# teofum/rust_raytracer

Measured on AMD Instinct MI355X. Metric: Msamples/sec (whole node), cornell_dragon 870k tri @1000spp, higher is better.
Workload: dtype f64; 1 GPU; scenes/cornell_dragon 1200x1200 @1000spp (10 replicas x 10x10 strata), 871200-tri stand-in mesh; spp=1000, seed=1, pipeline=auto, frames_in_flight=1, partition=1200-row bands round-robin over 1 GPU(s)

## Files before the change

### include/rt_mi355.h

```cpp
#ifndef RT_MI355_H
#define RT_MI355_H

#include <stdint.h>
#include <stddef.h>

#ifdef __cplusplus
extern "C" {
#endif

#define RT_MI355_ABI_VERSION 2

typedef enum RtStatus {
    RT_OK = 0,
    RT_E_INVALID = -1,
    RT_E_UNSUPPORTED = -2,
    RT_E_DEVICE = -3,
    RT_E_NOMEM = -4
} RtStatus;

typedef enum RtNodeType {
    RT_NODE_SPHERE = 1,
    RT_NODE_PLANE = 2,
    RT_NODE_MESH = 3,
    RT_NODE_LIST = 4,
// ... 58 lines not shown

typedef enum RtTextureType {
    RT_TEX_CONST_COLOR = 1,
    RT_TEX_CONST_FLOAT = 2,
    RT_TEX_CHECKER = 3,
    RT_TEX_CHECKER_SOLID = 4,
    RT_TEX_LERP = 5,
    RT_TEX_IMAGE = 6,
    RT_TEX_NOISE_SOLID = 7,
    RT_TEX_CHANNEL = 8,
    RT_TEX_UV_DEBUG = 9
} RtTextureType;

typedef struct RtTexture {
    uint32_t type;
    int32_t  a, b, c;
    uint32_t channel;
    uint32_t samples;
    double   v[3];
    double   scale;
    const float* texels;
    uint32_t width, height;
    const double*   perlin_vec;
    const uint32_t* perlin_perm;
} RtTexture;

typedef struct RtSceneDesc {
    uint32_t abi_version;
    uint32_t n_nodes;
    const RtNode* nodes;
    uint32_t n_child_indices;
    uint32_t n_transforms;
    const uint32_t* child_indices;
    const RtTransform* transforms;
    uint32_t n_meshes;
    uint32_t n_materials;
    const RtMesh* meshes;
    const RtMaterial* materials;
    uint32_t n_textures;
    uint32_t world_root;
    const RtTexture* textures;
    uint32_t lights_root;
    uint32_t flags;
} RtSceneDesc;

#define RT_SCENE_BVH_ON_DEVICE 1u

typedef struct RtCameraDesc {
    uint32_t image_width, image_height;
    double position[3];
    double first_pixel[3];
    double pixel_delta_u[3];
    double pixel_delta_v[3];
    double basis_u[3];
    double basis_v[3];
    uint32_t has_aperture;
    uint32_t _pad;
    double aperture_radius;
} RtCameraDesc;

typedef enum RtPrecision { RT_PRECISION_F64 = 0, RT_PRECISION_F32 = 1 } RtPrecision;
typedef enum RtPipeline { RT_PIPELINE_AUTO = 0, RT_PIPELINE_MEGAKERNEL = 1, RT_PIPELINE_WAVEFRONT = 2 } RtPipeline;

typedef struct RtRenderParams {
    uint32_t sqrt_spt;
    uint32_t thread_count;
    uint32_t max_depth;
    uint32_t has_background;
    double   light_bias;
    double   background[3];
    uint64_t seed;
    uint32_t band_rows;
    uint32_t n_parts;
    uint32_t part;
    uint32_t precision;
    uint32_t pipeline;
    uint32_t collect_stats;
} RtRenderParams;

typedef struct RtRenderStats {
    double   kernel_ms;
    double   traversal_kernel_ms;
    uint32_t n_launches;
    uint32_t pipeline_used;
    uint64_t samples;
    uint64_t rays;
    uint64_t mesh_rays;
    uint64_t node_visits;
    uint64_t tri_tests;
    uint64_t prim_tests;
    uint64_t bytes_node;
    uint64_t bytes_tri;
    uint64_t bytes_attr;
    uint64_t bytes_state;
    double   prims_kernel_ms;
    double   shade_kernel_ms;
    uint64_t bytes_state_prims;
    uint64_t bytes_state_shade;
    uint32_t n_iterations;
    uint32_t n_replica_groups;
    uint32_t n_tail_compactions;
    uint32_t _reserved;
} RtRenderStats;

typedef struct RtScene RtScene;

int rt_device_count(void);

int rt_scene_create(const RtSceneDesc* desc, int device, RtScene** out);
void rt_scene_destroy(RtScene* scene);

typedef struct RtSceneUpdateInfo {
    uint32_t n_meshes_refit;
    uint32_t n_triangles_refit;
    uint64_t bytes_uploaded;
    double   refit_kernel_ms;
    double   total_ms;
    uint32_t _reserved[4];
} RtSceneUpdateInfo;
int rt_scene_update(RtScene* scene, const RtSceneDesc* desc, RtSceneUpdateInfo* info_or_null);
int rt_scene_update_check(const RtSceneDesc* a, const RtSceneDesc* b);
int rt_scene_refit_mesh(const RtSceneDesc* a, const RtSceneDesc* b, uint32_t mesh, uint32_t f32, int32_t* children_out,
                        uint32_t* cones_out, float* boxes_out, uint32_t node_capacity, uint32_t* n_nodes_out,
                        double* tris_out, uint32_t* tri_order_out, uint32_t tri_capacity, uint32_t* n_tris_out);
int rt_debug_scene_mesh(const RtScene* scene, uint32_t mesh, uint32_t f32, int32_t* children_out, uint32_t* cones_out,
                        float* boxes_out, uint32_t node_capacity, uint32_t* n_nodes_out, double* tris_out,
                        uint32_t* tri_order_out, uint32_t tri_capacity, uint32_t* n_tris_out);
int rt_debug_scene_mesh_digest(const RtScene* scene, uint32_t f32, uint64_t out[8]);
int rt_debug_live_resources(uint64_t out[4]);

uint32_t rt_owned_rows(uint32_t image_height, const RtRenderParams* params);

int rt_render(const RtScene* scene, const RtCameraDesc* camera,
              const RtRenderParams* params, double* rgba_out);

int rt_render_device(const RtScene* scene, const RtCameraDesc* camera,
                     const RtRenderParams* params, double* d_rgba_out, void* stream);

int rt_get_stats(const RtScene* scene, RtRenderStats* out);

int rt_debug_trace_sample(const RtScene* scene, const RtCameraDesc* camera, const RtRenderParams* params,
                          uint32_t tid, uint32_t x, uint32_t y, uint32_t sx, uint32_t sy,
                          double* rgb_out, double* trace_out, uint32_t max_bounces);

int rt_debug_fuzzy_reflection(int device, uint32_t n, const double* reflected, const double* fuzz, const uint64_t* state, double* out, uint64_t* state_out);

#define RT_SCENE_INFO_ZERO_WEIGHT_STOP 1u
#define RT_SCENE_INFO_TEX_INTERPRETER 2u
#define RT_SCENE_INFO_VOLUMES 4u
int rt_scene_info(const RtSceneDesc* desc, uint32_t* flags_out);
int rt_scene_mesh_stats(const RtSceneDesc* desc, uint64_t out[8]);
int rt_scene_mesh_cones(const RtSceneDesc* desc, uint32_t mesh, uint32_t f32, int32_t* children_out, uint32_t* cones_out,
                        uint32_t node_capacity, uint32_t* n_nodes_out, double* tris_out, uint32_t tri_capacity, uint32_t* n_tris_out);
int rt_debug_handout_replay(const uint32_t* policy, uint32_t n, uint32_t waves, const uint32_t* order, uint32_t n_order, uint32_t* asks_out,
                            uint32_t capacity, uint32_t* n_asks_out, uint32_t* atomics_out);
int rt_scene_program(const RtSceneDesc* desc, int32_t* ops_out, uint32_t capacity, uint32_t* n_ops_out, uint64_t info[8]);

int rt_scene_set_tail_flag(RtScene* scene, int32_t* flag);

typedef struct RtAccum RtAccum;
int rt_accum_create(const RtScene* scene, const RtCameraDesc* camera, const RtRenderParams* params, RtAccum** out);
void rt_accum_destroy(RtAccum* acc);
int rt_accum_render(RtAccum* acc, uint32_t n_replicas, const RtRenderParams* params_or_null, void* stream);
uint32_t rt_accum_replicas_done(const RtAccum* acc);
int rt_accum_estimate(const RtAccum* acc, double* rgba_out);
int rt_accum_estimate_device(const RtAccum* acc, double* d_rgba_out, void* stream);
int rt_accum_preview_rgb8(const RtAccum* acc, uint8_t* rgb_out);
size_t rt_accum_state_size(const RtAccum* acc);
int rt_accum_save_state(const RtAccum* acc, void* buf, size_t size);
int rt_accum_load_state(RtAccum* acc, const void* buf, size_t size);
int rt_tonemap_rgb8_device(int device, const double* d_rgba, uint32_t width, uint32_t height, uint8_t* d_rgb, void* stream);

int rt_render_aov(const RtScene* scene, const RtCameraDesc* camera, const RtRenderParams* params, uint32_t n_replicas,
                  double* aov_out);
int rt_render_aov_device(const RtScene* scene, const RtCameraDesc* camera, const RtRenderParams* params, uint32_t n_replicas,
                         double* d_aov_out, void* stream);

#define RT_DENOISE_DEMODULATE 1u
#define RT_DENOISE_MAX_ITERATIONS 16u
typedef struct RtDenoiseParams {
    uint32_t iterations;
    uint32_t aov_replicas;
    uint32_t flags;
    uint32_t _reserved0;
    double   sigma_color, sigma_normal, sigma_albedo, sigma_depth;
    double   _reserved[4];
} RtDenoiseParams;
int rt_denoise_default_params(RtDenoiseParams* out);
int rt_denoise(int device, const double* rgba, const double* aov, uint32_t w, uint32_t h, const RtDenoiseParams* dp,
               double* rgba_out);
int rt_denoise_device(int device, const double* d_rgba, const double* d_aov, uint32_t w, uint32_t h,
                      const RtDenoiseParams* dp, double* d_rgba_out, void* stream);
int rt_accum_estimate_denoised(const RtAccum* acc, const RtDenoiseParams* dp, double* rgba_out);
int rt_accum_preview_denoised_rgb8(const RtAccum* acc, const RtDenoiseParams* dp, uint8_t* rgb_out);

typedef struct RtAdaptiveParams {
    double   threshold;
    double   floor;
    uint32_t min_replicas;
    uint32_t check_interval;
    uint32_t radius;
    uint32_t _reserved0;
    double   _reserved[4];
} RtAdaptiveParams;
int rt_adaptive_default_params(RtAdaptiveParams* out);
int rt_accum_set_adaptive(RtAccum* acc, const RtAdaptiveParams* params);
uint32_t rt_accum_active_pixels(const RtAccum* acc);
int rt_accum_finished(const RtAccum* acc);
int rt_accum_sample_counts(const RtAccum* acc, uint32_t* counts_out);
int rt_accum_noise(const RtAccum* acc, double* noise_out);

#define RT_LIGHT_GROUPS_MAX 16u
typedef struct RtLightGroups {
    uint32_t n_groups;
    uint32_t n_materials;
    const uint8_t* material_group;
    uint32_t background_group, unlit_group;
    uint32_t _reserved[4];
} RtLightGroups;
int rt_light_groups_auto(const RtSceneDesc* desc, uint32_t max_groups, int has_background, uint8_t* material_group_out,
                         uint32_t* background_group_out, uint32_t* n_groups_out);
int rt_render_light_groups(const RtScene* scene, const RtCameraDesc* camera, const RtRenderParams* params,
                           const RtLightGroups* groups, double* groups_out, double* rgba_out_or_null);
int rt_render_light_groups_device(const RtScene* scene, const RtCameraDesc* camera, const RtRenderParams* params,
                                  const RtLightGroups* groups, double* d_groups_out, double* d_rgba_out_or_null, void* stream);
int rt_light_mix(int device, const double* groups, uint32_t n_groups, uint32_t w, uint32_t h, const double* tints,
                 double* rgba_out);
int rt_light_mix_device(int device, const double* d_groups, uint32_t n_groups, uint32_t w, uint32_t h, const double* tints,
                        double* d_rgba_out, void* stream);

#define RT_RAY_HIT          1u
#define RT_RAY_FRONT_FACE   2u
#define RT_RAY_ENVIRONMENT  4u
typedef struct RtRayHit {
    double   t;
    double   pos[3], normal[3];
    double   u, v;
    int32_t  material;
    int32_t  node;
    int32_t  prim;
    uint32_t flags;
    uint64_t _reserved;
} RtRayHit;
typedef struct RtRayQueryStats {
    double   kernel_ms;
    uint64_t rays;
    uint32_t n_chunks, precision;
    uint32_t _reserved[4];
} RtRayQueryStats;

int rt_trace_rays(const RtScene* scene, uint64_t n, const double* origins, const double* dirs, uint32_t precision, RtRayHit* hits_out);
int rt_trace_rays_device(const RtScene* scene, uint64_t n, const double* d_origins, const double* d_dirs, uint32_t precision,
                         RtRayHit* d_hits_out, void* stream);
int rt_occluded(const RtScene* scene, uint64_t n, const double* origins, const double* dirs, const double* t_min, const double* t_max,
                uint32_t precision, uint8_t* out);
int rt_occluded_device(const RtScene* scene, uint64_t n, const double* d_origins, const double* d_dirs, const double* d_t_min,
                       const double* d_t_max, uint32_t precision, uint8_t* d_out, void* stream);
int rt_ray_query_stats(const RtScene* scene, RtRayQueryStats* out);
int rt_scene_op_nodes(const RtSceneDesc* desc, int32_t* nodes_out, uint32_t capacity, uint32_t* n_ops_out);

typedef struct RtBakeParams {
    uint32_t samples;
    uint32_t precision;
    uint64_t seed;
    double   bias;
    double   max_distance;
    uint32_t _reserved[4];
} RtBakeParams;
typedef struct RtBakeResult {
    double   visibility;
    double   bent[3];
} RtBakeResult;
int rt_bake_visibility(const RtScene* scene, uint64_t n, const double* positions, const double* normals, const RtBakeParams* params,
                       RtBakeResult* out);
int rt_bake_visibility_device(const RtScene* scene, uint64_t n, const double* d_positions, const double* d_normals,
                              const RtBakeParams* params, RtBakeResult* d_out, void* stream);
int rt_bake_visibility_hits_device(const RtScene* scene, uint64_t n, const RtRayHit* d_hits, const RtBakeParams* params,
                                   RtBakeResult* d_out, void* stream);
int rt_bake_stats(const RtScene* scene, RtRayQueryStats* out);

const char* rt_last_error(void);

#ifdef __cplusplus
}
#endif
#endif
```

### rust_raytracer_amd/api.py

```python
from __future__ import annotations

import ctypes as C
import os
import sys
from typing import Optional, Sequence

import numpy as np

PKG_DIR = os.path.dirname(os.path.abspath(__file__))
REPO_DIR = os.path.dirname(PKG_DIR)

RT_OK = 0
RT_E_INVALID, RT_E_UNSUPPORTED, RT_E_DEVICE, RT_E_NOMEM = -1, -2, -3, -4
RT_PRECISION_F64, RT_PRECISION_F32 = 0, 1
RT_PIPELINE_AUTO, RT_PIPELINE_MEGAKERNEL, RT_PIPELINE_WAVEFRONT = 0, 1, 2
RT_SCENE_BVH_ON_DEVICE = 1
RT_MESH_HIT_BACK_FACES = 2
RT_DENOISE_DEMODULATE = 1
RT_DENOISE_MAX_ITERATIONS = 16
AOV_CHANNELS = 8

(RT_NODE_SPHERE, RT_NODE_PLANE, RT_NODE_MESH, RT_NODE_LIST, RT_NODE_TRANSFORM, RT_NODE_BVH,
 RT_NODE_SKY, RT_NODE_SUN, RT_NODE_VOLUME, RT_NODE_NULL) = range(1, 11)
(RT_MAT_LAMBERTIAN, RT_MAT_METAL, RT_MAT_DIELECTRIC, RT_MAT_GLOSSY, RT_MAT_EMISSIVE,
# ... 128 lines not shown
                ("background_group", C.c_uint32), ("unlit_group", C.c_uint32), ("_reserved", C.c_uint32 * 4)]

    @classmethod
    def make(cls, n_groups: int, material_group, background_group: int = 0, unlit_group: int = 0) -> "RtLightGroups":
        table = np.ascontiguousarray(material_group, dtype=np.uint8).copy()
        g = cls()
        g.n_groups, g.n_materials = n_groups, table.size
        g.material_group = table.ctypes.data_as(C.POINTER(C.c_uint8))
        g.background_group, g.unlit_group = background_group, unlit_group
        g._table = table
        return g

    @property
    def table(self) -> np.ndarray:
        return self._table


class RtSceneUpdateInfo(C.Structure):
    _fields_ = [("n_meshes_refit", C.c_uint32), ("n_triangles_refit", C.c_uint32), ("bytes_uploaded", C.c_uint64),
                ("refit_kernel_ms", C.c_double), ("total_ms", C.c_double), ("_reserved", C.c_uint32 * 4)]


class RtRayQueryStats(C.Structure):
    _fields_ = [("kernel_ms", C.c_double), ("rays", C.c_uint64), ("n_chunks", C.c_uint32), ("precision", C.c_uint32),
                ("_reserved", C.c_uint32 * 4)]


RT_RAY_HIT, RT_RAY_FRONT_FACE, RT_RAY_ENVIRONMENT = 1, 2, 4
RtRayHit = np.dtype([("t", "<f8"), ("pos", "<f8", (3,)), ("normal", "<f8", (3,)), ("u", "<f8"), ("v", "<f8"), ("material", "<i4"),
                     ("node", "<i4"), ("prim", "<i4"), ("flags", "<u4"), ("_reserved", "<u8")])
assert RtRayHit.itemsize == 96


class RtBakeParams(C.Structure):
    _fields_ = [("samples", C.c_uint32), ("precision", C.c_uint32), ("seed", C.c_uint64), ("bias", C.c_double),
                ("max_distance", C.c_double), ("_reserved", C.c_uint32 * 4)]

    @classmethod
    def defaults(cls, **overrides) -> "RtBakeParams":
        p = cls(samples=64, precision=RT_PRECISION_F64, seed=0, bias=1e-3, max_distance=float("inf"))
        for k, v in overrides.items():
            setattr(p, k, v)
        return p


RtBakeResult = np.dtype([("visibility", "<f8"), ("bent", "<f8", (3,))])
assert RtBakeResult.itemsize == 32


class RtError(RuntimeError):
    def __init__(self, status: int, message: str):
        super().__init__(f"rt status {status}: {message}")
        self.status = status


HOST_LIB_PATH = os.path.join(PKG_DIR, "librt_host.so")
DEVICE_LIB_PATH = os.environ.get("RT_DEVICE_LIB") or os.path.join(PKG_DIR, "librt_mi355.so")

_host_lib = None
_device_lib = None


def load_host_lib() -> C.CDLL:
    global _host_lib
    if _host_lib is None:
        if not os.path.exists(HOST_LIB_PATH):
            raise FileNotFoundError(
                f"{HOST_LIB_PATH} is missing: run `python -c 'import __graft_entry__ as g; g.build()'`")
        lib = C.CDLL(HOST_LIB_PATH)
        lib.rth_load.argtypes = [C.c_int, C.POINTER(C.c_char_p), C.POINTER(C.c_void_p)]
        lib.rth_load.restype = C.c_int
        lib.rth_destroy.argtypes = [C.c_void_p]
        lib.rth_destroy.restype = None
        lib.rth_scene.argtypes = [C.c_void_p]
        lib.rth_scene.restype = C.POINTER(RtSceneDesc)
        lib.rth_camera.argtypes = [C.c_void_p]
        lib.rth_camera.restype = C.POINTER(RtCameraDesc)
        lib.rth_params.argtypes = [C.c_void_p]
        lib.rth_params.restype = C.POINTER(RtRenderParams)
        lib.rth_gpus.argtypes = [C.c_void_p]
        lib.rth_gpus.restype = C.c_uint32
        lib.rth_band_rows.argtypes = [C.c_uint32, C.c_uint32]
        lib.rth_band_rows.restype = C.c_uint32
        lib.rth_samples_per_pixel.argtypes = [C.c_void_p]
        lib.rth_samples_per_pixel.restype = C.c_uint32
        lib.rth_pick.argtypes = [C.c_void_p, C.c_void_p, C.c_uint32]
        lib.rth_pick.restype = C.c_uint32
        lib.rth_ao.argtypes = [C.c_void_p, C.POINTER(C.c_double)]
        lib.rth_ao.restype = C.c_uint32
        lib.rth_log.argtypes = [C.c_void_p]
        lib.rth_log.restype = C.c_char_p
        lib.rth_make_camera.argtypes = [C.c_uint32, C.c_double, C.c_double, C.c_double, C.c_double,
                                        C.POINTER(C.c_double), C.POINTER(C.c_double),
                                        C.POINTER(RtCameraDesc)]
        lib.rth_make_camera.restype = C.c_int
        lib.rth_tonemap_rgb8.argtypes = [C.c_void_p, C.c_uint32, C.c_uint32, C.c_void_p]
        lib.rth_tonemap_rgb8.restype = C.c_int
        lib.rth_save_png.argtypes = [C.c_char_p, C.c_void_p, C.c_uint32, C.c_uint32]
        lib.rth_save_png.restype = C.c_int
        lib.rth_load_image.argtypes = [C.c_char_p, C.POINTER(C.POINTER(C.c_float)), C.POINTER(C.c_uint32), C.POINTER(C.c_uint32)]
        lib.rth_load_image.restype = C.c_int
        lib.rth_free_image.argtypes = [C.POINTER(C.c_float)]
        lib.rth_free_image.restype = None
        lib.rth_last_error.argtypes = []
        lib.rth_last_error.restype = C.c_char_p
        _host_lib = lib
    return _host_lib


def load_device_lib() -> C.CDLL:
    global _device_lib
    if _device_lib is None:
        if not os.path.exists(DEVICE_LIB_PATH):
            raise FileNotFoundError(
                f"{DEVICE_LIB_PATH} is missing — the HIP render path was not built "
                "(run __graft_entry__.build()); refusing to fall back to any CPU path")
        if "torch" not in sys.modules and os.environ.get("RT_NO_TORCH_PRELOAD", "0") != "1":
            try:
                import torch
            except Exception:
                pass
        lib = C.CDLL(DEVICE_LIB_PATH)
        lib.rt_device_count.argtypes = []
        lib.rt_device_count.restype = C.c_int
        lib.rt_scene_create.argtypes = [C.POINTER(RtSceneDesc), C.c_int, C.POINTER(C.c_void_p)]
        lib.rt_scene_create.restype = C.c_int
        lib.rt_scene_destroy.argtypes = [C.c_void_p]
        lib.rt_scene_destroy.restype = None
        lib.rt_owned_rows.argtypes = [C.c_uint32, C.POINTER(RtRenderParams)]
        lib.rt_owned_rows.restype = C.c_uint32
        lib.rt_render.argtypes = [C.c_void_p, C.POINTER(RtCameraDesc), C.POINTER(RtRenderParams), C.c_void_p]
        lib.rt_render.restype = C.c_int
        lib.rt_render_device.argtypes = [C.c_void_p, C.POINTER(RtCameraDesc), C.POINTER(RtRenderParams),
                                         C.c_void_p, C.c_void_p]
        lib.rt_render_device.restype = C.c_int
        lib.rt_get_stats.argtypes = [C.c_void_p, C.POINTER(RtRenderStats)]
        lib.rt_get_stats.restype = C.c_int
        lib.rt_debug_trace_sample.argtypes = [C.c_void_p, C.POINTER(RtCameraDesc), C.POINTER(RtRenderParams),
                                              C.c_uint32, C.c_uint32, C.c_uint32, C.c_uint32, C.c_uint32,
                                              C.POINTER(C.c_double), C.POINTER(C.c_double), C.c_uint32]
        lib.rt_debug_trace_sample.restype = C.c_int
        lib.rt_scene_info.argtypes = [C.POINTER(RtSceneDesc), C.POINTER(C.c_uint32)]
        lib.rt_scene_info.restype = C.c_int
        if hasattr(lib, "rt_scene_set_tail_flag"):
            lib.rt_scene_set_tail_flag.argtypes = [C.c_void_p, C.c_void_p]
            lib.rt_scene_set_tail_flag.restype = C.c_int
        if hasattr(lib, "rt_scene_mesh_stats"):
            lib.rt_scene_mesh_stats.argtypes = [C.POINTER(RtSceneDesc), C.POINTER(C.c_uint64)]
            lib.rt_scene_mesh_stats.restype = C.c_int
        if hasattr(lib, "rt_scene_mesh_cones"):
            lib.rt_scene_mesh_cones.argtypes = [C.POINTER(RtSceneDesc), C.c_uint32, C.c_uint32, C.c_void_p, C.c_void_p, C.c_uint32,
                                                C.POINTER(C.c_uint32), C.c_void_p, C.c_uint32, C.POINTER(C.c_uint32)]
            lib.rt_scene_mesh_cones.restype = C.c_int
        if hasattr(lib, "rt_debug_handout_replay"):
            lib.rt_debug_handout_replay.argtypes = [C.c_void_p, C.c_uint32, C.c_uint32, C.c_void_p, C.c_uint32, C.c_void_p, C.c_uint32,
                                                    C.POINTER(C.c_uint32), C.c_void_p]
            lib.rt_debug_handout_replay.restype = C.c_int
        if hasattr(lib, "rt_accum_create"):
            for name, res, args in (
                    ("rt_accum_create", C.c_int, [C.c_void_p, C.POINTER(RtCameraDesc), C.POINTER(RtRenderParams), C.POINTER(C.c_void_p)]),
                    ("rt_accum_destroy", None, [C.c_void_p]),
                    ("rt_accum_render", C.c_int, [C.c_void_p, C.c_uint32, C.POINTER(RtRenderParams), C.c_void_p]),
                    ("rt_accum_replicas_done", C.c_uint32, [C.c_void_p]),
                    ("rt_accum_estimate", C.c_int, [C.c_void_p, C.c_void_p]),
                    ("rt_accum_estimate_device", C.c_int, [C.c_void_p, C.c_void_p, C.c_void_p]),
                    ("rt_accum_preview_rgb8", C.c_int, [C.c_void_p, C.c_void_p]),
                    ("rt_accum_state_size", C.c_size_t, [C.c_void_p]),
                    ("rt_accum_save_state", C.c_int, [C.c_void_p, C.c_void_p, C.c_size_t]),
                    ("rt_accum_load_state", C.c_int, [C.c_void_p, C.c_void_p, C.c_size_t]),
                    ("rt_tonemap_rgb8_device", C.c_int, [C.c_int, C.c_void_p, C.c_uint32, C.c_uint32, C.c_void_p, C.c_void_p])):
                fn = getattr(lib, name)
                fn.argtypes = args
                fn.restype = res
        if hasattr(lib, "rt_render_aov"):
            dp = C.POINTER(RtDenoiseParams)
            for name, res, args in (
                    ("rt_render_aov", C.c_int, [C.c_void_p, C.POINTER(RtCameraDesc), C.POINTER(RtRenderParams), C.c_uint32, C.c_void_p]),
                    ("rt_render_aov_device", C.c_int, [C.c_void_p, C.POINTER(RtCameraDesc), C.POINTER(RtRenderParams), C.c_uint32,
                                                       C.c_void_p, C.c_void_p]),
                    ("rt_denoise_default_params", C.c_int, [dp]),
                    ("rt_denoise", C.c_int, [C.c_int, C.c_void_p, C.c_void_p, C.c_uint32, C.c_uint32, dp, C.c_void_p]),
                    ("rt_denoise_device", C.c_int, [C.c_int, C.c_void_p, C.c_void_p, C.c_uint32, C.c_uint32, dp, C.c_void_p, C.c_void_p]),
                    ("rt_accum_estimate_denoised", C.c_int, [C.c_void_p, dp, C.c_void_p]),
                    ("rt_accum_preview_denoised_rgb8", C.c_int, [C.c_void_p, dp, C.c_void_p])):
                fn = getattr(lib, name)
                fn.argtypes = args
                fn.restype = res
        if hasattr(lib, "rt_accum_set_adaptive"):
            for name, res, args in (
                    ("rt_adaptive_default_params", C.c_int, [C.POINTER(RtAdaptiveParams)]),
                    ("rt_accum_set_adaptive", C.c_int, [C.c_void_p, C.POINTER(RtAdaptiveParams)]),
                    ("rt_accum_active_pixels", C.c_uint32, [C.c_void_p]),
                    ("rt_accum_finished", C.c_int, [C.c_void_p]),
                    ("rt_accum_sample_counts", C.c_int, [C.c_void_p, C.c_void_p]),
                    ("rt_accum_noise", C.c_int, [C.c_void_p, C.c_void_p])):
                fn = getattr(lib, name)
                fn.argtypes = args
                fn.restype = res
        if hasattr(lib, "rt_render_light_groups"):
            lg = C.POINTER(RtLightGroups)
            for name, res, args in (
                    ("rt_light_groups_auto", C.c_int, [C.POINTER(RtSceneDesc), C.c_uint32, C.c_int, C.c_void_p, C.POINTER(C.c_uint32),
                                                       C.POINTER(C.c_uint32)]),
                    ("rt_render_light_groups", C.c_int, [C.c_void_p, C.POINTER(RtCameraDesc), C.POINTER(RtRenderParams), lg, C.c_void_p,
                                                         C.c_void_p]),
                    ("rt_render_light_groups_device", C.c_int, [C.c_void_p, C.POINTER(RtCameraDesc), C.POINTER(RtRenderParams), lg,
                                                                C.c_void_p, C.c_void_p, C.c_void_p]),
                    ("rt_light_mix", C.c_int, [C.c_int, C.c_void_p, C.c_uint32, C.c_uint32, C.c_uint32, C.c_void_p, C.c_void_p]),
                    ("rt_light_mix_device", C.c_int, [C.c_int, C.c_void_p, C.c_uint32, C.c_uint32, C.c_uint32, C.c_void_p, C.c_void_p,
                                                      C.c_void_p])):
                fn = getattr(lib, name)
                fn.argtypes = args
                fn.restype = res
        if hasattr(lib, "rt_scene_update"):
            mesh_out = [C.c_void_p, C.c_void_p, C.c_void_p, C.c_uint32, C.POINTER(C.c_uint32), C.c_void_p, C.c_void_p, C.c_uint32,
                        C.POINTER(C.c_uint32)]
            for name, res, args in (
                    ("rt_scene_update", C.c_int, [C.c_void_p, C.POINTER(RtSceneDesc), C.POINTER(RtSceneUpdateInfo)]),
                    ("rt_scene_update_check", C.c_int, [C.POINTER(RtSceneDesc), C.POINTER(RtSceneDesc)]),
                    ("rt_scene_refit_mesh", C.c_int, [C.POINTER(RtSceneDesc), C.POINTER(RtSceneDesc), C.c_uint32, C.c_uint32] + mesh_out),
                    ("rt_debug_scene_mesh", C.c_int, [C.c_void_p, C.c_uint32, C.c_uint32] + mesh_out),
                    ("rt_debug_scene_mesh_digest", C.c_int, [C.c_void_p, C.c_uint32, C.POINTER(C.c_uint64)])):
                fn = getattr(lib, name)
                fn.argtypes = args
                fn.restype = res
        if hasattr(lib, "rt_trace_rays"):
            for name, res, args in (
                    ("rt_trace_rays", C.c_int, [C.c_void_p, C.c_uint64, C.c_void_p, C.c_void_p, C.c_uint32, C.c_void_p]),
                    ("rt_trace_rays_device", C.c_int, [C.c_void_p, C.c_uint64, C.c_void_p, C.c_void_p, C.c_uint32, C.c_void_p, C.c_void_p]),
                    ("rt_occluded", C.c_int, [C.c_void_p, C.c_uint64, C.c_void_p, C.c_void_p, C.c_void_p, C.c_void_p, C.c_uint32, C.c_void_p]),
                    ("rt_occluded_device", C.c_int, [C.c_void_p, C.c_uint64, C.c_void_p, C.c_void_p, C.c_void_p, C.c_void_p, C.c_uint32,
                                                     C.c_void_p, C.c_void_p]),
                    ("rt_ray_query_stats", C.c_int, [C.c_void_p, C.POINTER(RtRayQueryStats)]),
                    ("rt_scene_op_nodes", C.c_int, [C.POINTER(RtSceneDesc), C.c_void_p, C.c_uint32, C.POINTER(C.c_uint32)])):
                fn = getattr(lib, name)
                fn.argtypes = args
                fn.restype = res
        if hasattr(lib, "rt_bake_visibility"):
            for name, res, args in (
                    ("rt_bake_visibility", C.c_int, [C.c_void_p, C.c_uint64, C.c_void_p, C.c_void_p, C.POINTER(RtBakeParams), C.c_void_p]),
                    ("rt_bake_visibility_device", C.c_int, [C.c_void_p, C.c_uint64, C.c_void_p, C.c_void_p, C.POINTER(RtBakeParams),
                                                            C.c_void_p, C.c_void_p]),
                    ("rt_bake_visibility_hits_device", C.c_int, [C.c_void_p, C.c_uint64, C.c_void_p, C.POINTER(RtBakeParams), C.c_void_p,
                                                                 C.c_void_p]),
                    ("rt_bake_stats", C.c_int, [C.c_void_p, C.POINTER(RtRayQueryStats)])):
                fn = getattr(lib, name)
                fn.argtypes = args
                fn.restype = res
        if hasattr(lib, "rt_debug_live_resources"):
            lib.rt_debug_live_resources.argtypes = [C.POINTER(C.c_uint64)]
            lib.rt_debug_live_resources.restype = C.c_int
        lib.rt_last_error.argtypes = []
        lib.rt_last_error.restype = C.c_char_p
        _device_lib = lib
    return _device_lib


RT_SCENE_INFO_ZERO_WEIGHT_STOP, RT_SCENE_INFO_TEX_INTERPRETER, RT_SCENE_INFO_VOLUMES = 1, 2, 4


def scene_info(desc) -> int:
    lib = load_device_lib()
    flags = C.c_uint32()
    st = lib.rt_scene_info(desc, C.byref(flags))
    if st != RT_OK:
        raise RtError(st, lib.rt_last_error().decode())
    return flags.value


def scene_mesh_stats(desc) -> dict:
    lib = load_device_lib()
    out = (C.c_uint64 * 8)()
    st = lib.rt_scene_mesh_stats(desc, out)
    if st != RT_OK:
        raise RtError(st, lib.rt_last_error().decode())
    return dict(zip(("triangles", "bvh2_nodes", "bvh4_nodes", "bvh2_depth", "bvh4_stack", "ops", "rebuilt_groups", "rebuilt_prims"),
                    [int(x) for x in out]))


def live_resources() -> tuple:
    lib = load_device_lib()
    out = (C.c_uint64 * 4)()
    st = lib.rt_debug_live_resources(out)
    if st != RT_OK:
        raise RtError(st, lib.rt_last_error().decode())
    return tuple(int(x) for x in out)


def handout_replay(n: int, waves: int, order, policy=None, out=None) -> tuple:
    lib = load_device_lib()
    order = np.ascontiguousarray(order, dtype=np.uint32)
    pol = None if policy is None else np.asarray(policy, dtype=np.uint32)
    cap = n // 64 + 4 * waves + 16
    if out is None or out.shape[0] < cap:
        out = np.empty((cap, 3), dtype=np.uint32)
    n_asks = C.c_uint32(0)
    atomics = np.zeros(2, dtype=np.uint32)
    st = lib.rt_debug_handout_replay(None if pol is None else pol.ctypes.data, n, waves, order.ctypes.data, order.size, out.ctypes.data,
                                     out.shape[0], C.byref(n_asks), atomics.ctypes.data)
    if st != 0:
        raise RuntimeError(f"rt_debug_handout_replay: {lib.rt_last_error().decode()}")
    if n_asks.value > out.shape[0]:
        raise RuntimeError(f"rt_debug_handout_replay: {n_asks.value} asks for n = {n}, {waves} waves")
    return out[:n_asks.value], int(atomics[0]), int(atomics[1])


def scene_mesh_cones(desc, mesh: int = 0, f32: bool = False) -> tuple:
    import numpy as np
    lib = load_device_lib()
    nn, nt = C.c_uint32(), C.c_uint32()
    st = lib.rt_scene_mesh_cones(desc, mesh, int(f32), None, None, 0, C.byref(nn), None, 0, C.byref(nt))
    if st != RT_OK:
        raise RtError(st, lib.rt_last_error().decode())
    children = np.zeros((nn.value, 4), dtype=np.int32)
    cones = np.zeros((nn.value, 4), dtype=np.uint32)
    tris = np.zeros((nt.value, 3, 3), dtype=np.float64)
    st = lib.rt_scene_mesh_cones(desc, mesh, int(f32), children.ctypes.data, cones.ctypes.data, nn.value, C.byref(nn),
                                 tris.ctypes.data, nt.value, C.byref(nt))
    if st != RT_OK:
        raise RtError(st, lib.rt_last_error().decode())
    return children, cones.view(np.int8).reshape(-1, 4, 4), tris


def scene_update_check(a, b) -> None:
    lib = load_device_lib()
    st = lib.rt_scene_update_check(a, b)
    if st != RT_OK:
        raise RtError(st, lib.rt_last_error().decode())


def _mesh_export(call) -> dict:
    lib = load_device_lib()
    nn, nt = C.c_uint32(), C.c_uint32()
    st = call(None, None, None, 0, C.byref(nn), None, None, 0, C.byref(nt))
    if st != RT_OK:
        raise RtError(st, lib.rt_last_error().decode())
    children = np.zeros((nn.value, 4), dtype=np.int32)
    cones = np.zeros((nn.value, 4), dtype=np.uint32)
    boxes = np.zeros((nn.value, 4, 2, 3), dtype=np.float32)
    tris = np.zeros((nt.value, 3, 3), dtype=np.float64)
    order = np.zeros(nt.value, dtype=np.uint32)
    st = call(children.ctypes.data, cones.ctypes.data, boxes.ctypes.data, nn.value, C.byref(nn), tris.ctypes.data, order.ctypes.data,
              nt.value, C.byref(nt))
    if st != RT_OK:
        raise RtError(st, lib.rt_last_error().decode())
    return {"children": children, "cones": cones.view(np.int8).reshape(-1, 4, 4), "boxes": boxes, "tris": tris, "order": order}


def scene_refit_mesh(a, b, mesh: int = 0, f32: bool = False) -> dict:
    lib = load_device_lib()
    return _mesh_export(lambda *out: lib.rt_scene_refit_mesh(a, b, mesh, int(f32), *out))


def scene_program(desc) -> tuple:
    import numpy as np
    lib = load_device_lib()
    lib.rt_scene_program.argtypes = [C.POINTER(RtSceneDesc), C.POINTER(C.c_int32), C.c_uint32, C.POINTER(C.c_uint32), C.POINTER(C.c_uint64)]
    lib.rt_scene_program.restype = C.c_int
    n = C.c_uint32()
    info = (C.c_uint64 * 8)()
    st = lib.rt_scene_program(desc, None, 0, C.byref(n), info)
    if st != RT_OK:
        raise RtError(st, lib.rt_last_error().decode())
    ops = np.zeros((n.value, 4), dtype=np.int32)
    st = lib.rt_scene_program(desc, ops.ctypes.data_as(C.POINTER(C.c_int32)), n.value, C.byref(n), info)
    if st != RT_OK:
        raise RtError(st, lib.rt_last_error().decode())
    plan = int(info[6])
    return ops, {"mesh_ops": int(info[0]), "groups": int(info[1]), "group_nodes": int(info[2]), "group_stack": int(info[3]),
                 "lights": int(info[4]), "volumes": int(info[5]), "group_prims": int(info[7]),
                 "split": bool(plan & 1), "vol_prims": bool(plan & 2), "multi_mesh": bool(plan & 4), "group_bvh": bool(plan & 8)}


def scene_op_nodes(desc) -> np.ndarray:
    lib = load_device_lib()
    n = C.c_uint32()
    st = lib.rt_scene_op_nodes(desc, None, 0, C.byref(n))
    if st != RT_OK:
        raise RtError(st, lib.rt_last_error().decode())
    nodes = np.full(n.value, -1, dtype=np.int32)
    st = lib.rt_scene_op_nodes(desc, nodes.ctypes.data, n.value, C.byref(n))
    if st != RT_OK:
        raise RtError(st, lib.rt_last_error().decode())
    return nodes


def light_groups_auto(desc, max_groups: int = RT_LIGHT_GROUPS_MAX, has_background: bool = False) -> RtLightGroups:
    lib = load_device_lib()
    d = desc.contents if hasattr(desc, "contents") else desc
    table = np.zeros(d.n_materials, dtype=np.uint8)
    bg, n = C.c_uint32(), C.c_uint32()
    st = lib.rt_light_groups_auto(desc, max_groups, int(bool(has_background)), table.ctypes.data, C.byref(bg), C.byref(n))
    if st != RT_OK:
        raise RtError(st, lib.rt_last_error().decode())
    return RtLightGroups.make(n.value, table, bg.value, 0)


def light_mix(groups: np.ndarray, tints, device: int = 0) -> np.ndarray:
    lib = load_device_lib()
    groups = np.ascontiguousarray(groups, dtype=np.float64)
    if groups.ndim != 4 or groups.shape[3] != 4:
        raise ValueError(f"light_mix: expected a (G, H, W, 4) array, got {groups.shape}")
    g, h, w = groups.shape[:3]
    tints = np.asarray(tints, dtype=np.float64)
    if tints.ndim == 1:
        tints = np.repeat(tints[:, None], 3, axis=1)
    tints = np.ascontiguousarray(tints)
    if tints.shape != (g, 3):
        raise ValueError(f"light_mix: expected {g} x 3 tints, got {tints.shape}")
    out = np.empty((h, w, 4), dtype=np.float64)
    st = lib.rt_light_mix(device, groups.ctypes.data, g, w, h, tints.ctypes.data, out.ctypes.data)
    if st != RT_OK:
        raise RtError(st, lib.rt_last_error().decode())
    return out


def owned_rows(height: int, params: RtRenderParams) -> list:
    if params.band_rows == 0 or params.n_parts <= 1:
        return list(range(height))
    return [y for y in range(height) if (y // params.band_rows) % params.n_parts == params.part]


class HostScene:

    def __init__(self, args: Sequence[str], cwd: Optional[str] = None):
        lib = load_host_lib()
        argv = [b"rtrace"] + [a.encode() for a in args]
        arr = (C.c_char_p * len(argv))(*argv)
        handle = C.c_void_p()
        old = os.getcwd()
        try:
            os.chdir(cwd or REPO_DIR)
            st = lib.rth_load(len(argv), arr, C.byref(handle))
        finally:
            os.chdir(old)
        if st != RT_OK:
            raise RtError(st, lib.rth_last_error().decode())
        self._lib = lib
        self._h = handle
        self.desc = lib.rth_scene(handle)
        self.camera = lib.rth_camera(handle).contents
        self.params = lib.rth_params(handle).contents.copy()
        self.gpus = lib.rth_gpus(handle)
        self.spp = lib.rth_samples_per_pixel(handle)
        self.log = lib.rth_log(handle).decode()
        xy = np.zeros((lib.rth_pick(handle, None, 0), 2), dtype=np.uint32)
        lib.rth_pick(handle, xy.ctypes.data, len(xy))
        self.pick = [(int(x), int(y)) for x, y in xy]
        dist = C.c_double()
        self.ao = (int(lib.rth_ao(handle, C.byref(dist))), dist.value)

    @property
    def width(self) -> int:
        return self.camera.image_width

    @property
    def height(self) -> int:
        return self.camera.image_height

    def close(self):
        if self._h:
            self._lib.rth_destroy(self._h)
            self._h = None

    def __del__(self):
        try:
            self.close()
        except Exception:
            pass


def tonemap_rgb8(rgba: np.ndarray) -> np.ndarray:
    lib = load_host_lib()
    rgba = np.ascontiguousarray(rgba, dtype=np.float64)
    h, w = rgba.shape[:2]
    out = np.empty((h, w, 3), dtype=np.uint8)
# ... 420 lines not shown
```

### rust_raytracer_amd/csrc/rt_bvh.cpp

```cpp
#include "rt_bvh.h"

#include <algorithm>
#include <cmath>
#include <cstdlib>
#include <limits>

#include "rt_refit.h"
#include "rt_scene.h"

namespace rt {
namespace {

constexpr int kMaxBins = 64;
static int g_bins = 16;
constexpr double kInf = std::numeric_limits<double>::infinity();

struct Box {
    double lo[3] = {kInf, kInf, kInf};
    double hi[3] = {-kInf, -kInf, -kInf};
    void grow(const double* p) {
        for (int a = 0; a < 3; a++) {
            if (p[a] < lo[a]) lo[a] = p[a];
            if (p[a] > hi[a]) hi[a] = p[a];
        }
// ... 125 lines not shown
    BvhBuild out;
    if (n_tris <= b.max_leaf) {
        BuildNode root{};
        Box bx;
        for (uint32_t t = 0; t < n_tris; t++) bx.grow(b.tri_box[t]);
        for (int a = 0; a < 3; a++) {
            root.lo0[a] = bx.lo[a]; root.hi0[a] = bx.hi[a];
            root.lo1[a] = kInf; root.hi1[a] = -kInf;
        }
        root.c0 = n_tris ? Builder::leaf_ref(0, n_tris) : kEmptyChild;
        root.c1 = kEmptyChild;
        out.nodes.push_back(root);
        out.max_depth = 1;
    } else {
        Box root_box;
        b.build(0, n_tris, &root_box, 0);
        out.nodes = std::move(b.nodes);
        out.max_depth = b.max_depth;
    }
    out.tri_order = std::move(b.order);
    return out;
}


namespace {
struct Cand {
    int32_t ref;
    double lo[3], hi[3];
    double area() const {
        double dx = hi[0] - lo[0], dy = hi[1] - lo[1], dz = hi[2] - lo[2];
        if (!(dx >= 0 && dy >= 0 && dz >= 0)) return -1.0;
        return dx * dy + dy * dz + dz * dx;
    }
};
template <int W>
struct Collapser {
    const BvhBuild& b2;
    BvhNBuild<W> out;
    uint32_t build(int32_t n2, uint32_t depth, uint32_t stack_above) {
        uint32_t idx = uint32_t(out.nodes.size());
        out.nodes.emplace_back();
        if (depth + 1 > out.max_depth) out.max_depth = depth + 1;
        std::vector<Cand> c;
        auto add_children = [&](int32_t node2) {
            const BuildNode& n = b2.nodes[size_t(node2)];
            Cand a{n.c0, {n.lo0[0], n.lo0[1], n.lo0[2]}, {n.hi0[0], n.hi0[1], n.hi0[2]}};
            Cand b{n.c1, {n.lo1[0], n.lo1[1], n.lo1[2]}, {n.hi1[0], n.hi1[1], n.hi1[2]}};
            if (a.ref != kEmptyChild) c.push_back(a);
            if (b.ref != kEmptyChild) c.push_back(b);
        };
        add_children(n2);
        for (;;) {
            if (c.size() >= size_t(W)) break;
            int best = -1;
            double best_area = -1.0;
            for (size_t i = 0; i < c.size(); i++)
                if (c[i].ref >= 0 && c[i].area() > best_area) { best_area = c[i].area(); best = int(i); }
            if (best < 0) break;
            int32_t expand = c[size_t(best)].ref;
            c.erase(c.begin() + best);
            add_children(expand);
        }
        uint32_t n_children = uint32_t(c.size());
        uint32_t stack_here = stack_above + (n_children > 0 ? n_children - 1 : 0);
        if (stack_here + 1 > out.max_stack) out.max_stack = stack_here + 1;
        BuildNodeN<W> node{};
        for (int k = 0; k < W; k++) {
            node.child[k] = kEmptyChild;
            for (int a = 0; a < 3; a++) { node.lo[k][a] = kInf; node.hi[k][a] = -kInf; }
        }
        for (uint32_t k = 0; k < n_children; k++) {
            for (int a = 0; a < 3; a++) { node.lo[k][a] = c[k].lo[a]; node.hi[k][a] = c[k].hi[a]; }
            node.child[k] = c[k].ref;
        }
        out.nodes[idx] = node;
        for (uint32_t k = 0; k < n_children; k++)
            if (c[k].ref >= 0) {
                uint32_t child_idx = build(c[k].ref, depth + 1, stack_here);
                out.nodes[idx].child[k] = int32_t(child_idx);
            }
        return idx;
    }
};
}

namespace {
template <int W>
BvhNBuild<W> collapse(const BvhBuild& b2) {
    Collapser<W> c{b2, {}};
    c.out.nodes.reserve(b2.nodes.size() / (W == 4 ? 2 : 3) + 4);
    c.build(0, 0, 0);
    for (int a = 0; a < 3; a++) { c.out.root_lo[a] = kInf; c.out.root_hi[a] = -kInf; }
    const BuildNodeN<W>& r = c.out.nodes[0];
    for (int k = 0; k < W; k++)
        if (r.child[k] != kEmptyChild)
            for (int a = 0; a < 3; a++) {
                c.out.root_lo[a] = std::min(c.out.root_lo[a], r.lo[k][a]);
                c.out.root_hi[a] = std::max(c.out.root_hi[a], r.hi[k][a]);
            }
    return std::move(c.out);
}
}

Bvh4Build collapse_bvh4(const BvhBuild& b2) { return collapse<4>(b2); }



ConeLimits cone_limits(bool f32) {
    if (f32) return ConeLimits{1.0 / 32.0, 1e-12, 1e12};
    return ConeLimits{1.0 / 1048576.0, 1e-100, 1e100};
}

void build_mesh_cones(const std::vector<BuildNode4>& nodes4, const std::vector<TriRec<double>>& tris, const ConeLimits& lim,
                      std::vector<uint32_t>* out) {
    const size_t n_tris = tris.size();
    std::vector<double> normal(3 * n_tris);
    const double kNaN = std::numeric_limits<double>::quiet_NaN();
    for (size_t t = 0; t < n_tris; t++) rf_tri_normal(tris[t].v0, tris[t].e1, tris[t].e2, lim, &normal[3 * t]);
    struct Below {
        uint32_t lo = UINT32_MAX, hi = 0, count = 0;
        double sum[3] = {0.0, 0.0, 0.0};
        void add(const Below& o) {
            lo = std::min(lo, o.lo); hi = std::max(hi, o.hi); count += o.count;
            for (int a = 0; a < 3; a++) sum[a] += o.sum[a];
        }
    };
    auto cone_word = [&](const Below& b) -> uint32_t { return rf_cone_word(normal.data(), b.lo, b.hi, b.count, b.sum); };
    out->assign(4 * nodes4.size(), kNeutralCone);
    std::vector<Below> below(nodes4.size());
    for (size_t i = nodes4.size(); i-- > 0;) {
        const BuildNode4& nd = nodes4[i];
        Below all;
        for (int k = 0; k < 4; k++) {
            const int32_t ch = nd.child[k];
            if (ch == kEmptyChild) continue;
            Below b;
            if (ch >= 0) {
                if (size_t(ch) <= i || size_t(ch) >= nodes4.size()) { all.sum[0] = kNaN; continue; }
                b = below[size_t(ch)];
            } else {
                const uint32_t code = uint32_t(~ch), first = code >> 3, count = (code & 7u) + 1u;
                if (size_t(first) + count > n_tris) { all.sum[0] = kNaN; continue; }
                b.lo = first; b.hi = first + count; b.count = count;
                for (uint32_t t = first; t < first + count; t++)
                    for (int a = 0; a < 3; a++) b.sum[a] += normal[3 * size_t(t) + a];
            }
            (*out)[4 * i + size_t(k)] = cone_word(b);
            all.add(b);
        }
        below[i] = all;
    }
}

}
```

### rust_raytracer_amd/csrc/rt_bvh.h

```cpp
#pragma once
#include <cstdint>
#include <string>
#include <vector>

#include "rt_scene.h"

namespace rt {

struct BuildNode {
    double lo0[3], hi0[3], lo1[3], hi1[3];
    int32_t c0, c1;
};

struct BvhBuild {
    std::vector<BuildNode> nodes;
    std::vector<uint32_t> tri_order;
    uint32_t max_depth = 0;
};

BvhBuild build_bvh(const double* positions, const uint32_t* tri_pos, uint32_t n_tris, uint32_t max_leaf);

bool build_bvh_device(const double* positions, uint32_t n_positions, const uint32_t* tri_pos, uint32_t n_tris, uint32_t max_leaf,
                      BvhBuild* out, std::string* err);

template <int W>
struct BuildNodeN {
    double lo[W][3], hi[W][3];
    int32_t child[W];
};
template <int W>
struct BvhNBuild {
    std::vector<BuildNodeN<W>> nodes;
    uint32_t max_depth = 0;
    uint32_t max_stack = 0;
    double root_lo[3], root_hi[3];
};
using BuildNode4 = BuildNodeN<4>;
using Bvh4Build = BvhNBuild<4>;
Bvh4Build collapse_bvh4(const BvhBuild& bvh2);

struct ConeLimits {
    double sigma;
    double min_edge;
    double max_edge;
};
ConeLimits cone_limits(bool f32);
void build_mesh_cones(const std::vector<BuildNode4>& nodes4, const std::vector<TriRec<double>>& tris, const ConeLimits& lim,
                      std::vector<uint32_t>* out);

}
```

### rust_raytracer_amd/csrc/rt_kernels.hip

```cpp
#include <hip/hip_runtime.h>

#include <algorithm>
#include <array>
#include <chrono>
#include <cmath>
#include <cstdio>
#include <cstdlib>
#include <cstring>
#include <memory>
#include <new>
#include <string>
#include <type_traits>
#include <variant>
#include <vector>

#include "rt_aov.h"
#include "rt_bake.h"
#include "rt_compile.h"
#include "rt_device.h"
#include "rt_owned.h"
#include "rt_query.h"
#include "rt_refit.h"
#include "rt_wavefront.h"

// ... 85 lines not shown
    }
}

template <typename R>
__global__ void k_trace_sample(SceneView<R> sc, CameraView<R> cam, ParamsView<R> prm, uint32_t tid, uint32_t px, uint32_t py,
                               uint32_t sx, uint32_t sy, double* rgb, double* trace, uint32_t max_bounces, uint32_t* n_out) {
    extern __shared__ int lds_stack[];
    if (threadIdx.x != 0) return;
    LaneCounters cnt;
    Rng rng;
    rng.key(prm.seed, tid, uint64_t(py) * cam.width + px, sy * cam.sqrt_spt + sx);
    PathState<R> ps;
    ps.ray = get_ray(cam, px, py, sx, sy, rng);
    ps.throughput = mk<R>(1, 1, 1);
    ps.radiance = mk<R>(0, 0, 0);
    ps.depth = cam.max_depth;
    uint32_t n = 0;
    while (ps.depth != 0) {
        Best<R> best;
        world_test<R, false, true>(sc, ps.ray, R(0.001), best, lds_stack, int(blockDim.x), cnt, &rng);
        if (n < max_bounces) {
            double* t = trace + 17 * n;
            for (int k = 0; k < 17; k++) t[k] = 0;
            t[0] = double(best.t);
            t[4] = -1; t[5] = -1; t[6] = double(best.tri);
            if (best.pc >= 0) {
                HitInfo<R> h = resolve_hit<R, true>(sc, ps.ray, best);
                t[1] = double(h.pos.x); t[2] = double(h.pos.y); t[3] = double(h.pos.z);
                t[4] = double(h.material);
                t[5] = double(sc.ops[best.pc].type);
                t[8] = double(h.normal.x); t[9] = double(h.normal.y); t[10] = double(h.normal.z);
            }
            t[11] = double(ps.ray.o.x); t[12] = double(ps.ray.o.y); t[13] = double(ps.ray.o.z);
            t[14] = double(ps.ray.d.x); t[15] = double(ps.ray.d.y); t[16] = double(ps.ray.d.z);
        }
        n++;
        bool cont = shade<R, false, true>(sc, prm, ps, best, rng, cnt);
        ps.depth--;
        if (cont && ps.depth == 0) end_black(ps);
        if (!cont) break;
    }
    rgb[0] = double(ps.radiance.x); rgb[1] = double(ps.radiance.y); rgb[2] = double(ps.radiance.z);
    *n_out = n;
}

struct DeviceBuffers {
    std::vector<DevBuf<char>> allocs;
    uint64_t uploaded_bytes = 0;
    void adopt(DeviceBuffers& from, const void* p) {
        auto it = std::find_if(from.allocs.begin(), from.allocs.end(), [p](const DevBuf<char>& b) { return b.get() == p; });
        if (it == from.allocs.end()) return;
        allocs.push_back(std::move(*it));
        from.allocs.erase(it);
    }
    template <typename T> int alloc(size_t bytes, T** out) {
        allocs.emplace_back();
        if (int st = allocs.back().reserve(bytes)) return st;
        *out = reinterpret_cast<T*>(allocs.back().get());
        return RT_OK;
    }
    template <typename T> int upload(const std::vector<T>& v, const T** out) {
        *out = nullptr;
        T* p = nullptr;
        if (int st = alloc((v.empty() ? 1 : v.size()) * sizeof(T), &p)) return st;
        if (!v.empty()) HIP_TRY(hipMemcpy(p, v.data(), v.size() * sizeof(T), hipMemcpyHostToDevice));
        uploaded_bytes += v.size() * sizeof(T);
        *out = p;
        return RT_OK;
    }
};

template <typename R, size_t N> void cast_arr(R (&dst)[N], const double (&src)[N]) {
    for (size_t i = 0; i < N; i++) dst[i] = R(src[i]);
}

template <typename R>
struct DeviceScene {
    using Real = R;
    DeviceBuffers buf;
    SceneView<R> view{};

    int build(const CompiledScene& cs, const DeviceScene<R>* keep = nullptr) {
        const bool mesh_tables = keep == nullptr;
        std::vector<Bounds<R>> bounds(cs.bounds.size());
        for (size_t i = 0; i < bounds.size(); i++) {
            cast_arr(bounds[i].lo, cs.bounds[i].lo);
            cast_arr(bounds[i].hi, cs.bounds[i].hi);
        }
        std::vector<Xform<R>> xforms(cs.xforms.size());
        for (size_t i = 0; i < xforms.size(); i++) {
            cast_arr(xforms[i].m, cs.xforms[i].m);
            cast_arr(xforms[i].inv, cs.xforms[i].inv);
        }
        std::vector<SpherePrim<R>> spheres(cs.spheres.size());
        for (size_t i = 0; i < spheres.size(); i++) {
            cast_arr(spheres[i].center, cs.spheres[i].center);
            spheres[i].radius = R(cs.spheres[i].radius);
            spheres[i].material = cs.spheres[i].material;
            spheres[i]._pad = 0;
        }
        std::vector<PlanePrim<R>> planes(cs.planes.size());
        for (size_t i = 0; i < planes.size(); i++) {
            const auto& s = cs.planes[i];
            cast_arr(planes[i].corner, s.corner); cast_arr(planes[i].normal, s.normal);
            cast_arr(planes[i].u, s.u); cast_arr(planes[i].v, s.v);
            cast_arr(planes[i].inv_u, s.inv_u); cast_arr(planes[i].inv_v, s.inv_v);
            planes[i].area = R(s.area);
            planes[i].material = s.material;
            planes[i].backface = s.backface;
        }
        std::vector<SunPrim<R>> suns(cs.suns.size());
        for (size_t i = 0; i < suns.size(); i++) {
            cast_arr(suns[i].direction, cs.suns[i].direction);
            suns[i].material = cs.suns[i].material;
            suns[i]._pad = 0;
        }
        std::vector<BvhNode<R>> nodes(mesh_tables ? cs.nodes.size() : 0);
        for (size_t i = 0; i < nodes.size(); i++) {
            const BuildNode& s = cs.nodes[i];
            BvhNode<R>& n = nodes[i];
            for (int a = 0; a < 3; a++) {
                rf_pad_box2<R>(s.lo0[a], s.hi0[a], &n.lo0[a], &n.hi0[a]);
                rf_pad_box2<R>(s.lo1[a], s.hi1[a], &n.lo1[a], &n.hi1[a]);
            }
            n.c0 = s.c0;
            n.c1 = s.c1;
        }
        std::vector<BvhNode4f> nodes4(mesh_tables ? cs.nodes4.size() : 0);
        {
            size_t inst = 0;
            std::vector<std::pair<uint32_t, double>> pads;
            for (const MeshInst& mi : cs.meshes) {
                const Bounds<double>& b = cs.mesh_bounds[inst++];
                pads.emplace_back(mi.node4_base, rf_pad_of_box(b.lo, b.hi));
            }
            std::sort(pads.begin(), pads.end());
            size_t pi = 0;
            for (size_t i = 0; i < nodes4.size(); i++) {
                while (pi + 1 < pads.size() && pads[pi + 1].first <= i) pi++;
                const double m = pads.empty() ? 0.0 : pads[pi].second;
                const BuildNode4& sn = cs.nodes4[i];
                BvhNode4f& dn = nodes4[i];
                for (int k = 0; k < 4; k++) {
                    float* lo[3] = {&dn.lox[k], &dn.loy[k], &dn.loz[k]};
                    float* hi[3] = {&dn.hix[k], &dn.hiy[k], &dn.hiz[k]};
                    for (int a = 0; a < 3; a++) rf_pad_box4f(sn.lo[k][a], sn.hi[k][a], m, lo[a], hi[a]);
                    dn.child[k] = sn.child[k];
                    dn._pad[k] = 0;
                }
            }
        }
        std::vector<BvhNode4q> nodes4q(mesh_tables ? cs.nodes4.size() : 0);
        std::vector<BvhNode4q> group_nodes;
        {
            auto pad_of = [&]() {
                std::vector<std::pair<uint32_t, double>> pads;
                size_t inst = 0;
                for (const MeshInst& mi : cs.meshes) {
                    const Bounds<double>& b = cs.mesh_bounds[inst++];
                    pads.emplace_back(mi.node4_base, rf_pad_of_box(b.lo, b.hi));
                }
                std::sort(pads.begin(), pads.end());
                return pads;
            };
            auto quantise = [](const BuildNode4& sn, double m, BvhNode4q& qn) -> bool {
                for (int k = 0; k < 4; k++) qn.child[k] = sn.child[k];
                return rf_quantise4(sn.lo, sn.hi, sn.child, m, qn.org, qn.cell, qn.qlo, qn.qhi);
            };
            const auto pads4 = pad_of();
            size_t pi = 0;
            for (size_t i = 0; i < nodes4q.size(); i++) {
                while (pi + 1 < pads4.size() && pads4[pi + 1].first <= i) pi++;
                const BuildNode4& sn = cs.nodes4[i];
                BvhNode4q& qn = nodes4q[i];
                if (!quantise(sn, pads4.empty() ? 0.0 : pads4[pi].second, qn))
                    return set_err(RT_E_UNSUPPORTED, "BVH node does not fit the 8-bit grid");
            }
            group_nodes.resize(cs.group_nodes4.size());
            for (size_t g = 0; g < cs.groups.size(); g++) {
                const GroupRec<double>& gr = cs.groups[g];
                double S = 0.0;
                for (int a = 0; a < 3; a++) S = std::fmax(S, std::fmax(std::fabs(gr.lo[a]), std::fabs(gr.hi[a])));
                if (!std::isfinite(S)) return set_err(RT_E_UNSUPPORTED, "primitive group with an unbounded box");
                const size_t end = g + 1 < cs.groups.size() ? cs.groups[g + 1].root : cs.group_nodes4.size();
                for (size_t i = gr.root; i < end; i++) {
                    const BuildNode4& sn = cs.group_nodes4[i];
                    BvhNode4q& qn = group_nodes[i];
                    if (!quantise(sn, S * (1.0 / 524288.0), qn))
                        return set_err(RT_E_UNSUPPORTED, "group BVH node does not fit the 8-bit grid");
                }
            }
        }
        std::vector<uint32_t> cone_words;
        if (mesh_tables) build_mesh_cones(cs.nodes4, cs.tris, cone_limits(sizeof(R) == 4), &cone_words);
        std::vector<MeshNode4qc> nodes4qc(mesh_tables ? cs.nodes4.size() : 0);
        for (size_t i = 0; i < nodes4qc.size(); i++) {
            nodes4qc[i].node = nodes4q[i];
            for (int k = 0; k < 4; k++) nodes4qc[i].cones.word[k] = cone_words[4 * i + size_t(k)];
            for (uint32_t& x : nodes4qc[i]._pad) x = 0;
        }
        std::vector<Bounds<R>> mesh_bounds(cs.mesh_bounds.size());
        for (size_t i = 0; i < mesh_bounds.size(); i++)
            for (int a = 0; a < 3; a++) {
                mesh_bounds[i].lo[a] = round_down<R>(cs.mesh_bounds[i].lo[a]);
                mesh_bounds[i].hi[a] = round_up<R>(cs.mesh_bounds[i].hi[a]);
            }
        std::vector<TriRec<R>> tris(mesh_tables ? cs.tris.size() : 0);
        for (size_t i = 0; i < tris.size(); i++) {
            cast_arr(tris[i].v0, cs.tris[i].v0); cast_arr(tris[i].e1, cs.tris[i].e1); cast_arr(tris[i].e2, cs.tris[i].e2);
            tris[i]._pad = R(0);
        }
        std::vector<TriAttr<R>> attrs(mesh_tables ? cs.attrs.size() : 0);
        for (size_t i = 0; i < attrs.size(); i++) {
            const auto& s = cs.attrs[i];
            cast_arr(attrs[i].n0, s.n0); cast_arr(attrs[i].n1, s.n1); cast_arr(attrs[i].n2, s.n2);
            cast_arr(attrs[i].uv0, s.uv0); cast_arr(attrs[i].uv1, s.uv1); cast_arr(attrs[i].uv2, s.uv2);
            attrs[i].has_uv = s.has_uv;
            attrs[i]._pad = 0;
        }
        std::vector<MaterialParams<R>> mparams(cs.material_params.size());
        for (size_t i = 0; i < mparams.size(); i++) {
            mparams[i].ior = R(cs.material_params[i].ior);
            mparams[i].inv_ior = R(cs.material_params[i].inv_ior);
            auto r0_of = [](R x) { R r0 = (R(1) - x) / (R(1) + x); return r0 * r0; };
            mparams[i].inv_ior_r = R(1) / mparams[i].ior;
            mparams[i].r0_glossy = r0_of(mparams[i].inv_ior);
            mparams[i].r0_front = r0_of(mparams[i].inv_ior_r);
            mparams[i].r0_back = r0_of(mparams[i].ior);
        }
        std::vector<TextureRec<R>> textures(cs.textures.size());
        for (size_t i = 0; i < textures.size(); i++) {
            const auto& s = cs.textures[i];
            textures[i].type = s.type; textures[i].aux = s.aux; textures[i].data = s.data;
            textures[i].width = s.width; textures[i].height = s.height; textures[i]._pad = 0;
            cast_arr(textures[i].v, s.v);
            textures[i].scale = R(s.scale);
        }
        std::vector<VolumeRec<R>> volumes(cs.volumes.size());
        for (size_t i = 0; i < volumes.size(); i++) {
            volumes[i].neg_inv_density = R(cs.volumes[i].neg_inv_density);
            volumes[i].material = cs.volumes[i].material;
            volumes[i]._pad = 0;
        }
        std::vector<R> perlin_vec(cs.perlin_vec.size());
        for (size_t i = 0; i < perlin_vec.size(); i++) perlin_vec[i] = R(cs.perlin_vec[i]);
        int st;
        if ((st = buf.upload(cs.ops, &view.ops)) != RT_OK) return st;
        if ((st = buf.upload(bounds, &view.bounds)) != RT_OK) return st;
        if ((st = buf.upload(cs.chain_offsets, &view.chain_offsets)) != RT_OK) return st;
        if ((st = buf.upload(cs.chain_items, &view.chain_items)) != RT_OK) return st;
        if ((st = buf.upload(xforms, &view.xforms)) != RT_OK) return st;
        if ((st = buf.upload(spheres, &view.spheres)) != RT_OK) return st;
        if ((st = buf.upload(planes, &view.planes)) != RT_OK) return st;
        if ((st = buf.upload(suns, &view.suns)) != RT_OK) return st;
        if ((st = buf.upload(cs.meshes, &view.meshes)) != RT_OK) return st;
        if ((st = buf.upload(volumes, &view.volumes)) != RT_OK) return st;
        if (mesh_tables) {
            if ((st = buf.upload(nodes, &view.nodes)) != RT_OK) return st;
            if ((st = buf.upload(nodes4, &view.nodes4)) != RT_OK) return st;
            if ((st = buf.upload(nodes4qc, &view.nodes4q)) != RT_OK) return st;
            if ((st = buf.upload(tris, &view.tris)) != RT_OK) return st;
            if ((st = buf.upload(attrs, &view.attrs)) != RT_OK) return st;
        } else {
            view.nodes = keep->view.nodes; view.nodes4 = keep->view.nodes4; view.nodes4q = keep->view.nodes4q;
            view.tris = keep->view.tris; view.attrs = keep->view.attrs;
        }
        if ((st = buf.upload(mesh_bounds, &view.mesh_bounds)) != RT_OK) return st;
        if ((st = buf.upload(cs.mesh_ops, &view.mesh_ops)) != RT_OK) return st;
        view.n_mesh_ops = int32_t(cs.mesh_ops.size());
        std::vector<MeshOpRec<R>> mesh_op_recs(cs.mesh_ops.size());
        for (size_t m = 0; m < mesh_op_recs.size(); m++) {
            const Op& op = cs.ops[size_t(cs.mesh_ops[m])];
            const MeshInst& mi = cs.meshes[size_t(op.arg)];
            MeshOpRec<R>& r = mesh_op_recs[m];
            r.pc = cs.mesh_ops[m];
            r.chain = op.chain;
            r.node4_base = mi.node4_base;
            const int32_t cb = cs.chain_offsets[size_t(op.chain)], ce = cs.chain_offsets[size_t(op.chain) + 1];
            r.flags = (mi.flags & 0xFFFFu) | (uint32_t(std::min(ce - cb, 0xFFFF)) << 16);
            for (int a = 0; a < 3; a++) { r.lo[a] = mesh_bounds[size_t(op.arg)].lo[a]; r.hi[a] = mesh_bounds[size_t(op.arg)].hi[a]; }
            for (int k = 0; k < 12; k++) r.inv[k] = ce - cb == 1 ? xforms[size_t(cs.chain_items[size_t(cb)])].inv[k] : R(0);
        }
        if ((st = buf.upload(mesh_op_recs, &view.mesh_op_recs)) != RT_OK) return st;
        std::vector<GroupRec<R>> groups(cs.groups.size());
        for (size_t g = 0; g < groups.size(); g++) {
            groups[g].root = cs.groups[g].root;
            for (int a = 0; a < 3; a++) { groups[g].lo[a] = round_down<R>(cs.groups[g].lo[a]); groups[g].hi[a] = round_up<R>(cs.groups[g].hi[a]); }
        }
        if ((st = buf.upload(groups, &view.groups)) != RT_OK) return st;
        if ((st = buf.upload(group_nodes, &view.group_nodes)) != RT_OK) return st;
        if ((st = buf.upload(cs.group_prims, &view.group_prims)) != RT_OK) return st;
        if ((st = buf.upload(cs.group_guards, &view.group_guards)) != RT_OK) return st;
        view.n_group_nodes = int32_t(group_nodes.size());
        view.group_stack_levels = int32_t(cs.max_group_stack);
        if ((st = buf.upload(cs.materials, &view.materials)) != RT_OK) return st;
        if ((st = buf.upload(mparams, &view.material_params)) != RT_OK) return st;
        if ((st = buf.upload(textures, &view.textures)) != RT_OK) return st;
        if ((st = buf.upload(cs.texels, &view.texels)) != RT_OK) return st;
        if ((st = buf.upload(perlin_vec, &view.perlin_vec)) != RT_OK) return st;
        if ((st = buf.upload(cs.perlin_perm, &view.perlin_perm)) != RT_OK) return st;
        if ((st = buf.upload(cs.lights, &view.lights)) != RT_OK) return st;
        {
            struct Tbl { const void* data; size_t bytes; };
            const Tbl tbl[ST_COUNT] = {
                {cs.ops.data(), cs.ops.size() * sizeof(Op)}, {bounds.data(), bounds.size() * sizeof(Bounds<R>)},
                {cs.chain_offsets.data(), cs.chain_offsets.size() * 4}, {cs.chain_items.data(), cs.chain_items.size() * 4},
                {xforms.data(), xforms.size() * sizeof(Xform<R>)}, {spheres.data(), spheres.size() * sizeof(SpherePrim<R>)},
                {planes.data(), planes.size() * sizeof(PlanePrim<R>)}, {suns.data(), suns.size() * sizeof(SunPrim<R>)},
                {cs.meshes.data(), cs.meshes.size() * sizeof(MeshInst)}, {cs.materials.data(), cs.materials.size() * sizeof(MaterialRec)},
                {mparams.data(), mparams.size() * sizeof(MaterialParams<R>)}, {textures.data(), textures.size() * sizeof(TextureRec<R>)},
                {cs.lights.data(), cs.lights.size() * sizeof(LightRec)}};
            auto pack = [&](const int (&order)[ST_COUNT], SmallLayout& L, const char** out) -> int {
                std::vector<char> blob;
                for (int k : order) {
                    const size_t off = (blob.size() + 15) & ~size_t(15);
                    blob.resize(off + tbl[k].bytes);
                    if (tbl[k].bytes) std::memcpy(blob.data() + off, tbl[k].data, tbl[k].bytes);
                    L.begin[k] = uint32_t(off);
                    L.end[k] = uint32_t(off + tbl[k].bytes);
                }
                blob.resize((blob.size() + 15) & ~size_t(15));
                L.total_bytes = uint32_t(blob.size());
                return buf.upload(blob, out);
            };
            const int order_prims[ST_COUNT] = {ST_OPS, ST_CHAIN_OFFSETS, ST_CHAIN_ITEMS, ST_XFORMS, ST_MESHES, ST_SUNS, ST_PLANES, ST_BOUNDS, ST_SPHERES,
                                               ST_MATERIALS, ST_MATERIAL_PARAMS, ST_LIGHTS, ST_TEXTURES};
            const int order_shade[ST_COUNT] = {ST_OPS, ST_CHAIN_OFFSETS, ST_CHAIN_ITEMS, ST_XFORMS, ST_MESHES, ST_SUNS, ST_LIGHTS, ST_PLANES, ST_MATERIALS,
                                               ST_MATERIAL_PARAMS, ST_TEXTURES, ST_SPHERES, ST_BOUNDS};
            if ((st = pack(order_prims, view.lay, &view.small_blob)) != RT_OK) return st;
            if ((st = pack(order_shade, view.lay_shade, &view.small_blob_shade)) != RT_OK) return st;
        }
        view.n_lights = cs.n_top_lights;
        view.inv_n_lights = R(1) / R(cs.n_top_lights);
        view.lights_is_list = cs.lights_is_list;
        view.stop_on_zero_weight = cs.zero_weight_stop ? 1 : 0;
        if (const char* e = std::getenv("RT_ZERO_WEIGHT_STOP")) view.stop_on_zero_weight = std::atoi(e) != 0;
        view.stack_entries = int32_t(std::max(cs.max_bvh_depth + 2, cs.max_bvh4_stack + 1));
        view.n_ops = int32_t(cs.ops.size());
        HIP_TRY(hipDeviceSynchronize());
        return RT_OK;
    }
    void take_mesh_tables(DeviceScene<R>& from) {
        for (const void* p : {(const void*)view.nodes, (const void*)view.nodes4, (const void*)view.nodes4q, (const void*)view.tris, (const void*)view.attrs})
            buf.adopt(from.buf, p);
    }
};

struct HeldDesc {
    RtSceneDesc d{};
    std::vector<RtNode> nodes;
    std::vector<uint32_t> child_indices;
// ... 99 lines not shown
    return "scene update: the description has another structure than the scene (first difference: " + field + ")";
}

template <typename R>
struct PathPool {
    WfPool<R> view{};
    WfPool<R>* dev = nullptr;
    uint32_t* queue[2] = {nullptr, nullptr};
    uint32_t* mesh_queue = nullptr;
    std::vector<DevBuf<char>> owned;
};
template <typename R> using PoolPair = std::array<PathPool<R>, 2>;
using AnyPools = std::variant<std::monostate, PoolPair<float>, PoolPair<double>>;

struct ChunkStage {
    DevBuf<char> staging;
    Event ev0, ev1;
};

}

struct RtScene {
    int device = -1;
    rt::CompiledScene compiled;
    std::unique_ptr<rt::DeviceScene<double>> f64;
    std::unique_ptr<rt::DeviceScene<float>> f32;
    rt::Stream stream;
    rt::Event ev0, ev1;
    rt::DevBuf<rt::DeviceCounters> d_counters;
    RtRenderStats stats{};
    int32_t* tail_flag = nullptr;
    uint64_t content_digest = 0;
    rt::HeldDesc held;
    uint64_t generation = 0;
    std::vector<rt::RefitMesh> refit;
    struct Wavefront {
        rt::AnyPools pools;
        rt::DevBuf<uint2> mesh_spill;
        rt::DevBuf<rt::WfCounters> d_ctr;
        rt::PinnedBuf<rt::WfCounters> h_ctr;
        rt::DevBuf<double> sample_L, acc;
        rt::DevBuf<uint8_t> sample_G, lg_table;
        rt::DevBuf<double> acc_g;
        rt::Event ev_res[2];
        std::vector<rt::Event> events;
    } wf;
    struct Query {
        rt::AnyPools pools;
        rt::DevBuf<uint2> mesh_spill;
        rt::DevBuf<rt::WfCounters> d_ctr;
        rt::PinnedBuf<rt::WfCounters> h_ctr;
        rt::DevBuf<int32_t> op_node;
        rt::DevBuf<uint32_t> tri_order;
        uint64_t tables_generation = ~0ull;
        rt::ChunkStage stage;
        RtRayQueryStats stats{};
    } rq;
    struct Bake {
        rt::ChunkStage stage;
        RtRayQueryStats stats{};
    } bake;
    ~RtScene() { if (device >= 0) (void)hipSetDevice(device); }
};

namespace rt {

template <typename R> CameraView<R> make_camera_view(const RtCameraDesc& c, const RtRenderParams& p) {
    CameraView<R> v{};
    for (int i = 0; i < 3; i++) {
        v.position[i] = R(c.position[i]);
        v.first_pixel[i] = R(c.first_pixel[i]);
        v.pdu[i] = R(c.pixel_delta_u[i]);
        v.pdv[i] = R(c.pixel_delta_v[i]);
        v.basis_u[i] = R(c.basis_u[i]);
        v.basis_v[i] = R(c.basis_v[i]);
    }
    v.aperture_radius = R(c.aperture_radius);
    v.inv_sqrt_spt = R(1.0 / double(p.sqrt_spt));
    v.has_aperture = int32_t(c.has_aperture);
    v.width = c.image_width;
    v.height = c.image_height;
    v.sqrt_spt = p.sqrt_spt;
    v.thread_count = p.thread_count;
    v.max_depth = p.max_depth;
    return v;
}

template <typename R> ParamsView<R> make_params_view(const RtRenderParams& p, uint32_t owned) {
    ParamsView<R> v{};
    v.light_bias = R(p.light_bias);
    for (int i = 0; i < 3; i++) v.background[i] = p.has_background ? R(p.background[i]) : R(0);
    v.seed = p.seed;
    v.band_rows = p.band_rows;
    v.n_parts = p.n_parts;
    v.part = p.part;
    v.owned_rows = owned;
    v.spp = double(p.sqrt_spt) * double(p.sqrt_spt) * double(p.thread_count);
    v.inv_spp = 1.0 / v.spp;
    return v;
}

template <typename R>
int render_typed(RtScene* s, DeviceScene<R>& ds, const RtCameraDesc& cam, const RtRenderParams& p, uint32_t owned,
                 uint32_t t_first, uint32_t n, double* d_out, hipStream_t stream) {
    CameraView<R> cv = make_camera_view<R>(cam, p);
    ParamsView<R> pv = make_params_view<R>(p, owned);
    const uint32_t tiles_x = (cam.image_width + 15u) / 16u, tiles_y = (owned + 15u) / 16u;
    const dim3 grid(tiles_x * tiles_y), block(256);
    const size_t lds = size_t(ds.view.stack_entries) * 256 * sizeof(int);
    if (lds > 160 * 1024) return set_err(RT_E_UNSUPPORTED, "mesh BVH too deep for the LDS traversal stack");
    HIP_TRY(hipMemsetAsync(s->d_counters, 0, sizeof(DeviceCounters), stream));
    HIP_TRY(hipEventRecord(s->ev0, stream));
    const bool tex = s->compiled.needs_tex_interpreter || !s->compiled.volumes.empty();
#define RT_LAUNCH_MEGA(ST, TX) hipLaunchKernelGGL((k_megakernel<R, ST, TX>), grid, block, lds, stream, ds.view, cv, pv, d_out, s->d_counters.get(), t_first, n)
    if (p.collect_stats) { if (tex) RT_LAUNCH_MEGA(true, true); else RT_LAUNCH_MEGA(true, false); }
    else { if (tex) RT_LAUNCH_MEGA(false, true); else RT_LAUNCH_MEGA(false, false); }
#undef RT_LAUNCH_MEGA
    HIP_TRY(hipGetLastError());
    HIP_TRY(hipEventRecord(s->ev1, stream));
    HIP_TRY(hipStreamSynchronize(stream));
    float ms = 0.f;
    HIP_TRY(hipEventElapsedTime(&ms, s->ev0, s->ev1));
    DeviceCounters hc{};
    HIP_TRY(hipMemcpy(&hc, s->d_counters, sizeof hc, hipMemcpyDeviceToHost));
    RtRenderStats& st = s->stats;
    st = RtRenderStats{};
    st.kernel_ms = ms;
    st.traversal_kernel_ms = ms;
    st.n_launches = 1;
    st.pipeline_used = RT_PIPELINE_MEGAKERNEL;
    st.samples = uint64_t(cam.image_width) * owned * p.sqrt_spt * p.sqrt_spt * n;
    st.rays = hc.rays;
    st.mesh_rays = hc.mesh_rays;
    st.node_visits = hc.node_visits;
    st.tri_tests = hc.tri_tests;
    st.prim_tests = hc.prim_tests;
    st.bytes_node = sizeof(BvhNode<R>);
    st.bytes_tri = sizeof(TriRec<R>);
    st.bytes_attr = sizeof(TriAttr<R>);
    st.bytes_state = 0;
    return RT_OK;
}

template <typename R>
int aov_typed(RtScene* s, DeviceScene<R>& ds, const RtCameraDesc& cam, const RtRenderParams& p, uint32_t owned, uint32_t n,
              double* d_out, hipStream_t stream) {
    if (size_t(ds.view.stack_entries) * 256 * sizeof(int) > 160 * 1024) return set_err(RT_E_UNSUPPORTED, "mesh BVH too deep for the LDS traversal stack");
    const bool tex = s->compiled.needs_tex_interpreter || !s->compiled.volumes.empty();
    HIP_TRY(aov_launch<R>(ds.view, make_camera_view<R>(cam, p), make_params_view<R>(p, owned), tex, n, d_out, stream));
    HIP_TRY(hipStreamSynchronize(stream));
    return RT_OK;
}

static uint32_t env_u32(const char* name, uint32_t dflt) {
    const char* v = std::getenv(name);
    if (!v || !*v) return dflt;
    return uint32_t(std::strtoul(v, nullptr, 10));
}

template <typename R> using IntersectKernel = decltype(&k_wf_intersect<R, false, false>);
template <typename R> using PrimsKernel = decltype(&k_wf_prims<R, false, 0, false, false>);
template <typename R> using MeshKernel = decltype(&k_wf_mesh<R, false, 1, false>);
template <typename R, typename G> using ShadeKernel = decltype(&k_wf_shade<R, false, 0, false, G, false>);

template <typename R>
IntersectKernel<R> pick_intersect(bool stats, bool vol) {
    if (stats) return vol ? &k_wf_intersect<R, true, true> : &k_wf_intersect<R, true, false>;
    return vol ? &k_wf_intersect<R, false, true> : &k_wf_intersect<R, false, false>;
}

template <typename R, bool ST>
PrimsKernel<R> pick_prims_st(bool vol, bool groups, int lds) {
    if (vol) return &k_wf_prims<R, ST, 0, true, false>;
    if (groups) return lds == 2 ? &k_wf_prims<R, ST, 2, false, true> : (lds == 1 ? &k_wf_prims<R, ST, 1, false, true> : &k_wf_prims<R, ST, 0, false, true>);
    return lds == 2 ? &k_wf_prims<R, ST, 2, false, false> : (lds == 1 ? &k_wf_prims<R, ST, 1, false, false> : &k_wf_prims<R, ST, 0, false, false>);
}
template <typename R>
PrimsKernel<R> pick_prims(bool stats, bool vol, bool groups, int lds) {
    return stats ? pick_prims_st<R, true>(vol, groups, lds) : pick_prims_st<R, false>(vol, groups, lds);
}

template <typename R, bool ST>
MeshKernel<R> pick_mesh_st(int node_kind, bool multi) {
    if (node_kind == 1) return multi ? &k_wf_mesh<R, ST, 1, true> : &k_wf_mesh<R, ST, 1, false>;
    return multi ? &k_wf_mesh<R, ST, 0, true> : &k_wf_mesh<R, ST, 0, false>;
}
template <typename R>
MeshKernel<R> pick_mesh(bool stats, int node_kind, bool multi) {
    return stats ? pick_mesh_st<R, true>(node_kind, multi) : pick_mesh_st<R, false>(node_kind, multi);
}

template <typename R, typename G>
ShadeKernel<R, G> pick_shade_lean(int lds, bool tex) {
    if (tex) return &k_wf_shade<R, false, 0, true, G>;
    return lds == 1 ? &k_wf_shade<R, false, 1, false, G> : (lds == 2 ? &k_wf_shade<R, false, 2, false, G> : &k_wf_shade<R, false, 0, false, G>);
}
template <typename R>
ShadeKernel<R, WfGroup<R>> pick_shade(bool stats, int lds, bool tex, bool fuse) {
    if (fuse) return &k_wf_shade<R, false, 1, false, WfGroup<R>, true>;
    if (!stats) return pick_shade_lean<R, WfGroup<R>>(lds, tex);
    if (tex) return &k_wf_shade<R, true, 0, true>;
    return lds == 1 ? &k_wf_shade<R, true, 1, false> : (lds == 2 ? &k_wf_shade<R, true, 2, false> : &k_wf_shade<R, true, 0, false>);
}

template <typename R>
struct SearchSetup {
    WavefrontPlan plan;
    bool stats, vol;
    bool use_split, prims_only, split;
    bool multi_mesh;
    int node_kind;
    uint32_t cones_on;
    int mesh_levels, lds_levels;
    uint32_t refill_min, inner_min;
    HandoutPolicy handout;
    bool lds_tables;
    uint32_t lds_budget;
    bool groups;
    uint32_t group_levels;
    size_t lds_groups;
    uint32_t staged_prims;
    int lds_prims;
    size_t lds_isect, lds_mesh, lds_prims_launch;
    uint32_t isect_blocks;
    int blocks_per_cu;
    size_t spill_bytes;
    IntersectKernel<R> k_intersect;
    PrimsKernel<R> k_prims;
    MeshKernel<R> k_mesh;
};

static uint32_t staged_prefix(const SmallLayout& L, bool lds_tables, uint32_t lds_budget) {
    if (!lds_tables) return 0u;
    if (L.total_bytes <= lds_budget) return L.total_bytes;
    uint32_t best = 0;
    for (int k = 0; k < ST_COUNT; k++)
        if (L.end[k] <= lds_budget && L.end[k] > best) best = L.end[k];
    return (best + 15u) & ~15u;
}

template <typename R>
int make_search_setup(RtScene* s, DeviceScene<R>& ds, bool stats, bool vol, SearchSetup<R>* out) {
    SearchSetup<R>& su = *out;
    su.stats = stats;
    su.vol = vol;
    su.lds_isect = size_t(ds.view.stack_entries) * 256 * sizeof(int);
    if (su.lds_isect > 160 * 1024) return set_err(RT_E_UNSUPPORTED, "mesh BVH too deep for the LDS traversal stack");
    su.plan = plan_wavefront(s->compiled);
    const int n_mesh_ops = int(s->compiled.mesh_ops.size());
    su.use_split = env_u32("RT_WF_SPLIT", 1) != 0 && su.plan.split;
    su.prims_only = su.use_split && n_mesh_ops == 0;
    su.split = su.use_split && n_mesh_ops > 0;
    su.multi_mesh = su.plan.multi_mesh || env_u32("RT_WF_MESH_MULTI", 0) != 0;
    su.node_kind = env_u32("RT_WF_NODES", 1) != 0 ? 1 : 0;
    su.cones_on = env_u32("RT_WF_CONES", 1) != 0 ? 1u : 0u;
    su.mesh_levels = int(s->compiled.max_bvh4_stack) + 1;
    su.lds_levels = std::min<int>(su.mesh_levels, int(env_u32("RT_WF_LDS_LEVELS", 12)));
    su.lds_mesh = size_t(su.lds_levels) * 256 * sizeof(uint2) + 4 * kMeshWaveLds<R>;
    su.refill_min = env_u32("RT_WF_REFILL", 32);
    su.inner_min = env_u32("RT_WF_INNER_MIN", 24);
    su.handout.mode = std::min<uint32_t>(env_u32("RT_WF_HANDOUT", 2), 2u);
    su.handout.left256 = env_u32("RT_WF_HANDOUT_256", kHandoutLeft256);
    su.handout.left128 = std::min<uint32_t>(env_u32("RT_WF_HANDOUT_128", kHandoutLeft128), su.handout.left256);
    su.lds_tables = env_u32("RT_LDS_TABLES", 1) != 0;
    su.lds_budget = env_u32("RT_LDS_BUDGET", 32u * 1024u);
    su.group_levels = uint32_t(ds.view.group_stack_levels);
    const size_t group_node_bytes = size_t(ds.view.n_group_nodes) * sizeof(BvhNode4q);
    su.groups = (su.split || su.prims_only) && su.plan.groups && env_u32("RT_WF_GROUPS", 1) != 0;
    su.lds_groups = su.groups ? size_t(su.group_levels) * 256 * 8 + group_node_bytes : 0;
    su.staged_prims = staged_prefix(ds.view.lay, su.lds_tables, su.lds_budget);
    if (su.groups && su.lds_groups + su.staged_prims > 44u * 1024u) su.staged_prims = 0;
    su.lds_prims = su.staged_prims == 0 ? 0 : (su.staged_prims == ds.view.lay.total_bytes ? 1 : 2);
    su.lds_prims_launch = (vol ? size_t(0) : size_t(su.staged_prims) + su.lds_groups) + (WF_CHUNK + 4) * 4;
    su.k_intersect = pick_intersect<R>(stats, vol);
    su.k_prims = pick_prims<R>(stats, vol, su.groups, su.lds_prims);
    su.k_mesh = pick_mesh<R>(stats, su.node_kind, su.multi_mesh);
    int n_cu = 0, blocks_per_cu = 0;
    HIP_TRY(hipDeviceGetAttribute(&n_cu, hipDeviceAttributeMultiprocessorCount, s->device));
    if (su.split) HIP_TRY(hipOccupancyMaxActiveBlocksPerMultiprocessor(&blocks_per_cu, su.k_mesh, 256, su.lds_mesh));
    else HIP_TRY(hipOccupancyMaxActiveBlocksPerMultiprocessor(&blocks_per_cu, pick_intersect<R>(false, vol), 256, su.lds_isect));
    if (blocks_per_cu < 1) blocks_per_cu = 1;
    if (su.split) blocks_per_cu = std::min<int>(blocks_per_cu, int(env_u32("RT_WF_MESH_BLOCKS", 64)));
    su.isect_blocks = uint32_t(n_cu) * uint32_t(blocks_per_cu);
    su.blocks_per_cu = blocks_per_cu;
    if (const uint32_t grid = env_u32("RT_WF_MESH_GRID", 0)) su.isect_blocks = std::min<uint32_t>(grid, 16384u);
    su.spill_bytes = su.split ? size_t(std::max(su.mesh_levels - su.lds_levels, 1)) * su.isect_blocks * 256 * sizeof(uint2) : size_t(0);
    return RT_OK;
}

struct SearchQueues {
    const uint32_t* queue;
    uint32_t* mesh_queue;
    void* mesh_spill;
    WfCounters* ctr;
    DeviceCounters* counters;
    hipStream_t stream;
};
template <typename R>
void launch_prims(const SearchSetup<R>& su, const DeviceScene<R>& ds, const WfPool<R>& pool, const SearchQueues& sq, uint32_t n_queued) {
    hipLaunchKernelGGL(su.k_prims, dim3((n_queued + WF_CHUNK - 1) / WF_CHUNK), dim3(256), su.lds_prims_launch, sq.stream, ds.view, pool, sq.queue,
                       sq.mesh_queue, sq.ctr, sq.counters, su.staged_prims, su.group_levels);
}
template <typename R>
void launch_mesh(const SearchSetup<R>& su, const DeviceScene<R>& ds, const WfPool<R>& pool, const SearchQueues& sq) {
    hipLaunchKernelGGL(su.k_mesh, dim3(su.isect_blocks), dim3(256), su.lds_mesh, sq.stream, ds.view, pool, sq.mesh_queue, sq.ctr, sq.counters,
                       su.refill_min, su.inner_min, static_cast<uint2*>(sq.mesh_spill), su.lds_levels, &sq.ctr->n_mesh, &sq.ctr->cursor, su.cones_on, su.handout.mode, su.handout.left256, su.handout.left128);
}
template <typename R>
void launch_intersect(const SearchSetup<R>& su, const DeviceScene<R>& ds, const WfPool<R>& pool, const SearchQueues& sq) {
    hipLaunchKernelGGL(su.k_intersect, dim3(su.isect_blocks), dim3(256), su.lds_isect, sq.stream, ds.view, pool, sq.queue, sq.ctr, sq.counters,
                       su.refill_min, su.handout.mode, su.handout.left256, su.handout.left128);
}

template <typename R>
int build_pool(PathPool<R>& pl, uint32_t capacity, bool full, int n_queues, const char* nomem) {
    pl = PathPool<R>{};
    WfPool<R>& v = pl.view;
    v.capacity = capacity;
    std::vector<std::pair<void**, size_t>> want;
    auto per_slot = [&](auto** at, size_t each) { want.emplace_back(reinterpret_cast<void**>(at), size_t(capacity) * each); };
    for (R** r : {&v.ox, &v.oy, &v.oz, &v.dx, &v.dy, &v.dz, &v.ht, &v.hu, &v.hv}) per_slot(r, sizeof(R));
    per_slot(&v.hpc, 4);
    per_slot(&v.htri, 4);
    if (full) {
        for (R** r : {&v.tr, &v.tg, &v.tb}) per_slot(r, sizeof(R));
        per_slot(&v.rng, 8);
        per_slot(&v.sample, 8);
        per_slot(&v.depth, 4);
    }
    for (int q = 0; q < n_queues; q++) per_slot(&pl.queue[q], 4);
    if (n_queues) per_slot(&pl.mesh_queue, 4);
    if (full) want.emplace_back(reinterpret_cast<void**>(&pl.dev), sizeof(WfPool<R>));
    const uint32_t limit = env_u32("RT_WF_FAKE_OOM_ABOVE", 0);
    int st = RT_OK;
    for (size_t i = 0; i < want.size() && st == RT_OK; i++) {
        pl.owned.emplace_back();
        if (limit && capacity > limit && i + 1 == want.size()) st = set_err(RT_E_NOMEM, std::string(nomem) + " (RT_WF_FAKE_OOM_ABOVE)");
        else st = pl.owned.back().reserve(want[i].second, nomem);
        *want[i].first = pl.owned.back().get();
    }
    if (st == RT_OK && full)
        if (const hipError_t e = hipMemcpy(pl.dev, &v, sizeof v, hipMemcpyHostToDevice); e != hipSuccess) st = set_err(RT_E_DEVICE, std::string("hipMemcpy: ") + hipGetErrorString(e));
    if (st != RT_OK) pl = PathPool<R>{};
    return st;
}

template <typename R>
int wf_ensure(RtScene* s, uint32_t capacity) {
    RtScene::Wavefront& w = s->wf;
    const auto* have = std::get_if<PoolPair<R>>(&w.pools);
    if (have && (*have)[0].view.capacity == capacity) return RT_OK;
    w.pools = std::monostate{};
    const char* nomem = "path pool does not fit in device memory";
    if (int st = w.d_ctr.reserve(sizeof(WfCounters), nomem)) return st;
    if (int st = w.h_ctr.reserve(sizeof(WfCounters), nomem)) return st;
    w.events.resize(136);
    for (Event& e : w.events)
        if (int st = e.ensure()) return st;
    PoolPair<R> pp;
    if (int st = build_pool(pp[0], capacity, true, 2, nomem)) return st;
    if (int st = build_pool(pp[1], std::max<uint32_t>(64u, uint32_t((uint64_t(capacity) * 3 + 3) / 4)), true, 0, nomem)) return st;
    w.pools = std::move(pp);
    return RT_OK;
}

struct AdaptivePass {
    const uint32_t* active = nullptr;
    uint32_t n_active = 0;
    bool sparse = false;
    double *s1 = nullptr, *s2 = nullptr;
    uint32_t* cnt = nullptr;
};

struct LightGroupPass {
    uint32_t n_groups = 0, n_materials = 0;
    const uint8_t* table = nullptr;
    double* d_groups_out = nullptr;
};

static uint32_t wf_pool_capacity(uint32_t strata, uint64_t npix_frame, uint32_t T) {
    const double total_samples = double(strata) * double(npix_frame) * double(T);
    double c = 134217728.0 * std::sqrt(total_samples / 1.44e9);
    c = std::fmin(std::fmax(c, 1048576.0), 134217728.0);
    uint32_t capacity = env_u32("RT_WF_POOL", uint32_t(c) & ~0xFFFFFu);
    if (capacity > (1u << 28)) capacity = 1u << 28;
    if (uint64_t(capacity) > uint64_t(strata) * npix_frame * T) capacity = uint32_t(uint64_t(strata) * npix_frame * T);
    return std::max<uint32_t>(capacity, 64u);
}

static int wf_plan_samples(RtScene::Wavefront& w, uint64_t per_replica, uint64_t npix, uint32_t n, bool adaptive, const LightGroupPass* lg,
                           hipStream_t stream, uint32_t* group_out) {
    size_t free_b = 0, total_b = 0;
    HIP_TRY(hipMemGetInfo(&free_b, &total_b));
    size_t budget = size_t(env_u32("RT_WF_SAMPLE_GB", 64)) << 30;
    size_t avail = free_b + w.sample_L.bytes() + (lg ? w.sample_G.bytes() : size_t(0));
    if (budget > avail / 2) budget = avail / 2;
    uint64_t bytes_per_replica = per_replica * (lg ? 25ull : 24ull);
    uint32_t group = uint32_t(std::min<uint64_t>(n, std::max<uint64_t>(1, budget / bytes_per_replica)));
    group = (n + (n + group - 1) / group - 1) / ((n + group - 1) / group);
    if (bytes_per_replica > avail) return set_err(RT_E_NOMEM, "per-sample radiance buffer of one replica does not fit in device memory");
    if (int st = w.sample_L.reserve(size_t(per_replica) * 24 * group)) return st;
    if (lg) {
        if (int st = w.sample_G.reserve(size_t(per_replica) * group)) return st;
        if (int st = w.acc_g.reserve(group < n ? size_t(npix) * 24 * lg->n_groups : size_t(0))) return st;
        const size_t need_t = size_t(lg->n_materials) + 2;
        if (int st = w.lg_table.reserve(need_t)) return st;
        HIP_TRY(hipMemcpyAsync(w.lg_table, lg->table, need_t, hipMemcpyHostToDevice, stream));
        HIP_TRY(hipStreamSynchronize(stream));
        for (Event& e : w.ev_res)
            if (int st = e.ensure()) return st;
    }
    if (group < n && !adaptive)
        if (int st = w.acc.reserve(size_t(npix) * 24)) return st;
    *group_out = group;
    return RT_OK;
}

template <typename R>
int wf_trace_dump(const WfPool<R>& pool, uint32_t first, const uint32_t* queue, uint32_t n_in, uint32_t iteration) {
    const uint32_t n = std::min<uint32_t>(std::min(first, pool.capacity), env_u32("RT_WF_TRACE", 0));
    std::vector<R> a[12];
    R* src[12] = {pool.ox, pool.oy, pool.oz, pool.dx, pool.dy, pool.dz, pool.tr, pool.tg, pool.tb, pool.ht, pool.hu, pool.hv};
    for (int k = 0; k < 12; k++) { a[k].resize(n); HIP_TRY(hipMemcpy(a[k].data(), src[k], n * sizeof(R), hipMemcpyDeviceToHost)); }
    std::vector<uint64_t> rngs(n), smp(n);
    std::vector<uint32_t> dep(n), qn(first);
    std::vector<int32_t> hpc(n);
    HIP_TRY(hipMemcpy(rngs.data(), pool.rng, n * 8, hipMemcpyDeviceToHost));
    HIP_TRY(hipMemcpy(smp.data(), pool.sample, n * 8, hipMemcpyDeviceToHost));
    HIP_TRY(hipMemcpy(dep.data(), pool.depth, n * 4, hipMemcpyDeviceToHost));
    HIP_TRY(hipMemcpy(hpc.data(), pool.hpc, n * 4, hipMemcpyDeviceToHost));
    HIP_TRY(hipMemcpy(qn.data(), queue, size_t(n_in) * 4, hipMemcpyDeviceToHost));
    std::fprintf(stderr, "[wf trace] iteration %u: %u paths queued:", iteration, n_in);
    for (uint32_t k = 0; k < n_in && k < 64; k++) std::fprintf(stderr, " %u", qn[k]);
    std::fprintf(stderr, "\n");
    for (uint32_t k = 0; k < n; k++)
        std::fprintf(stderr, "  slot %u sample %llu depth %u o %.17g %.17g %.17g d %.17g %.17g %.17g thr %.6g %.6g %.6g hit t %.17g pc %d rng %016llx\n", k,
                     (unsigned long long)smp[k], dep[k], double(a[0][k]), double(a[1][k]), double(a[2][k]), double(a[3][k]), double(a[4][k]),
                     double(a[5][k]), double(a[6][k]), double(a[7][k]), double(a[8][k]), double(a[9][k]), hpc[k], (unsigned long long)rngs[k]);
    return RT_OK;
}

struct WfTally {
    double phase_ms[3];
    double resolve_ms;
    uint32_t search_launches;
    uint32_t iterations, n_groups, n_compactions;
};

template <typename R>
int wf_fill_stats(RtScene* s, const SearchSetup<R>& su, const WfTally& ty, const LightGroupPass* lg, bool fusable, uint64_t samples) {
    float ms = 0.f;
    HIP_TRY(hipEventElapsedTime(&ms, s->ev0, s->ev1));
    DeviceCounters hc{};
    HIP_TRY(hipMemcpy(&hc, s->d_counters, sizeof hc, hipMemcpyDeviceToHost));
    RtRenderStats& st = s->stats;
    st = RtRenderStats{};
    st.kernel_ms = ms;
    st.traversal_kernel_ms = su.prims_only ? 0.0 : ty.phase_ms[1];
    st.prims_kernel_ms = (su.split || su.prims_only) ? ty.phase_ms[0] : 0.0;
// ... 1053 lines not shown
    const MeshExportOut o{children_out, cones_out, boxes_out, node_capacity, n_nodes_out, tris_out, tri_order_out, tri_capacity, n_tris_out};
    return with_tables(s, f32 ? RT_PRECISION_F32 : RT_PRECISION_F64, [&](auto& ds) { return mesh_export_device(s->compiled, *g, ds, o); });
}

int rt_debug_scene_mesh_digest(const RtScene* scene, uint32_t f32, uint64_t out[8]) {
    using namespace rt;
    if (!scene || !out) return set_err(RT_E_INVALID, "rt_debug_scene_mesh_digest: NULL argument");
    RtScene* s = const_cast<RtScene*>(scene);
    HIP_TRY(hipSetDevice(s->device));
    const CompiledScene& cs = s->compiled;
    std::vector<char> h;
    auto digest_of = [&](const void* d_ptr, size_t bytes, uint64_t* o) -> int {
        h.resize(bytes);
        if (bytes) HIP_TRY(hipMemcpy(h.data(), d_ptr, bytes, hipMemcpyDeviceToHost));
        Digest g;
        g.bytes(h.data(), bytes);
        *o = g.value();
        return RT_OK;
    };
    for (int k = 0; k < 8; k++) out[k] = 0;
    if (int st = with_tables(s, f32 ? RT_PRECISION_F32 : RT_PRECISION_F64, [&](auto& ds) -> int {
            using R = typename std::decay_t<decltype(ds)>::Real;
            const std::pair<const void*, size_t> tables[7] = {
                {ds.view.nodes, cs.nodes.size() * sizeof(BvhNode<R>)},        {ds.view.nodes4, cs.nodes4.size() * sizeof(BvhNode4f)},
                {ds.view.nodes4q, cs.nodes4.size() * sizeof(MeshNode4qc)},    {ds.view.tris, cs.tris.size() * sizeof(TriRec<R>)},
                {ds.view.attrs, cs.attrs.size() * sizeof(TriAttr<R>)},        {ds.view.mesh_bounds, cs.mesh_bounds.size() * sizeof(Bounds<R>)},
                {ds.view.mesh_op_recs, cs.mesh_ops.size() * sizeof(MeshOpRec<R>)}};
            for (int k = 0; k < 7; k++)
                if (int st = digest_of(tables[k].first, tables[k].second, &out[k])) return st;
            return RT_OK;
        }))
        return st;
    out[7] = s->generation;
    return RT_OK;
}

int rt_scene_info(const RtSceneDesc* desc, uint32_t* flags_out) {
    using namespace rt;
    if (!desc || !flags_out) return set_err(RT_E_INVALID, "rt_scene_info: NULL argument");
    CompiledScene cs;
    std::string err;
    int st = compile_scene(desc, &cs, &err, CompileOptions());
    if (st != RT_OK) return set_err(st, err);
    *flags_out = (cs.zero_weight_stop ? RT_SCENE_INFO_ZERO_WEIGHT_STOP : 0u) | (cs.needs_tex_interpreter ? RT_SCENE_INFO_TEX_INTERPRETER : 0u) |
                 (cs.volumes.empty() ? 0u : RT_SCENE_INFO_VOLUMES);
    return RT_OK;
}

int rt_scene_mesh_stats(const RtSceneDesc* desc, uint64_t out[8]) {
    using namespace rt;
    if (!desc || !out) return set_err(RT_E_INVALID, "rt_scene_mesh_stats: NULL argument");
    CompiledScene cs;
    std::string err;
    const CompileOptions opt = compile_options_from_env();
    int st = compile_scene(desc, &cs, &err, opt);
    if (st != RT_OK) return set_err(st, err);
    out[0] = cs.tris.size();
    out[1] = cs.nodes.size();
    out[2] = cs.nodes4.size();
    out[3] = cs.max_bvh_depth;
    out[4] = cs.max_bvh4_stack;
    out[5] = cs.ops.size();
    out[6] = cs.n_rebuilt_groups;
    out[7] = cs.n_rebuilt_prims;
    return RT_OK;
}

int rt_debug_handout_replay(const uint32_t* policy, uint32_t n, uint32_t waves, const uint32_t* order, uint32_t n_order, uint32_t* asks_out,
                            uint32_t capacity, uint32_t* n_asks_out, uint32_t* atomics_out) {
    using namespace rt;
    if (!order || !n_asks_out || !atomics_out || (!asks_out && capacity)) return set_err(RT_E_INVALID, "rt_debug_handout_replay: NULL argument");
    if (waves == 0u || waves > 65536u || n_order == 0u) return set_err(RT_E_INVALID, "rt_debug_handout_replay: 1..65536 waves and a non-empty order");
    std::vector<uint8_t> seen(waves, 0);
    for (uint32_t i = 0; i < n_order; i++) {
        if (order[i] >= waves) return set_err(RT_E_INVALID, "rt_debug_handout_replay: wave index out of range");
        seen[order[i]] = 1;
    }
    for (uint32_t g = 0; g < waves; g++)
        if (!seen[g]) return set_err(RT_E_INVALID, "rt_debug_handout_replay: every wave must appear in the order");
    HandoutPolicy hp{2u, kHandoutLeft256, kHandoutLeft128};
    if (policy) hp = HandoutPolicy{policy[0], policy[1], policy[2]};
    struct Wave { uint32_t end = 0; uint8_t state = 0; };
    std::vector<Wave> ws(waves);
    const uint32_t s0 = handout_first(hp, n, waves), start = waves * s0;
    uint32_t cursor = 0, n_asks = 0, open = waves;
    atomics_out[0] = atomics_out[1] = 0;
    auto record = [&](uint32_t g, uint32_t base, uint32_t end) {
        if (n_asks < capacity) { asks_out[3 * size_t(n_asks)] = g; asks_out[3 * size_t(n_asks) + 1] = base; asks_out[3 * size_t(n_asks) + 2] = end; }
        n_asks++;
    };
    for (uint32_t i = 0; open != 0u; i = (i + 1u) % n_order) {
        const uint32_t g = order[i];
        Wave& w = ws[g];
        if (w.state == 3) continue;
        if (w.state == 0) {
            uint32_t cur = 0;
            handout_static(n, s0, g, &cur, &w.end);
            w.state = 1;
            if (cur < w.end) { record(g, cur, w.end); continue; }
        }
        uint32_t base = 0, end = 0;
        uint32_t& atomics = atomics_out[w.state == 2 ? 1 : 0];
        const bool got = handout_next(hp, n, waves, start, w.end, [&](uint32_t size) { atomics++; const uint32_t old = cursor; cursor += size; return old; }, &base, &end);
        if (got) { w.end = end; record(g, base, end); }
        else record(g, 0xFFFFFFFFu, 0xFFFFFFFFu);
        if (w.state == 2) { w.state = 3; open--; }
        else if (!got) w.state = 2;
    }
    *n_asks_out = n_asks;
    return RT_OK;
}

int rt_scene_mesh_cones(const RtSceneDesc* desc, uint32_t mesh, uint32_t f32, int32_t* children_out, uint32_t* cones_out,
                        uint32_t node_capacity, uint32_t* n_nodes_out, double* tris_out, uint32_t tri_capacity, uint32_t* n_tris_out) {
    using namespace rt;
    if (!desc || !n_nodes_out || !n_tris_out) return set_err(RT_E_INVALID, "rt_scene_mesh_cones: NULL argument");
    CompiledScene cs;
    std::string err;
    int st = compile_scene(desc, &cs, &err, CompileOptions());
    if (st != RT_OK) return set_err(st, err);
    if (mesh >= cs.meshes.size()) return set_err(RT_E_INVALID, "rt_scene_mesh_cones: mesh index out of range");
    const MeshInst& mi = cs.meshes[mesh];
    size_t node_end = cs.nodes4.size();
    for (const MeshInst& o : cs.meshes)
        if (o.node4_base > mi.node4_base) node_end = std::min(node_end, size_t(o.node4_base));
    const size_t n_nodes = node_end - mi.node4_base;
    *n_nodes_out = uint32_t(n_nodes);
    *n_tris_out = mi.n_tris;
    if (children_out && cones_out) {
        std::vector<uint32_t> words;
        build_mesh_cones(cs.nodes4, cs.tris, cone_limits(f32 != 0), &words);
        for (size_t i = 0; i < n_nodes && i < node_capacity; i++)
            for (int k = 0; k < 4; k++) {
                int32_t ch = cs.nodes4[mi.node4_base + i].child[k];
                if (ch != kEmptyChild) {
                    if (ch >= 0) ch -= int32_t(mi.node4_base);
                    else {
                        const uint32_t code = uint32_t(~ch);
                        ch = ~int32_t((((code >> 3) - mi.tri_base) << 3) | (code & 7u));
                    }
                }
                children_out[4 * i + size_t(k)] = ch;
                cones_out[4 * i + size_t(k)] = words[4 * (mi.node4_base + i) + size_t(k)];
            }
    }
    if (tris_out)
        for (size_t t = 0; t < mi.n_tris && t < tri_capacity; t++) {
            const TriRec<double>& r = cs.tris[mi.tri_base + t];
            for (int a = 0; a < 3; a++) { tris_out[9 * t + size_t(a)] = r.v0[a]; tris_out[9 * t + 3 + size_t(a)] = r.e1[a]; tris_out[9 * t + 6 + size_t(a)] = r.e2[a]; }
        }
    return RT_OK;
}

int rt_scene_program(const RtSceneDesc* desc, int32_t* ops_out, uint32_t capacity, uint32_t* n_ops_out, uint64_t info[8]) {
    using namespace rt;
    if (!desc || !n_ops_out || !info) return set_err(RT_E_INVALID, "rt_scene_program: NULL argument");
    CompiledScene cs;
    std::string err;
    const CompileOptions opt = compile_options_from_env();
    int st = compile_scene(desc, &cs, &err, opt);
    if (st != RT_OK) return set_err(st, err);
    *n_ops_out = uint32_t(cs.ops.size());
    if (ops_out)
        for (size_t i = 0; i < cs.ops.size() && i < capacity; i++) {
            ops_out[4 * i + 0] = cs.ops[i].type; ops_out[4 * i + 1] = cs.ops[i].arg;
            ops_out[4 * i + 2] = cs.ops[i].skip; ops_out[4 * i + 3] = cs.ops[i].chain;
        }
    const WavefrontPlan plan = plan_wavefront(cs);
    info[0] = cs.mesh_ops.size();
    info[1] = cs.groups.size();
    info[2] = cs.group_nodes4.size();
    info[3] = cs.max_group_stack;
    info[4] = cs.lights.size();
    info[5] = cs.volumes.size();
    info[6] = (plan.split ? 1u : 0u) | (plan.vol_prims ? 2u : 0u) | (plan.multi_mesh ? 4u : 0u) | (plan.groups ? 8u : 0u);
    info[7] = cs.group_prims.size();
    return RT_OK;
}

int rt_accum_create(const RtScene* scene, const RtCameraDesc* camera, const RtRenderParams* params, RtAccum** out) {
    using namespace rt;
    if (!out) return set_err(RT_E_INVALID, "rt_accum_create: out is NULL");
    *out = nullptr;
    if (!scene || !camera || !params) return set_err(RT_E_INVALID, "rt_accum_create: NULL argument");
    if (int v = validate_render_args(camera, params)) return v;
    const uint32_t owned = owned_rows(camera->image_height, params);
    if (owned == 0) return set_err(RT_E_INVALID, "rt_accum_create: the row partition gives this part no rows");
    std::unique_ptr<RtAccum> a(new (std::nothrow) RtAccum);
    if (!a) return set_err(RT_E_NOMEM, "out of memory");
    a->scene = const_cast<RtScene*>(scene);
    a->generation = scene->generation;
    a->device = scene->device;
    a->camera = *camera;
    a->params = *params;
    a->owned = owned;
    a->T = params->thread_count;
    a->frame_digest = frame_digest(*camera, *params);
    HIP_TRY(hipSetDevice(scene->device));
    if (int st = a->d_sum.reserve(a->n_doubles() * sizeof(double))) return st;
    HIP_TRY(hipMemset(a->d_sum, 0, a->n_doubles() * sizeof(double)));
    HIP_TRY(hipDeviceSynchronize());
    *out = a.release();
    return RT_OK;
}

void rt_accum_destroy(RtAccum* acc) { delete acc; }

static int adaptive_compact(RtAccum* a, const uint32_t* src, uint32_t n_src, hipStream_t st) {
    using namespace rt;
    const uint32_t n_blocks = (n_src + AD_CHUNK - 1) / AD_CHUNK;
    hipLaunchKernelGGL(k_ad_scan, dim3(1), dim3(64), 0, st, a->d_block.get(), n_blocks, a->d_n_out.get());
    hipLaunchKernelGGL(k_ad_scatter, dim3(n_blocks), dim3(256), 0, st, src, n_src, a->d_keep.get(), a->d_block.get(), a->d_active[a->cur ^ 1].get(), a->d_state.get());
    HIP_TRY(hipGetLastError());
    uint32_t n_new = 0;
    HIP_TRY(hipMemcpyAsync(&n_new, a->d_n_out, 4, hipMemcpyDeviceToHost, st));
    HIP_TRY(hipStreamSynchronize(st));
    if (n_new > n_src) return set_err(RT_E_DEVICE, "adaptive compaction returned more pixels than it was given");
    a->cur ^= 1;
    a->n_active = n_new;
    return RT_OK;
}

static int adaptive_decide(RtAccum* a, hipStream_t st) {
    using namespace rt;
    if (a->n_active == 0) return RT_OK;
    const uint32_t n = a->n_active, n_blocks = (n + AD_CHUNK - 1) / AD_CHUNK;
    const uint32_t* list = a->d_active[a->cur];
    hipLaunchKernelGGL(k_ad_quiet, dim3((n + 255) / 256), dim3(256), 0, st, list, n, a->d_s1.get(), a->d_s2.get(), a->k, a->ap.threshold, a->ap.floor, a->d_state.get());
    hipLaunchKernelGGL(k_ad_window, dim3(n_blocks), dim3(256), 0, st, list, n, a->d_state.get(), a->camera.image_width, a->owned, int(a->ap.radius), a->d_keep.get(), a->d_block.get());
    return adaptive_compact(a, list, n, st);
}

static int adaptive_rebuild(RtAccum* a, hipStream_t st) {
    using namespace rt;
    const uint32_t n = uint32_t(a->npix()), n_blocks = (n + AD_CHUNK - 1) / AD_CHUNK;
    hipLaunchKernelGGL(k_ad_flags_from_counts, dim3(n_blocks), dim3(256), 0, st, a->d_cnt.get(), n, a->k, a->d_active[a->cur].get(), a->d_keep.get(), a->d_state.get(), a->d_block.get());
    if (int r = adaptive_compact(a, a->d_active[a->cur], n, st)) return r;
    if (a->decision_point(a->k)) return adaptive_decide(a, st);
    return RT_OK;
}

static void stats_add(RtRenderStats& total, const RtRenderStats& part, bool first) {
    if (first) { total = part; return; }
    total.kernel_ms += part.kernel_ms; total.traversal_kernel_ms += part.traversal_kernel_ms;
    total.prims_kernel_ms += part.prims_kernel_ms; total.shade_kernel_ms += part.shade_kernel_ms;
    total.n_launches += part.n_launches; total.n_iterations += part.n_iterations; total.samples += part.samples;
    total.n_replica_groups += part.n_replica_groups; total.n_tail_compactions += part.n_tail_compactions;
}

static int accum_render_adaptive(RtAccum* acc, uint32_t n_replicas, RtRenderParams p, void* stream) {
    using namespace rt;
    if (p.pipeline == RT_PIPELINE_MEGAKERNEL) return set_err(RT_E_UNSUPPORTED, "rt_accum_render: adaptive passes run the wavefront scheduler, RT_PIPELINE_MEGAKERNEL is not supported");
    if (p.collect_stats) return set_err(RT_E_UNSUPPORTED, "rt_accum_render: collect_stats is not supported on an adaptive accumulator");
    p.pipeline = RT_PIPELINE_WAVEFRONT;
    RtScene* s = acc->scene;
    HIP_TRY(hipSetDevice(acc->device));
    hipStream_t st = stream ? static_cast<hipStream_t>(stream) : s->stream;
    uint32_t left = std::min(n_replicas, acc->T - acc->k);
    RtRenderStats total{};
    bool first = true;
    int32_t* const flag = s->tail_flag;
    s->tail_flag = nullptr;
    int r = RT_OK;
    while (left > 0 && acc->n_active > 0) {
        uint32_t next = acc->T;
        if (acc->k < acc->ap.min_replicas) next = std::min(acc->T, acc->ap.min_replicas);
        else if (acc->k < acc->T) next = uint32_t(std::min<uint64_t>(acc->T, uint64_t(acc->k) + acc->ap.check_interval - (acc->k - acc->ap.min_replicas) % acc->ap.check_interval));
        const uint32_t m = std::min(left, next - acc->k);
        AdaptivePass ad;
        ad.active = acc->d_active[acc->cur];
        ad.n_active = acc->n_active;
        ad.sparse = acc->n_active < acc->npix();
        ad.s1 = acc->d_s1; ad.s2 = acc->d_s2; ad.cnt = acc->d_cnt;
        r = render_device_impl(s, &acc->camera, &p, acc->k, m, acc->d_sum, st, &ad);
        if (r != RT_OK) break;
        stats_add(total, s->stats, first);
        first = false;
        acc->k += m;
        left -= m;
        if (acc->decision_point(acc->k) && (r = adaptive_decide(acc, st)) != RT_OK) break;
    }
    s->tail_flag = flag;
    if (!first) s->stats = total;
    else if (r == RT_OK) { s->stats = RtRenderStats{}; s->stats.pipeline_used = RT_PIPELINE_WAVEFRONT; }
    return r;
}

static int accum_render_impl(RtAccum* acc, uint32_t n_replicas, const RtRenderParams* params_or_null, void* stream) {
    using namespace rt;
    if (!acc) return set_err(RT_E_INVALID, "rt_accum_render: NULL accumulator");
    if (accum_is_stale(acc)) return accum_stale_error();
    RtRenderParams p = acc->params;
    if (params_or_null) {
        const RtRenderParams a = frame_fields(acc->params), b = frame_fields(*params_or_null);
        if (std::memcmp(&a, &b, sizeof a) != 0)
            return set_err(RT_E_INVALID, "rt_accum_render: params differ from the accumulator's in more than pipeline / collect_stats");
        p.pipeline = params_or_null->pipeline;
        p.collect_stats = params_or_null->collect_stats;
    }
    if (acc->adaptive) return accum_render_adaptive(acc, n_replicas, p, stream);
    const uint32_t n = std::min(n_replicas, acc->T - acc->k);
    if (n == 0) return RT_OK;
    const int r = render_device_impl(acc->scene, &acc->camera, &p, acc->k, n, acc->d_sum, stream);
    if (r == RT_OK) acc->k += n;
    return r;
}
// ... 644 lines not shown
```

### rust_raytracer_amd/csrc/rt_refit.h

```cpp
#pragma once
#include <cmath>
#include <cstdint>
#include <cstring>
#include <limits>
#include <string>
#include <vector>

#include "../../include/rt_mi355.h"
#include "rt_bvh.h"
#include "rt_scene.h"

#if defined(__HIP__)
#include <hip/hip_runtime.h>

#include "rt_owned.h"
#define RT_HD __host__ __device__
#else
#define RT_HD
#endif

namespace rt {

RT_HD inline double rf_min(double a, double b) { return b < a ? b : a; }
RT_HD inline double rf_max(double a, double b) { return b > a ? b : a; }
// ... 6 lines not shown
    else b -= 1u;
    memcpy(&f, &b, 4);
    return f;
}
RT_HD inline float rf_float_above(float f) {
    uint32_t b;
    memcpy(&b, &f, 4);
    if ((b << 1) == 0u) b = 0x00000001u;
    else if (b >> 31) b -= 1u;
    else b += 1u;
    memcpy(&f, &b, 4);
    return f;
}

template <typename R> RT_HD inline R round_down(double x);
template <typename R> RT_HD inline R round_up(double x);
template <> RT_HD inline double round_down<double>(double x) { return x; }
template <> RT_HD inline double round_up<double>(double x) { return x; }
template <> RT_HD inline float round_down<float>(double x) {
    float f = float(x);
    if (double(f) > x) f = rf_float_below(f);
    return f;
}
template <> RT_HD inline float round_up<float>(double x) {
    float f = float(x);
    if (double(f) < x) f = rf_float_above(f);
    return f;
}

template <typename R> RT_HD inline void rf_pad_box2(double lo, double hi, R* olo, R* ohi) {
    if (!(lo <= hi)) { *olo = R(lo); *ohi = R(hi); return; }
    const double m = std::fmax(std::fabs(lo), std::fabs(hi));
    const double e = 8.0 * double(std::numeric_limits<R>::epsilon()) * std::fmax(m, hi - lo);
    *olo = round_down<R>(lo - e);
    *ohi = round_up<R>(hi + e);
}

RT_HD inline double rf_pad_of_box(const double* lo, const double* hi) {
    double S = 0.0;
    for (int a = 0; a < 3; a++) S = std::fmax(S, std::fmax(std::fabs(lo[a]), std::fabs(hi[a])));
    if (!std::isfinite(S)) S = 0.0;
    return S * (1.0 / 524288.0);
}

RT_HD inline void rf_pad_box4f(double lo, double hi, double m, float* olo, float* ohi) {
    if (!(lo <= hi)) { *olo = INFINITY; *ohi = -INFINITY; }
    else { *olo = round_down<float>(lo - m); *ohi = round_up<float>(hi + m); }
}

RT_HD inline bool rf_quantise4(const double (*lo)[3], const double (*hi)[3], const int32_t* child, double m, float* org_out, float* cell_out,
                               uint32_t* qlo, uint32_t* qhi) {
    for (int a = 0; a < 3; a++) {
        double flo[4], fhi[4];
        bool real[4];
        double lo_min = INFINITY, hi_max = -INFINITY;
        for (int k = 0; k < 4; k++) {
            real[k] = child[k] != kEmptyChild && lo[k][a] <= hi[k][a];
            if (!real[k]) continue;
            flo[k] = double(round_down<float>(lo[k][a] - m));
            fhi[k] = double(round_up<float>(hi[k][a] + m));
            lo_min = std::fmin(lo_min, flo[k]);
            hi_max = std::fmax(hi_max, fhi[k]);
        }
        const bool any = lo_min <= hi_max && std::isfinite(lo_min) && std::isfinite(hi_max);
        const double org = any ? lo_min : 0.0;
        const double ext = any ? hi_max - org : 0.0;
        int e = -100;
        if (ext > 0.0) {
            (void)std::frexp(ext / 255.0, &e);
            while (ext / std::ldexp(1.0, e) > 255.0) e++;
            while (e > -100 && ext / std::ldexp(1.0, e - 1) <= 255.0) e--;
            e = e < -100 ? -100 : (e > 120 ? 120 : e);
        }
        const double cell = std::ldexp(1.0, e);
        org_out[a] = float(org);
        cell_out[a] = float(cell);
        qlo[a] = 0;
        qhi[a] = 0;
        for (int k = 0; k < 4; k++) {
            uint32_t ql = 255u, qh = 0u;
            if (any && real[k]) {
                const double l = std::floor((flo[k] - org) / cell), h = std::ceil((fhi[k] - org) / cell);
                const double lc = 255.0 < l ? 255.0 : l, hc = 255.0 < h ? 255.0 : h;
                ql = uint32_t(0.0 < lc ? lc : 0.0);
                qh = uint32_t(0.0 < hc ? hc : 0.0);
                if (!(org + ql * cell <= flo[k] && org + qh * cell >= fhi[k])) return false;
            }
            qlo[a] |= ql << (8 * k);
            qhi[a] |= qh << (8 * k);
        }
    }
    return true;
}

constexpr double kConeDirSlack = 0.00682;
constexpr double kConeSafety = 0.001;
constexpr double kConeMinCos = 0.125;

RT_HD inline void rf_tri_normal(const double* v0, const double* a, const double* b, const ConeLimits& lim, double* out) {
    const double cx = a[1] * b[2] - a[2] * b[1], cy = a[2] * b[0] - a[0] * b[2], cz = a[0] * b[1] - a[1] * b[0];
    const double la = std::sqrt(a[0] * a[0] + a[1] * a[1] + a[2] * a[2]), lb = std::sqrt(b[0] * b[0] + b[1] * b[1] + b[2] * b[2]);
    const double lc = std::sqrt(cx * cx + cy * cy + cz * cz);
    bool ok = std::isfinite(v0[0]) && std::isfinite(v0[1]) && std::isfinite(v0[2]);
    ok = ok && la >= lim.min_edge && la <= lim.max_edge && lb >= lim.min_edge && lb <= lim.max_edge;
    ok = ok && lc >= lim.sigma * la * lb && lc > 0.0;
    const double kNaN = std::numeric_limits<double>::quiet_NaN();
    out[0] = ok ? cx / lc : kNaN;
    out[1] = ok ? cy / lc : kNaN;
    out[2] = ok ? cz / lc : kNaN;
}

RT_HD inline uint32_t rf_cone_around(const double* normal, uint32_t lo, uint32_t hi, const double* axis) {
    const double l = std::sqrt(axis[0] * axis[0] + axis[1] * axis[1] + axis[2] * axis[2]);
    if (!(l > 0.0) || !std::isfinite(l)) return kNeutralCone;
    int q[3];
    double al = 0.0;
    for (int a = 0; a < 3; a++) { q[a] = int(std::lround(127.0 * axis[a] / l)); al += double(q[a]) * double(q[a]); }
    al = std::sqrt(al);
    if (!(al > 0.0)) return kNeutralCone;
    const double ax = q[0] / al, ay = q[1] / al, az = q[2] / al;
    double c = 1.0;
    for (uint32_t t = lo; t < hi; t++) {
        const double d = ax * normal[3 * size_t(t)] + ay * normal[3 * size_t(t) + 1] + az * normal[3 * size_t(t) + 2];
        c = d < c ? d : c;
        if (c < kConeMinCos) return kNeutralCone;
    }
    if (!(c >= kConeMinCos)) return kNeutralCone;
    const double s = std::sqrt(std::fmax(0.0, 1.0 - c * c));
    const double w = std::ceil(al * (s + kConeDirSlack + kConeSafety));
    if (!(w >= 1.0 && w <= 127.0)) return kNeutralCone;
    return uint32_t(q[0] & 0xFF) | (uint32_t(q[1] & 0xFF) << 8) | (uint32_t(q[2] & 0xFF) << 16) | (uint32_t(w) << 24);
}

RT_HD inline uint32_t rf_cone_word(const double* normal, uint32_t lo, uint32_t hi, uint32_t count, const double* sum) {
    if (count == 0 || hi - lo != count) return kNeutralCone;
    uint32_t word = rf_cone_around(normal, lo, hi, sum);
    if (word == kNeutralCone && count >= 2 && count <= 8 && std::isfinite(sum[0])) {
        uint32_t bi = lo, bj = lo;
        double least = 2.0;
        for (uint32_t i = lo; i < hi; i++)
            for (uint32_t j = i + 1; j < hi; j++) {
                const double* ni = &normal[3 * size_t(i)];
                const double* nj = &normal[3 * size_t(j)];
                const double dij = ni[0] * nj[0] + ni[1] * nj[1] + ni[2] * nj[2];
                if (dij < least) { least = dij; bi = i; bj = j; }
            }
        const double mid[3] = {normal[3 * size_t(bi)] + normal[3 * size_t(bj)], normal[3 * size_t(bi) + 1] + normal[3 * size_t(bj) + 1],
                               normal[3 * size_t(bi) + 2] + normal[3 * size_t(bj) + 2]};
        word = rf_cone_around(normal, lo, hi, mid);
    }
    return word;
}

#if defined(__HIP__)
struct RefitMesh {
    uint32_t n_tris = 0, n_nodes = 0, n_nodes4 = 0, n_positions = 0, n_normals = 0, n_uvs = 0;
    DevBuf<uint32_t> tri_order, tri_pos, tri_nrm;
    DevBuf<int32_t> tri_uv;
    DevBuf<int32_t> child2, child4;
    DevBuf<int32_t> parent2, parent4;
    DevBuf<uint32_t> inner2, inner4;
    DevBuf<uint32_t> arrived2, arrived4;
    DevBuf<double> positions, normals, uvs;
    DevBuf<double> tri_box, tri_normal;
    DevBuf<double> box2, box4;
    DevBuf<double> sum4;
    DevBuf<uint32_t> run4;
};

template <typename R>
struct RefitTarget {
    BvhNode<R>* nodes;
    BvhNode4f* nodes4;
    MeshNode4qc* nodes4q;
    TriRec<R>* tris;
    TriAttr<R>* attrs;
    double pad4;
};

bool refit_mesh_upload(RefitMesh& rm, const RtMesh& m, const uint32_t* tri_order, const int32_t* child2, uint32_t n_nodes, const int32_t* child4,
                       uint32_t n_nodes4, hipStream_t stream, uint64_t* bytes, std::string* err);
template <typename R> bool refit_mesh_launch(RefitMesh& rm, const RefitTarget<R>& t, hipStream_t stream, std::string* err);
#endif

}
```

### rust_raytracer_amd/csrc/rt_refit.hip

```cpp
#include "rt_refit.h"

#include <algorithm>

namespace rt {
namespace {

#define REFIT_TRY(expr)                                                                 \
    do {                                                                                \
        hipError_t e_ = (expr);                                                         \
        if (e_ != hipSuccess) {                                                         \
            *err = std::string("scene refit: ") + hipGetErrorString(e_) + " at " #expr; \
            return false;                                                               \
        }                                                                               \
    } while (0)

template <typename R>
__global__ void k_refit_tris(uint32_t n, const uint32_t* __restrict__ tri_order, const uint32_t* __restrict__ tri_pos,
                             const uint32_t* __restrict__ tri_nrm, const int32_t* __restrict__ tri_uv, const double* __restrict__ positions,
                             const double* __restrict__ normals, const double* __restrict__ uvs, ConeLimits lim, TriRec<R>* __restrict__ tris,
                             TriAttr<R>* __restrict__ attrs, double* __restrict__ tri_box, double* __restrict__ tri_normal) {
    const uint32_t slot = blockIdx.x * blockDim.x + threadIdx.x;
    if (slot >= n) return;
    const size_t t = tri_order[slot];
    const double* p0 = positions + 3 * size_t(tri_pos[3 * t]);
    const double* p1 = positions + 3 * size_t(tri_pos[3 * t + 1]);
    const double* p2 = positions + 3 * size_t(tri_pos[3 * t + 2]);
    double v0[3], e1[3], e2[3];
    for (int a = 0; a < 3; a++) {
        v0[a] = p0[a];
        e1[a] = p1[a] - p0[a];
        e2[a] = p2[a] - p0[a];
        tri_box[6 * size_t(slot) + a] = rf_min(p0[a], rf_min(p1[a], p2[a]));
        tri_box[6 * size_t(slot) + 3 + a] = rf_max(p0[a], rf_max(p1[a], p2[a]));
    }
    TriRec<R>& r = tris[slot];
    for (int a = 0; a < 3; a++) { r.v0[a] = R(v0[a]); r.e1[a] = R(e1[a]); r.e2[a] = R(e2[a]); }
    rf_tri_normal(v0, e1, e2, lim, tri_normal + 3 * size_t(slot));
    TriAttr<R>& at = attrs[slot];
    const double* n0 = normals + 3 * size_t(tri_nrm[3 * t]);
    const double* n1 = normals + 3 * size_t(tri_nrm[3 * t + 1]);
    const double* n2 = normals + 3 * size_t(tri_nrm[3 * t + 2]);
    for (int a = 0; a < 3; a++) { at.n0[a] = R(n0[a]); at.n1[a] = R(n1[a]); at.n2[a] = R(n2[a]); }
    const bool has_uv = tri_uv && tri_uv[3 * t] >= 0 && tri_uv[3 * t + 1] >= 0 && tri_uv[3 * t + 2] >= 0;
    if (has_uv) {
        const double* a0 = uvs + 3 * size_t(tri_uv[3 * t]);
        const double* a1 = uvs + 3 * size_t(tri_uv[3 * t + 1]);
        const double* a2 = uvs + 3 * size_t(tri_uv[3 * t + 2]);
        at.uv0[0] = R(a0[0]); at.uv0[1] = R(a0[1]);
        at.uv1[0] = R(a1[0]); at.uv1[1] = R(a1[1]);
        at.uv2[0] = R(a2[0]); at.uv2[1] = R(a2[1]);
    }
}

template <int W>
__global__ void k_refit_parents(uint32_t n_nodes, const int32_t* __restrict__ child, int32_t* __restrict__ parent, uint32_t* __restrict__ inner) {
    const uint32_t i = blockIdx.x * blockDim.x + threadIdx.x;
    if (i >= n_nodes) return;
    uint32_t cnt = 0;
    for (int k = 0; k < W; k++) {
        const int32_t c = child[W * size_t(i) + k];
        if (c >= 0 && uint32_t(c) < n_nodes) { parent[c] = int32_t(i); cnt++; }
    }
    inner[i] = cnt;
    if (i == 0) parent[0] = -1;
}

template <int W>
__device__ inline void refit_node(uint32_t i, uint32_t n_nodes, uint32_t n_tris, const int32_t* __restrict__ child, const double* __restrict__ tri_box,
                                  const double* __restrict__ tri_normal, double* box, double* sum, uint32_t* run) {
    for (int k = 0; k < W; k++) {
        const int32_t c = child[W * size_t(i) + k];
        double lo[3] = {INFINITY, INFINITY, INFINITY}, hi[3] = {-INFINITY, -INFINITY, -INFINITY};
        double s[3] = {0.0, 0.0, 0.0};
        uint32_t rlo = UINT32_MAX, rhi = 0, cnt = 0;
        if (c != kEmptyChild && c < 0) {
            const uint32_t code = uint32_t(~c), first = code >> 3, count = (code & 7u) + 1u;
            if (first + count <= n_tris) {
                rlo = first; rhi = first + count; cnt = count;
                for (uint32_t t = first; t < first + count; t++) {
                    for (int a = 0; a < 3; a++) {
                        lo[a] = rf_min(lo[a], tri_box[6 * size_t(t) + a]);
                        hi[a] = rf_max(hi[a], tri_box[6 * size_t(t) + 3 + a]);
                        if (W == 4) s[a] += tri_normal[3 * size_t(t) + a];
                    }
                }
            }
        } else if (c != kEmptyChild && uint32_t(c) < n_nodes) {
            const volatile double* cb = box + 6 * W * size_t(c);
            const volatile double* cs = sum + 3 * W * size_t(c);
            const volatile uint32_t* cr = run + 3 * W * size_t(c);
            for (int j = 0; j < W; j++) {
                if (child[W * size_t(c) + j] == kEmptyChild) continue;
                for (int a = 0; a < 3; a++) {
                    lo[a] = rf_min(lo[a], cb[6 * j + a]);
                    hi[a] = rf_max(hi[a], cb[6 * j + 3 + a]);
                }
                if (W == 4) {
                    rlo = min(rlo, cr[3 * j]); rhi = max(rhi, cr[3 * j + 1]); cnt += cr[3 * j + 2];
                    for (int a = 0; a < 3; a++) s[a] += cs[3 * j + a];
                }
            }
        }
        for (int a = 0; a < 3; a++) {
            box[6 * (W * size_t(i) + k) + a] = lo[a];
            box[6 * (W * size_t(i) + k) + 3 + a] = hi[a];
        }
        if (W == 4) {
            for (int a = 0; a < 3; a++) sum[3 * (W * size_t(i) + k) + a] = s[a];
            run[3 * (W * size_t(i) + k)] = rlo; run[3 * (W * size_t(i) + k) + 1] = rhi; run[3 * (W * size_t(i) + k) + 2] = cnt;
        }
    }
}

template <int W>
__global__ void k_refit_up(uint32_t n_nodes, uint32_t n_tris, const int32_t* __restrict__ child, const int32_t* __restrict__ parent,
                           const uint32_t* __restrict__ inner, unsigned int* __restrict__ arrived, const double* __restrict__ tri_box,
                           const double* __restrict__ tri_normal, double* box, double* sum, uint32_t* run) {
    const uint32_t first = blockIdx.x * blockDim.x + threadIdx.x;
    if (first >= n_nodes || inner[first] != 0u) return;
    int32_t node = int32_t(first);
    for (uint32_t guard = 0; guard <= n_nodes; guard++) {
        refit_node<W>(uint32_t(node), n_nodes, n_tris, child, tri_box, tri_normal, box, sum, run);
        __threadfence();
        const int32_t up = parent[node];
        if (up < 0 || uint32_t(up) >= n_nodes) return;
        if (atomicAdd(&arrived[up], 1u) + 1u < inner[up]) return;
        __threadfence();
        node = up;
    }
}

template <typename R>
__global__ void k_refit_nodes2(uint32_t n_nodes, const double* __restrict__ box, BvhNode<R>* __restrict__ nodes) {
    const uint32_t i = blockIdx.x * blockDim.x + threadIdx.x;
    if (i >= n_nodes) return;
    BvhNode<R>& n = nodes[i];
    const double* b0 = box + 12 * size_t(i);
    const double* b1 = b0 + 6;
    for (int a = 0; a < 3; a++) {
        rf_pad_box2<R>(b0[a], b0[3 + a], &n.lo0[a], &n.hi0[a]);
        rf_pad_box2<R>(b1[a], b1[3 + a], &n.lo1[a], &n.hi1[a]);
    }
}

__global__ void k_refit_nodes4(uint32_t n_nodes, double pad, const int32_t* __restrict__ child, const double* __restrict__ box,
                               const double* __restrict__ sum, const uint32_t* __restrict__ run, const double* __restrict__ tri_normal,
                               BvhNode4f* __restrict__ nodes4, MeshNode4qc* __restrict__ nodes4q) {
    const uint32_t i = blockIdx.x * blockDim.x + threadIdx.x;
    if (i >= n_nodes) return;
    double lo[4][3], hi[4][3];
    int32_t ch[4];
    for (int k = 0; k < 4; k++) {
        ch[k] = child[4 * size_t(i) + k];
        for (int a = 0; a < 3; a++) { lo[k][a] = box[6 * (4 * size_t(i) + k) + a]; hi[k][a] = box[6 * (4 * size_t(i) + k) + 3 + a]; }
    }
    BvhNode4f& f = nodes4[i];
    for (int k = 0; k < 4; k++) {
        rf_pad_box4f(lo[k][0], hi[k][0], pad, &f.lox[k], &f.hix[k]);
        rf_pad_box4f(lo[k][1], hi[k][1], pad, &f.loy[k], &f.hiy[k]);
        rf_pad_box4f(lo[k][2], hi[k][2], pad, &f.loz[k], &f.hiz[k]);
    }
    float org[3], cell[3];
    uint32_t qlo[3], qhi[3];
    MeshNode4qc& q = nodes4q[i];
    if (rf_quantise4(lo, hi, ch, pad, org, cell, qlo, qhi))
        for (int a = 0; a < 3; a++) { q.node.org[a] = org[a]; q.node.cell[a] = cell[a]; q.node.qlo[a] = qlo[a]; q.node.qhi[a] = qhi[a]; }
    for (int k = 0; k < 4; k++) {
        uint32_t word = kNeutralCone;
        if (ch[k] != kEmptyChild) {
            const uint32_t* r = run + 3 * (4 * size_t(i) + k);
            word = rf_cone_word(tri_normal, r[0], r[1], r[2], sum + 3 * (4 * size_t(i) + k));
        }
        q.cones.word[k] = word;
    }
}

template <typename T>
bool dev_alloc(DevBuf<T>& p, size_t n, std::string* err) {
    if (p.reserve(std::max<size_t>(n, 1) * sizeof(T)) == RT_OK) return true;
    *err = "scene refit: " + g_err;
    return false;
}
template <typename T>
bool dev_put(DevBuf<T>& dst, const T* src, size_t n, hipStream_t stream, uint64_t* bytes, std::string* err) {
    if (n) REFIT_TRY(hipMemcpyAsync(dst, src, n * sizeof(T), hipMemcpyHostToDevice, stream));
    *bytes += n * sizeof(T);
    return true;
}

inline dim3 grid_for(uint32_t n) { return dim3((n + 255u) / 256u); }

}

bool refit_mesh_upload(RefitMesh& rm, const RtMesh& m, const uint32_t* tri_order, const int32_t* child2, uint32_t n_nodes, const int32_t* child4,
                       uint32_t n_nodes4, hipStream_t stream, uint64_t* bytes, std::string* err) {
    if (!rm.tri_order) {
        RefitMesh r;
        r.n_tris = m.n_triangles; r.n_nodes = n_nodes; r.n_nodes4 = n_nodes4;
        r.n_positions = m.n_positions; r.n_normals = m.n_normals; r.n_uvs = m.uvs && m.tri_uv ? m.n_uvs : 0;
        const size_t nt = r.n_tris;
        bool ok = dev_alloc(r.tri_order, nt, err) && dev_alloc(r.tri_pos, 3 * nt, err) && dev_alloc(r.tri_nrm, 3 * nt, err) &&
                  (!m.tri_uv || dev_alloc(r.tri_uv, 3 * nt, err)) && dev_alloc(r.child2, 2 * size_t(n_nodes), err) &&
                  dev_alloc(r.child4, 4 * size_t(n_nodes4), err) && dev_alloc(r.parent2, n_nodes, err) && dev_alloc(r.parent4, n_nodes4, err) &&
                  dev_alloc(r.inner2, n_nodes, err) && dev_alloc(r.inner4, n_nodes4, err) && dev_alloc(r.arrived2, n_nodes, err) &&
                  dev_alloc(r.arrived4, n_nodes4, err) && dev_alloc(r.positions, 3 * size_t(r.n_positions), err) &&
                  dev_alloc(r.normals, 3 * size_t(r.n_normals), err) && (!r.n_uvs || dev_alloc(r.uvs, 3 * size_t(r.n_uvs), err)) &&
                  dev_alloc(r.tri_box, 6 * nt, err) && dev_alloc(r.tri_normal, 3 * nt, err) && dev_alloc(r.box2, 12 * size_t(n_nodes), err) &&
                  dev_alloc(r.box4, 24 * size_t(n_nodes4), err) && dev_alloc(r.sum4, 12 * size_t(n_nodes4), err) &&
                  dev_alloc(r.run4, 12 * size_t(n_nodes4), err);
        ok = ok && dev_put(r.tri_order, tri_order, nt, stream, bytes, err) && dev_put(r.tri_pos, m.tri_pos, 3 * nt, stream, bytes, err) &&
             dev_put(r.tri_nrm, m.tri_nrm, 3 * nt, stream, bytes, err) && (!m.tri_uv || dev_put(r.tri_uv, m.tri_uv, 3 * nt, stream, bytes, err)) &&
             dev_put(r.child2, child2, 2 * size_t(n_nodes), stream, bytes, err) && dev_put(r.child4, child4, 4 * size_t(n_nodes4), stream, bytes, err);
        if (!ok) return false;
        hipLaunchKernelGGL(k_refit_parents<2>, grid_for(n_nodes), dim3(256), 0, stream, n_nodes, r.child2.get(), r.parent2.get(), r.inner2.get());
        hipLaunchKernelGGL(k_refit_parents<4>, grid_for(n_nodes4), dim3(256), 0, stream, n_nodes4, r.child4.get(), r.parent4.get(), r.inner4.get());
        hipError_t e = hipGetLastError();
        if (e == hipSuccess) e = hipStreamSynchronize(stream);
        if (e != hipSuccess) { *err = std::string("scene refit: ") + hipGetErrorString(e); return false; }
        rm = std::move(r);
    }
    if (rm.n_tris != m.n_triangles || rm.n_positions != m.n_positions || rm.n_normals != m.n_normals || rm.n_nodes != n_nodes || rm.n_nodes4 != n_nodes4) {
        *err = "scene refit: the mesh has another structure than at its first update";
        return false;
    }
    return dev_put(rm.positions, m.positions, 3 * size_t(rm.n_positions), stream, bytes, err) &&
           dev_put(rm.normals, m.normals, 3 * size_t(rm.n_normals), stream, bytes, err) &&
           (!rm.n_uvs || dev_put(rm.uvs, m.uvs, 3 * size_t(rm.n_uvs), stream, bytes, err));
}

template <typename R>
bool refit_mesh_launch(RefitMesh& rm, const RefitTarget<R>& t, hipStream_t stream, std::string* err) {
    if (rm.n_tris == 0) return true;
    const dim3 block(256);
    REFIT_TRY(hipMemsetAsync(rm.arrived2, 0, size_t(rm.n_nodes) * sizeof(uint32_t), stream));
    REFIT_TRY(hipMemsetAsync(rm.arrived4, 0, size_t(rm.n_nodes4) * sizeof(uint32_t), stream));
    hipLaunchKernelGGL((k_refit_tris<R>), grid_for(rm.n_tris), block, 0, stream, rm.n_tris, rm.tri_order.get(), rm.tri_pos.get(), rm.tri_nrm.get(), rm.uvs ? rm.tri_uv.get() : nullptr,
                       rm.positions.get(), rm.normals.get(), rm.uvs.get(), cone_limits(sizeof(R) == 4), t.tris, t.attrs, rm.tri_box.get(), rm.tri_normal.get());
    hipLaunchKernelGGL((k_refit_up<2>), grid_for(rm.n_nodes), block, 0, stream, rm.n_nodes, rm.n_tris, rm.child2.get(), rm.parent2.get(), rm.inner2.get(), rm.arrived2.get(),
                       rm.tri_box.get(), rm.tri_normal.get(), rm.box2.get(), static_cast<double*>(nullptr), static_cast<uint32_t*>(nullptr));
    hipLaunchKernelGGL((k_refit_up<4>), grid_for(rm.n_nodes4), block, 0, stream, rm.n_nodes4, rm.n_tris, rm.child4.get(), rm.parent4.get(), rm.inner4.get(), rm.arrived4.get(),
                       rm.tri_box.get(), rm.tri_normal.get(), rm.box4.get(), rm.sum4.get(), rm.run4.get());
    hipLaunchKernelGGL((k_refit_nodes2<R>), grid_for(rm.n_nodes), block, 0, stream, rm.n_nodes, rm.box2.get(), t.nodes);
    hipLaunchKernelGGL(k_refit_nodes4, grid_for(rm.n_nodes4), block, 0, stream, rm.n_nodes4, t.pad4, rm.child4.get(), rm.box4.get(), rm.sum4.get(), rm.run4.get(),
                       rm.tri_normal.get(), t.nodes4, t.nodes4q);
    REFIT_TRY(hipGetLastError());
    return true;
}
template bool refit_mesh_launch<float>(RefitMesh&, const RefitTarget<float>&, hipStream_t, std::string*);
template bool refit_mesh_launch<double>(RefitMesh&, const RefitTarget<double>&, hipStream_t, std::string*);

}
```

### rust_raytracer_amd/csrc/rt_scene.h

```cpp
#pragma once
#include <cstdint>

namespace rt {

enum OpType : int32_t {
    OP_END = 0,
    OP_BOUNDS = 1,
    OP_XFORM_PUSH = 2,
    OP_XFORM_POP = 3,
    OP_SPHERE = 4,
    OP_PLANE = 5,
    OP_MESH = 6,
    OP_SKY = 7,
    OP_SUN = 8,
    OP_VOL_BEGIN = 9,
    OP_VOL_MID = 10,
    OP_VOL_END = 11,
    OP_GROUP = 12,
};

struct Op {
    int32_t type;
    int32_t arg;
    int32_t skip;
    int32_t chain;
};

template <typename R>
struct Bounds {
    R lo[3], hi[3];
};

template <typename R>
struct Xform {
    R m[12];
    R inv[12];
};

template <typename R>
struct SpherePrim {
    R center[3];
    R radius;
    int32_t material;
    int32_t _pad;
};

template <typename R>
struct PlanePrim {
    R corner[3], normal[3], u[3], v[3], inv_u[3], inv_v[3];
    R area;
    int32_t material;
    int32_t backface;
};

template <typename R>
struct SunPrim {
    R direction[3];
    int32_t material;
    int32_t _pad;
};

template <typename R>
struct VolumeRec {
    R neg_inv_density;
    int32_t material;
    int32_t _pad;
};

template <typename R>
struct GroupRec {
    uint32_t root;
    uint32_t _pad[3];
    R lo[3], hi[3];
};
struct GroupPrimRef {
    int32_t pc;
    int32_t guard_first;
    int32_t guard_count;
    int32_t _pad;
};

struct MeshInst {
    uint32_t node_base;
    uint32_t tri_base;
    int32_t material;
    uint32_t flags;
    uint32_t n_tris;
    uint32_t max_depth;
    uint32_t node4_base;
    uint32_t _pad;
};
constexpr uint32_t MESH_HAS_UV = 0x100u;

template <typename R>
struct alignas(16) MeshOpRec {
    int32_t pc;
    int32_t chain;
    uint32_t node4_base;
    uint32_t flags;
    R lo[3], hi[3];
    R inv[12];
};


constexpr int32_t kEmptyChild = INT32_MIN;
template <typename R>
struct alignas(sizeof(R) == 8 ? 128 : 64) BvhNode {
    R lo0[3], hi0[3], lo1[3], hi1[3];
    int32_t c0, c1;
};

struct alignas(128) BvhNode4f {
    float lox[4], loy[4], loz[4], hix[4], hiy[4], hiz[4];
    int32_t child[4];
    uint32_t _pad[4];
};

struct alignas(64) BvhNode4q {
    float org[3];
    float cell[3];
    uint32_t qlo[3];
    uint32_t qhi[3];
    int32_t child[4];
};
static_assert(sizeof(BvhNode4q) == 64, "BvhNode4q must be 64 bytes");

struct alignas(16) NodeCones4 {
    uint32_t word[4];
};
struct alignas(128) MeshNode4qc {
    BvhNode4q node;
    NodeCones4 cones;
    uint32_t _pad[12];
};
static_assert(sizeof(MeshNode4qc) == 128, "one cache line per mesh node");
constexpr uint32_t kNeutralCone = 0x7F000000u;
constexpr uint32_t kNoCullDir = 0x81000000u;

template <typename R>
struct alignas(16) TriRec {
    R v0[3], e1[3], e2[3];
    R _pad;
};
template <typename R>
struct alignas(16) TriAttr {
    R n0[3], n1[3], n2[3];
    R uv0[2], uv1[2], uv2[2];
    int32_t has_uv;
    int32_t _pad;
};

struct MaterialRec {
    int32_t type;
    int32_t tex_a, tex_b, tex_c;
    int32_t needs_uv;
    int32_t has_normal_map;
};
template <typename R>
struct MaterialParams {
    R ior;
    R inv_ior;
    R inv_ior_r;
    R r0_glossy;
    R r0_front;
    R r0_back;
};

template <typename R>
struct TextureRec {
    int32_t type;
    int32_t aux;
    uint32_t data;
    uint32_t width, height;
    int32_t _pad;
    R v[3];
    R scale;
};
constexpr int kMaxVolDepth = 2;
constexpr int kTexStackDepth = 4;
constexpr int kTexStackMax = 16;
constexpr int32_t kTexProgShift = 20;

enum LightKind : int32_t { LIGHT_OTHER = 0, LIGHT_PLANE = 1, LIGHT_SPHERE = 2, LIGHT_SKY = 3, LIGHT_SUN = 4, LIGHT_LIST = 5 };
struct LightRec {
    int32_t kind;
    int32_t index;
};
constexpr int32_t kLightListShift = 20;
constexpr int kMaxLightDepth = 8;

enum SmallTable : int {
    ST_OPS, ST_BOUNDS, ST_CHAIN_OFFSETS, ST_CHAIN_ITEMS, ST_XFORMS, ST_SPHERES, ST_PLANES, ST_SUNS, ST_MESHES, ST_MATERIALS,
    ST_MATERIAL_PARAMS, ST_TEXTURES, ST_LIGHTS, ST_COUNT
};
struct SmallLayout {
    uint32_t begin[ST_COUNT], end[ST_COUNT];
    uint32_t total_bytes;
};

template <typename R>
struct SceneView {
    const Op* ops;
    const Bounds<R>* bounds;
    const int32_t* chain_offsets;
    const int32_t* chain_items;
    const Xform<R>* xforms;
    const SpherePrim<R>* spheres;
    const PlanePrim<R>* planes;
    const SunPrim<R>* suns;
    const MeshInst* meshes;
    const VolumeRec<R>* volumes;
    const BvhNode<R>* nodes;
    const BvhNode4f* nodes4;
    const MeshNode4qc* nodes4q;
    const Bounds<R>* mesh_bounds;
    const int32_t* mesh_ops;
    const MeshOpRec<R>* mesh_op_recs;
    int32_t n_mesh_ops;
    const GroupRec<R>* groups;
    const BvhNode4q* group_nodes;
    const GroupPrimRef* group_prims;
    const int32_t* group_guards;
    int32_t n_group_nodes;
    int32_t group_stack_levels;
    const TriRec<R>* tris;
    const TriAttr<R>* attrs;
    const MaterialRec* materials;
    const MaterialParams<R>* material_params;
    const TextureRec<R>* textures;
    const float* texels;
    const R* perlin_vec;
    const uint32_t* perlin_perm;
    const LightRec* lights;
    int32_t n_lights;
    R inv_n_lights;
    int32_t lights_is_list;
    int32_t stop_on_zero_weight;
    int32_t stack_entries;
    int32_t n_ops;
    const char* small_blob;
    SmallLayout lay;
    const char* small_blob_shade;
    SmallLayout lay_shade;
};

template <typename R>
struct CameraView {
    R position[3], first_pixel[3], pdu[3], pdv[3], basis_u[3], basis_v[3];
    R aperture_radius;
    R inv_sqrt_spt;
    int32_t has_aperture;
    uint32_t width, height;
    uint32_t sqrt_spt, thread_count, max_depth;
};

template <typename R>
struct ParamsView {
    R light_bias;
    R background[3];
    uint64_t seed;
    uint32_t band_rows, n_parts, part;
    uint32_t owned_rows;
    double inv_spp;
    double spp;
};

struct DeviceCounters {
    unsigned long long rays, mesh_rays, node_visits, tri_tests, prim_tests;
    unsigned long long node_wave_iters, tri_wave_iters, refill_wave_iters, refill_lanes, pops_culled;
};

}
```

### rust_raytracer_amd/csrc/rt_traverse.h

```cpp
#pragma once

namespace rt {

template <typename R> RT_DEV V3<R> clamped_inv(const Ray<R>& ray) {
    const R big = sizeof(R) == 8 ? R(1e150) : R(1e18);
    return {fabs(ray.inv.x) > big ? copysign(big, ray.inv.x) : ray.inv.x,
            fabs(ray.inv.y) > big ? copysign(big, ray.inv.y) : ray.inv.y,
            fabs(ray.inv.z) > big ? copysign(big, ray.inv.z) : ray.inv.z};
}

template <typename R> RT_DEV bool tri_test(const TriRec<R>& tr, V3<R> o, V3<R> d, bool hit_back, R& t, R& u, R& v) {
    V3<R> edge1 = ld3(tr.e1), edge2 = ld3(tr.e2);
    V3<R> ray_x_edge2 = cross(d, edge2);
    R det = dot(edge1, ray_x_edge2);
    R dd = hit_back ? fabs(det) : det;
    if (!(dd < Lim<R>::det_eps())) {
        R inv_det = R(1) / det;
        V3<R> b = o - ld3(tr.v0);
        R uu = dot(b, ray_x_edge2) * inv_det;
        if (!(uu < R(0) || uu > R(1))) {
            V3<R> b_x_edge1 = cross(b, edge1);
            R vv = dot(d, b_x_edge1) * inv_det;
            if (!(vv < R(0) || uu + vv > R(1))) {
                t = dot(edge2, b_x_edge1) * inv_det;
                u = uu;
                v = vv;
                return true;
            }
        }
    }
    return false;
}

template <typename R> RT_DEV bool node2_step(const BvhNode<R>& n, V3<R> inv, V3<R> oi, R t_lo, R t_max, int32_t& first, int32_t& second) {
    R t0x = n.lo0[0] * inv.x - oi.x, t1x = n.hi0[0] * inv.x - oi.x;
    R t0y = n.lo0[1] * inv.y - oi.y, t1y = n.hi0[1] * inv.y - oi.y;
    R t0z = n.lo0[2] * inv.z - oi.z, t1z = n.hi0[2] * inv.z - oi.z;
    R near0 = fmax(fmax(fmin(t0x, t1x), fmin(t0y, t1y)), fmax(fmin(t0z, t1z), t_lo));
    R far0 = fmin(fmin(fmax(t0x, t1x), fmax(t0y, t1y)), fmin(fmax(t0z, t1z), t_max));
    R s0x = n.lo1[0] * inv.x - oi.x, s1x = n.hi1[0] * inv.x - oi.x;
    R s0y = n.lo1[1] * inv.y - oi.y, s1y = n.hi1[1] * inv.y - oi.y;
    R s0z = n.lo1[2] * inv.z - oi.z, s1z = n.hi1[2] * inv.z - oi.z;
    R near1 = fmax(fmax(fmin(s0x, s1x), fmin(s0y, s1y)), fmax(fmin(s0z, s1z), t_lo));
    R far1 = fmin(fmin(fmax(s0x, s1x), fmax(s0y, s1y)), fmin(fmax(s0z, s1z), t_max));
    int32_t c0 = n.c0, c1 = n.c1;
    bool h0 = (near0 <= far0) && c0 != kEmptyChild;
    bool h1 = (near1 <= far1) && c1 != kEmptyChild;
    second = kEmptyChild;
    if (h0 && h1) {
        bool first0 = near0 <= near1;
        second = first0 ? c1 : c0;
        first = first0 ? c0 : c1;
        return true;
    }
    if (h0) { first = c0; return true; }
    if (h1) { first = c1; return true; }
    return false;
}

template <typename R> RT_DEV float f32_at_least(R x) {
    float f = float(x);
    return f + fabsf(f) * 9.5367431640625e-7f + 1e-30f;
}

template <typename R>
struct CullRay {
    float ivx, ivy, ivz;
    float oix, oiy, oiz;
    R t_shift;
    RT_DEV bool negx() const { return ivx < 0.0f; }
    RT_DEV bool negy() const { return ivy < 0.0f; }
    RT_DEV bool negz() const { return ivz < 0.0f; }
};
template <typename R> RT_DEV CullRay<R> make_cull_ray(const Ray<R>& ray, const R* lo, const R* hi, R floor, R& t_enter, R& t_exit) {
    const V3<R> inv = clamped_inv(ray);
    const R e0x = (lo[0] - ray.o.x) * inv.x, e1x = (hi[0] - ray.o.x) * inv.x;
    const R e0y = (lo[1] - ray.o.y) * inv.y, e1y = (hi[1] - ray.o.y) * inv.y;
    const R e0z = (lo[2] - ray.o.z) * inv.z, e1z = (hi[2] - ray.o.z) * inv.z;
    t_enter = fmax(fmax(fmin(e0x, e1x), fmin(e0y, e1y)), fmax(fmin(e0z, e1z), floor));
    t_exit = fmin(fmin(fmax(e0x, e1x), fmax(e0y, e1y)), fmax(e0z, e1z));
    CullRay<R> cr;
    cr.t_shift = fabs(t_enter) < Lim<R>::inf() ? t_enter : R(0);
    const V3<R> oc = ray.o + ray.d * cr.t_shift;
    const float big32 = 1e18f;
    cr.ivx = 1.0f / float(ray.d.x); cr.ivy = 1.0f / float(ray.d.y); cr.ivz = 1.0f / float(ray.d.z);
    cr.ivx = fabsf(cr.ivx) > big32 ? copysignf(big32, cr.ivx) : cr.ivx;
    cr.ivy = fabsf(cr.ivy) > big32 ? copysignf(big32, cr.ivy) : cr.ivy;
    cr.ivz = fabsf(cr.ivz) > big32 ? copysignf(big32, cr.ivz) : cr.ivz;
    cr.oix = float(oc.x) * cr.ivx; cr.oiy = float(oc.y) * cr.ivy; cr.oiz = float(oc.z) * cr.ivz;
    return cr;
}
template <typename R> RT_DEV bool span_misses(R t_enter, R t_exit, R t_max) {
    const R eps = Lim<R>::eps() * R(16);
    return (t_enter - fabs(t_enter) * eps > t_exit + fabs(t_exit) * eps) || (t_enter - fabs(t_enter) * eps > t_max);
}

template <typename R> RT_DEV uint32_t quantise_dir(V3<R> d, bool cull_allowed) {
    const R len2 = d.x * d.x + d.y * d.y + d.z * d.z;
    const R len_lo = sizeof(R) == 8 ? R(1e-200) : R(1e-24), len_hi = sizeof(R) == 8 ? R(1e200) : R(1e24);
    uint32_t dirq = kNoCullDir;
    if (cull_allowed && len2 > len_lo && len2 < len_hi) {
        const R sc127 = R(127) / sqrt(len2);
        const int qx = int(rint(d.x * sc127)), qy = int(rint(d.y * sc127)), qz = int(rint(d.z * sc127));
        dirq = (uint32_t(qx) & 0xFFu) | ((uint32_t(qy) & 0xFFu) << 8) | ((uint32_t(qz) & 0xFFu) << 16) | kNoCullDir;
    }
    return dirq;
}

RT_DEV void node4q_cull_cones(uint32_t dirq, uint4 cn, int4 cc, int32_t (&ch)[4]) {
    ch[0] = __builtin_amdgcn_sdot4(int(dirq), int(cn.x), 0, false) > 0 ? kEmptyChild : cc.x;
    ch[1] = __builtin_amdgcn_sdot4(int(dirq), int(cn.y), 0, false) > 0 ? kEmptyChild : cc.y;
    ch[2] = __builtin_amdgcn_sdot4(int(dirq), int(cn.z), 0, false) > 0 ? kEmptyChild : cc.z;
    ch[3] = __builtin_amdgcn_sdot4(int(dirq), int(cn.w), 0, false) > 0 ? kEmptyChild : cc.w;
}

constexpr float kNoEntry = __builtin_huge_valf();

template <typename R>
RT_DEV uint32_t node4q_entries(uint4 h0, uint4 h1, uint4 h2, const CullRay<R>& cr, float tmax32, const int32_t (&ch)[4], float (&nr)[4]) {
    const float ax = __uint_as_float(h0.w) * cr.ivx, ay = __uint_as_float(h1.x) * cr.ivy, az = __uint_as_float(h1.y) * cr.ivz;
    const float bx = fmaf(__uint_as_float(h0.x), cr.ivx, -cr.oix), by = fmaf(__uint_as_float(h0.y), cr.ivy, -cr.oiy), bz = fmaf(__uint_as_float(h0.z), cr.ivz, -cr.oiz);
    const bool negx = cr.negx(), negy = cr.negy(), negz = cr.negz();
    const uint32_t qnx = negx ? h2.y : h1.z, qfx = negx ? h1.z : h2.y;
    const uint32_t qny = negy ? h2.z : h1.w, qfy = negy ? h1.w : h2.z;
    const uint32_t qnz = negz ? h2.w : h2.x, qfz = negz ? h2.x : h2.w;
    uint32_t entered = 0u;
#pragma unroll
    for (int k = 0; k < 4; k++) {
        const float nxk = float((qnx >> (8 * k)) & 0xFFu), nyk = float((qny >> (8 * k)) & 0xFFu), nzk = float((qnz >> (8 * k)) & 0xFFu);
        const float fxk = float((qfx >> (8 * k)) & 0xFFu), fyk = float((qfy >> (8 * k)) & 0xFFu), fzk = float((qfz >> (8 * k)) & 0xFFu);
        const float tn = fmaxf(fmaxf(fmaf(nxk, ax, bx), fmaf(nyk, ay, by)), fmaxf(fmaf(nzk, az, bz), 0.0f));
        const float tf = fminf(fminf(fmaf(fxk, ax, bx), fmaf(fyk, ay, by)), fminf(fmaf(fzk, az, bz), tmax32));
        const bool h = (tn <= tf) && ch[k] != kEmptyChild;
        nr[k] = h ? tn : kNoEntry;
        entered |= uint32_t(h) << k;
    }
    return entered;
}

#define RT_CE(nr, ch, a, b)                                           \
    if (nr[a] > nr[b]) {                                              \
        float tn_ = nr[a]; nr[a] = nr[b]; nr[b] = tn_;                \
        int32_t tc_ = ch[a]; ch[a] = ch[b]; ch[b] = tc_;              \
    }
#define RT_SORT4_NEAREST_FIRST(nr, ch) RT_CE(nr, ch, 0, 1) RT_CE(nr, ch, 2, 3) RT_CE(nr, ch, 0, 2) RT_CE(nr, ch, 1, 3) RT_CE(nr, ch, 1, 2)

}
```

### rust_raytracer_amd/csrc/rt_wavefront.h

```cpp
#pragma once
#include "rt_device.h"
#include "rt_handout.h"

#ifndef RT_ISECT_WAVES
#define RT_ISECT_WAVES 3
#endif
#ifndef RT_MESH_WAVES
#define RT_MESH_WAVES 4
#endif
namespace rt {

template <typename R>
struct WfPool {
    uint32_t capacity;
    R *ox, *oy, *oz, *dx, *dy, *dz;
    R *tr, *tg, *tb;
    uint64_t* rng;
    uint64_t* sample;
    uint32_t* depth;
    R *ht, *hu, *hv;
    int32_t *hpc, *htri;
};

template <typename T> RT_DEV T& at(T* base, uint32_t slot) {
// ... 494 lines not shown
                if (STATS) cnt.prim_tests++;
                if (sphere_test<R, true>(sc.spheres[op.arg], cur, t_lo, best.t, t) && hit_takes_over(sc, t, op, best)) { best.t = t; best.pc = pc; }
                break;
            }
            case OP_PLANE: {
                R t, u, v;
                if (STATS) cnt.prim_tests++;
                if (plane_test<R, true>(sc.planes[op.arg], cur, t_lo, best.t, t, u, v) && hit_takes_over(sc, t, op, best)) { best.t = t; best.pc = pc; best.u = u; best.v = v; }
                break;
            }
            case OP_MESH: {
                const Bounds<R>& rb = sc.mesh_bounds[op.arg];
                const V3<R> inv = clamped_inv(cur);
                const R eps = Lim<R>::eps() * R(16);
                R t0x = (rb.lo[0] - fabs(rb.lo[0]) * eps - cur.o.x) * inv.x, t1x = (rb.hi[0] + fabs(rb.hi[0]) * eps - cur.o.x) * inv.x;
                R t0y = (rb.lo[1] - fabs(rb.lo[1]) * eps - cur.o.y) * inv.y, t1y = (rb.hi[1] + fabs(rb.hi[1]) * eps - cur.o.y) * inv.y;
                R t0z = (rb.lo[2] - fabs(rb.lo[2]) * eps - cur.o.z) * inv.z, t1z = (rb.hi[2] + fabs(rb.hi[2]) * eps - cur.o.z) * inv.z;
                R tn = fmax(fmax(fmin(t0x, t1x), fmin(t0y, t1y)), fmax(fmin(t0z, t1z), t_lo));
                R tf = fmin(fmin(fmax(t0x, t1x), fmax(t0y, t1y)), fmin(fmax(t0z, t1z), best.t));
                tf = tf + fabs(tf) * eps;
                to_mesh = to_mesh || ((tn <= tf) && rb.lo[0] <= rb.hi[0]);
                break;
            }
            case OP_SKY:
                if (STATS) cnt.prim_tests++;
                if (!(Lim<R>::inf() > best.t)) { best.t = Lim<R>::inf(); best.pc = pc; }
                break;
            case OP_SUN: {
                if (STATS) cnt.prim_tests++;
                const SunPrim<R>& s = sc.suns[op.arg];
                V3<R> unit_dir = to_unit(cur.d);
                if (!(fabs(dot(ld3(s.direction), unit_dir) - R(1)) > R(0.001)) && !(Lim<R>::max() >= best.t)) {
                    best.t = Lim<R>::max();
                    best.pc = pc;
                }
                break;
            }
            default: break;
        }
        pc++;
    }
    return to_mesh;
}

#ifndef RT_PRIMS_WAVES
#define RT_PRIMS_WAVES 5
#endif
template <typename R, bool STATS, int LDS, bool VOL, bool GROUPS>
__global__ void __launch_bounds__(256, VOL ? 2 : (GROUPS ? 3 : RT_PRIMS_WAVES)) k_wf_prims(SceneView<R> sc_g, WfPool<R> pool, const uint32_t* __restrict__ queue,
                                                  uint32_t* __restrict__ mesh_queue, WfCounters* __restrict__ ctr,
                                                  DeviceCounters* counters, uint32_t staged, uint32_t group_levels) {
    extern __shared__ __align__(16) char lds_raw[];
    uint32_t* mesh_list = reinterpret_cast<uint32_t*>(lds_raw);
    uint32_t* lc = mesh_list + WF_CHUNK;
    char* tables = reinterpret_cast<char*>(lc + 4);
    GroupCtx gc{};
    if constexpr (GROUPS) {
        gc.stack = (LdsU64*)(reinterpret_cast<unsigned long long*>(tables) + threadIdx.x);
        tables += size_t(group_levels) * 256 * 8;
        uint4* dst = reinterpret_cast<uint4*>(tables);
        const uint4* src = reinterpret_cast<const uint4*>(sc_g.group_nodes);
        const uint32_t n16 = uint32_t(sc_g.n_group_nodes) * uint32_t(sizeof(BvhNode4q) / 16);
        for (uint32_t i = threadIdx.x; i < n16; i += blockDim.x) dst[i] = src[i];
        gc.nodes = reinterpret_cast<const BvhNode4q*>(dst);
        tables += size_t(n16) * 16;
    }
    if (threadIdx.x < 4) lc[threadIdx.x] = 0;
    SceneView<R> sc = sc_g;
    if constexpr (LDS == 1) sc = scene_tables_to_lds<R, true>(sc_g, sc_g.lay, sc_g.small_blob, tables, staged);
    else if constexpr (LDS == 2) sc = scene_tables_to_lds<R, false>(sc_g, sc_g.lay, sc_g.small_blob, tables, staged);
    else __syncthreads();
    const uint32_t n = ctr->n_in;
    const bool full = n == pool.capacity;
    const uint32_t begin = blockIdx.x * WF_CHUNK;
    const uint32_t end = min(n, begin + WF_CHUNK);
    LaneCounters cnt;
    for (uint32_t base = begin; base < end; base += blockDim.x) {
        const uint32_t i = base + threadIdx.x;
        bool to_mesh = false;
        uint32_t slot = 0;
        if (i < end) {
            slot = full ? i : queue[i];
            const Ray<R> wray = make_ray(mk<R>(at(pool.ox, slot), at(pool.oy, slot), at(pool.oz, slot)), mk<R>(at(pool.dx, slot), at(pool.dy, slot), at(pool.dz, slot)));
            Best<R> best;
            if constexpr (VOL) {
                Rng rng;
                rng.s = at(pool.rng, slot);
                to_mesh = prims_search<R, STATS, true, false>(sc, wray, best, cnt, &rng);
                at(pool.rng, slot) = rng.s;
            } else {
                to_mesh = prims_search<R, STATS, false, GROUPS>(sc, wray, best, cnt, nullptr, &gc);
            }
            at(pool.ht, slot) = best.t; at(pool.hu, slot) = best.u; at(pool.hv, slot) = best.v;
            at(pool.hpc, slot) = best.pc; at(pool.htri, slot) = best.tri;
        }
        lds_append(to_mesh, slot, mesh_list, &lc[0]);
    }
    __syncthreads();
    const uint32_t n_list = lc[0];
    if (threadIdx.x == 0 && n_list) lc[1] = atomicAdd(&ctr->n_mesh, n_list);
    __syncthreads();
    const uint32_t qb = lc[1];
    for (uint32_t j = threadIdx.x; j < n_list; j += blockDim.x) mesh_queue[qb + j] = mesh_list[j];
    if (STATS) {
        uint32_t rays = cnt.rays, prims = cnt.prim_tests;
        for (int off = 32; off > 0; off >>= 1) { rays += __shfl_down(rays, off); prims += __shfl_down(prims, off); }
        if ((threadIdx.x & 63u) == 0 && rays) {
            atomicAdd(&counters->rays, (unsigned long long)rays);
            atomicAdd(&counters->prim_tests, (unsigned long long)prims);
        }
    }
}

typedef __attribute__((address_space(3))) char LdsByte;
struct MeshStack {
    static constexpr int32_t kLevel = 256 * int32_t(sizeof(uint2));
    static constexpr int kLevelShift = 11;
    static_assert(kLevel == 1 << kLevelShift, "a level is one entry per lane of the workgroup");
    LdsByte* lds;
    uint2* spill;
    int32_t empty;
    uint32_t spill_stride;
    RT_DEV static unsigned long long pack(int32_t child, float dist) { return (static_cast<unsigned long long>(__float_as_uint(dist)) << 32) | uint32_t(child); }
    RT_DEV LdsU64& at(int32_t addr) const { return *(LdsU64*)(lds + addr); }
    RT_DEV void put(int32_t& top, int32_t child, float dist) const {
        if (top >= kLevel) at(top - kLevel) = pack(child, dist);
        else spill[size_t(uint32_t(-(top >> kLevelShift))) * spill_stride] = make_uint2(uint32_t(child), __float_as_uint(dist));
        top -= kLevel;
    }
    RT_DEV uint2 get(int32_t& top) const {
        uint2 r;
        if (top >= 0) {
            unsigned long long e = at(top);
            r = make_uint2(uint32_t(e), uint32_t(e >> 32));
        } else {
            r = spill[size_t(uint32_t(-(top >> kLevelShift)) - 1u) * spill_stride];
        }
        top += kLevel;
        return r;
    }
    RT_DEV void push3(int32_t& top, const int32_t* ch, const float* nr, float no_entry) const {
        top -= kLevel * (1 + int32_t(nr[2] < no_entry) + int32_t(nr[3] < no_entry));
        at(top) = pack(ch[1], nr[1]);
        if (nr[2] < no_entry) {
            at(top + kLevel) = pack(ch[2], nr[2]);
            if (nr[3] < no_entry) at(top + 2 * kLevel) = pack(ch[3], nr[3]);
        }
    }
};

template <typename R> constexpr uint32_t kMeshStage = sizeof(R) == 8 ? kHandoutMax : 0u;
template <typename R> constexpr uint32_t kMeshWaveLds = 1024u + 3u * 64u * uint32_t(sizeof(R)) + 4u * kMeshStage<R>;

template <typename R, bool STATS, int NODE, bool MULTI>
__global__ void __launch_bounds__(256, (sizeof(R) == 4 && !STATS && NODE == 1) ? 5 : RT_MESH_WAVES) k_wf_mesh(SceneView<R> sc, WfPool<R> pool, const uint32_t* __restrict__ mesh_queue,
                                                                 WfCounters* __restrict__ ctr, DeviceCounters* counters,
                                                                 uint32_t refill_min, uint32_t inner_min,
                                                                 uint2* __restrict__ spill, int lds_levels,
                                                                 const uint32_t* __restrict__ n_ptr, uint32_t* __restrict__ cursor_ptr,
                                                                 uint32_t cones_on, uint32_t handout_mode, uint32_t handout_256, uint32_t handout_128) {
    const HandoutPolicy handout{handout_mode, handout_256, handout_128};
    extern __shared__ uint2 lds_stack2[];
    MeshStack stk;
    stk.lds = (LdsByte*)lds_stack2;
    const uint32_t lane = threadIdx.x & 63u;
    char* wave_area = reinterpret_cast<char*>(lds_stack2 + size_t(lds_levels) * 256) + (threadIdx.x >> 6) * kMeshWaveLds<R>;
    uint16_t* pair_tbl = reinterpret_cast<uint16_t*>(wave_area);
    R* res_t = reinterpret_cast<R*>(wave_area + 1024);
    R* res_u = res_t + 64;
    R* res_v = res_u + 64;
    uint32_t* stage = reinterpret_cast<uint32_t*>(res_v + 64);
    stk.spill = spill + (size_t(blockIdx.x) * blockDim.x + threadIdx.x);
    stk.empty = lds_levels * MeshStack::kLevel;
    stk.spill_stride = gridDim.x * blockDim.x;
    const uint32_t n = *n_ptr;
    const R t_lo = R(0.001);
    const BvhNode4f* nodes = sc.nodes4;
    const MeshNode4qc* nodesq = sc.nodes4q;
    const TriRec<R>* tris = sc.tris;
    const uint32_t n_mesh_ops = uint32_t(sc.n_mesh_ops);
    const MeshOpRec<R>* mrecs = sc.mesh_op_recs;
    auto load_rec = [&](uint32_t m, MeshOpRec<R>& rb) {
        const auto* rec = as_const_mem(mrecs) + m;
        rb.pc = rec->pc; rb.chain = rec->chain; rb.node4_base = rec->node4_base; rb.flags = rec->flags;
#pragma unroll
        for (int a = 0; a < 3; a++) { rb.lo[a] = rec->lo[a]; rb.hi[a] = rec->hi[a]; }
#pragma unroll
        for (int k = 0; k < 12; k++) rb.inv[k] = rec->inv[k];
    };
    MeshOpRec<R> rb0;
    if constexpr (!MULTI) load_rec(0u, rb0);
    LaneCounters cnt;
    uint32_t w_node = 0, w_tri = 0, w_refill = 0, l_refill = 0, l_culled = 0;
    bool has = false;
    bool pending = false;
    bool exhausted = false;
    WaveRange range;
    range.init(handout, n);
    uint32_t slot = 0;
    uint32_t mcur = 0;
    V3<R> o{}, d{};
    R t_max = R(0), hit_u = R(0), hit_v = R(0);
    int32_t hit_tri = -1;
    CullRay<R> cr{};
    float tmax32 = 0.f;
    int32_t node = 0;
    int32_t top = 0;
    uint32_t dirq = kNoCullDir;

    auto finish_path = [&]() {
        if constexpr (MULTI) {
            const uint32_t hm = (mcur >> 15) & 0x7FFFu;
            if (hm != 0u) {
                at(pool.ht, slot) = t_max; at(pool.hu, slot) = hit_u; at(pool.hv, slot) = hit_v;
                at(pool.hpc, slot) = sc.mesh_ops[hm - 1u]; at(pool.htri, slot) = hit_tri;
            }
        } else {
            if (hit_tri >= 0) {
                at(pool.ht, slot) = t_max; at(pool.hu, slot) = hit_u; at(pool.hv, slot) = hit_v;
                at(pool.hpc, slot) = rb0.pc; at(pool.htri, slot) = hit_tri;
            }
        }
    };
    auto pop_lds = [&]() -> bool {
        while (top < stk.empty) {
            const unsigned long long e = stk.at(top);
            top += MeshStack::kLevel;
            if (__uint_as_float(uint32_t(e >> 32)) <= tmax32) {
                node = int32_t(uint32_t(e));
                return true;
            }
            if (STATS) l_culled++;
        }
        return false;
    };
    auto pop_any = [&]() -> bool {
        while (top < stk.empty) {
            const uint2 e = stk.get(top);
            if (__uint_as_float(e.y) <= tmax32) {
                node = int32_t(e.x);
                return true;
            }
            if (STATS) l_culled++;
        }
        return false;
    };
    auto pop_next = [&]() {
        const bool found_entry = __ballot(top < 0) == 0ull ? pop_lds() : pop_any();
        if (!found_entry) {
            has = false;
            if constexpr (MULTI) {
                mcur = (mcur & 0x7FFFFFFFu) + 1u;
                if ((mcur & 0x7FFFu) < n_mesh_ops) pending = true;
                else finish_path();
            } else {
                finish_path();
            }
        }
    };
    auto enter_mesh = [&](const MeshOpRec<R>& rb) -> bool {
        const int32_t mpc = rb.pc;
        Ray<R> wray = make_ray(mk<R>(at(pool.ox, slot), at(pool.oy, slot), at(pool.oz, slot)), mk<R>(at(pool.dx, slot), at(pool.dy, slot), at(pool.dz, slot)));
        Ray<R> ray;
        const uint32_t n_chain = rb.flags >> 16;
        if (n_chain == 0u) ray = wray;
        else if (n_chain == 1u) ray = make_ray(xform_apply(rb.inv, wray.o, R(1)), xform_apply(rb.inv, wray.d, R(0)));
        else ray = ray_in_chain_uniform(sc, wray, rb.chain);
        o = ray.o;
        d = ray.d;
        const R bound = at(pool.ht, slot);
        const int32_t bpc = at(pool.hpc, slot);
        const R excl = (bpc > mpc && bound < Lim<R>::inf()) ? nextafter(bound, Lim<R>::inf()) : bound;
        if constexpr (MULTI) t_max = ((mcur >> 15) & 0x7FFFu) != 0u ? fmin(t_max, excl) : excl;
        else t_max = excl;
        R t_enter, t_exit;
        cr = make_cull_ray(ray, rb.lo, rb.hi, R(0), t_enter, t_exit);
        if constexpr (MULTI) {
            if (span_misses(t_enter, t_exit, t_max) || !(rb.lo[0] <= rb.hi[0])) return false;
        }
        tmax32 = f32_at_least(t_max - cr.t_shift);
        node = int32_t(rb.node4_base);
        top = stk.empty + int32_t(threadIdx.x * uint32_t(sizeof(uint2)));
        if constexpr (NODE == 1) dirq = quantise_dir(d, cones_on != 0u && (rb.flags & RT_MESH_HIT_BACK_FACES) == 0u);
        return true;
    };

    for (;;) {
        if constexpr (MULTI) {
            const unsigned long long idle = __ballot(!has);
            const unsigned long long waiting = __ballot(pending);
            if ((uint32_t(__popcll(idle)) >= refill_min && (!exhausted || waiting != 0ull)) || (waiting != 0ull && idle == ~0ull)) {
                const unsigned long long want = __ballot(!has && !pending);
                if (!exhausted && want != 0ull) {
                    if (STATS) w_refill++;
                    if (wave_fetch_entry<kMeshStage<R>>(range, want, cursor_ptr, n, handout, exhausted, mesh_queue, stage, slot)) {
                        if (STATS) l_refill++;
                        mcur = 0;
                        hit_tri = -1;
                        pending = true;
                    }
                }
                for (;;) {
                    const unsigned long long pend = __ballot(pending);
                    if (pend == 0ull) break;
                    const uint32_t m = uint32_t(__builtin_amdgcn_readfirstlane(int(__shfl(int(mcur & 0x7FFFu), __ffsll((long long)pend) - 1))));
                    MeshOpRec<R> rb;
                    load_rec(m, rb);
                    if (pending && (mcur & 0x7FFFu) == m) {
                        if (!enter_mesh(rb)) {
                            mcur++;
                            if ((mcur & 0x7FFFu) >= n_mesh_ops) { pending = false; finish_path(); }
                        } else {
                            if (rb.flags & RT_MESH_HIT_BACK_FACES) mcur |= 0x80000000u;
                            has = true;
                            pending = false;
                            if (STATS) cnt.mesh_rays++;
                        }
                    }
                }
            }
            if (__ballot(has) == 0ull) {
                if (exhausted && __ballot(pending) == 0ull) break;
                continue;
            }
        } else {
            const unsigned long long idle = __ballot(!has);
            if (!exhausted && uint32_t(__popcll(idle)) >= refill_min) {
                if (STATS) w_refill++;
                if (wave_fetch_entry<kMeshStage<R>>(range, idle, cursor_ptr, n, handout, exhausted, mesh_queue, stage, slot)) {
                    if (STATS) l_refill++;
                    hit_tri = -1;
                    enter_mesh(rb0);
                    has = true;
                    if (STATS) cnt.mesh_rays++;
                }
            }
            if (__ballot(has) == 0ull) {
                if (exhausted) break;
                continue;
            }
        }
        for (;;) {
            unsigned long long inner = __ballot(has && node >= 0);
            if (inner == 0ull) break;
            if (uint32_t(__popcll(inner)) < inner_min && __ballot(has && node < 0) != 0ull) break;
            if (STATS) w_node++;
            if (has && node >= 0) {
                if (STATS) cnt.node_visits++;
                float nr[4];
                int32_t ch[4];
                if constexpr (NODE == 1) {
                    const uint4* nd = reinterpret_cast<const uint4*>(nodesq + node);
                    const uint4 h0 = nd[0], h1 = nd[1], h2 = nd[2];
                    const int4 cc = *reinterpret_cast<const int4*>(nd + 3);
                    node4q_cull_cones(dirq, nd[4], cc, ch);
                    node4q_entries(h0, h1, h2, cr, tmax32, ch, nr);
                } else {
                    const float4* nd = reinterpret_cast<const float4*>(nodes + node);
                    const uint32_t nearx = cr.negx() ? 3u : 0u, neary = cr.negy() ? 4u : 1u, nearz = cr.negz() ? 5u : 2u;
                    const float4 nx = nd[nearx], fx = nd[3u - nearx];
                    const float4 ny = nd[neary], fy = nd[5u - neary];
                    const float4 nz = nd[nearz], fz = nd[7u - nearz];
                    const int4 cc = *reinterpret_cast<const int4*>(nd + 6);
                    ch[0] = cc.x; ch[1] = cc.y; ch[2] = cc.z; ch[3] = cc.w;
                    const float nxa[4] = {nx.x, nx.y, nx.z, nx.w}, fxa[4] = {fx.x, fx.y, fx.z, fx.w};
                    const float nya[4] = {ny.x, ny.y, ny.z, ny.w}, fya[4] = {fy.x, fy.y, fy.z, fy.w};
                    const float nza[4] = {nz.x, nz.y, nz.z, nz.w}, fza[4] = {fz.x, fz.y, fz.z, fz.w};
#pragma unroll
                    for (int k = 0; k < 4; k++) {
                        float tn = fmaxf(fmaxf(fmaf(nxa[k], cr.ivx, -cr.oix), fmaf(nya[k], cr.ivy, -cr.oiy)), fmaxf(fmaf(nza[k], cr.ivz, -cr.oiz), 0.0f));
                        float tf = fminf(fminf(fmaf(fxa[k], cr.ivx, -cr.oix), fmaf(fya[k], cr.ivy, -cr.oiy)), fminf(fmaf(fza[k], cr.ivz, -cr.oiz), tmax32));
                        bool h = (tn <= tf) && ch[k] != kEmptyChild;
                        nr[k] = h ? tn : kNoEntry;
                    }
                }
                RT_SORT4_NEAREST_FIRST(nr, ch)
                if (nr[0] < kNoEntry) {
                    if (__ballot(top < 3 * MeshStack::kLevel) == 0ull) {
                        if (nr[1] < kNoEntry) stk.push3(top, ch, nr, kNoEntry);
                    } else {
                        if (nr[3] < kNoEntry) stk.put(top, ch[3], nr[3]);
                        if (nr[2] < kNoEntry) stk.put(top, ch[2], nr[2]);
                        if (nr[1] < kNoEntry) stk.put(top, ch[1], nr[1]);
                    }
                    node = ch[0];
                } else {
                    pop_next();
                }
            }
        }
        {
            const bool leaf = has && node < 0;
            const uint32_t code = uint32_t(~node);
            const uint32_t first = leaf ? (code >> 3) : 0u, count = leaf ? ((code & 7u) + 1u) : 0u;
            uint32_t pre = 0, total = 0;
#pragma unroll
            for (int bit = 0; bit < 4; bit++) {
                unsigned long long m = __ballot(((count >> bit) & 1u) != 0u);
                pre += lane_prefix(m) << bit;
                total += uint32_t(__popcll(m)) << bit;
            }
            if (total != 0u) {
                for (uint32_t j = 0; j < 8u; j++) {
                    if (__ballot(j < count) == 0ull) break;
                    if (j < count) pair_tbl[pre + j] = uint16_t(lane | (j << 8));
                }
                __builtin_amdgcn_wave_barrier();
                for (uint32_t c0 = 0; c0 < total; c0 += 64u) {
                    if (STATS) w_tri++;
                    const uint32_t w = c0 + lane;
                    const bool act = w < total;
                    const uint32_t e = act ? uint32_t(pair_tbl[w]) : 0u;
                    const int owner = int(e & 0xFFu);
                    const uint32_t k = e >> 8;
                    const V3<R> po = {__shfl(o.x, owner), __shfl(o.y, owner), __shfl(o.z, owner)};
                    const V3<R> pd = {__shfl(d.x, owner), __shfl(d.y, owner), __shfl(d.z, owner)};
                    uint32_t pfirst;
                    bool hit_back;
                    if constexpr (MULTI) {
                        const uint32_t pfirst_hb = uint32_t(__shfl(int(first | (mcur & 0x80000000u)), owner));
                        pfirst = pfirst_hb & 0x7FFFFFFFu;
                        hit_back = (pfirst_hb >> 31) != 0u;
                    } else {
                        pfirst = uint32_t(__shfl(int(first), owner));
                        hit_back = (rb0.flags & RT_MESH_HIT_BACK_FACES) != 0u;
                    }
                    R rt = Lim<R>::inf(), ru = R(0), rv = R(0);
                    if (act) {
                        if (STATS) cnt.tri_tests++;
                        tri_test(tris[pfirst + k], po, pd, hit_back, rt, ru, rv);
                    }
                    res_t[lane] = rt; res_u[lane] = ru; res_v[lane] = rv;
                    __builtin_amdgcn_wave_barrier();
                    if (leaf) {
                        const int jlo = max(0, int(c0) - int(pre));
                        const int jhi = min(int(count), int(c0) + 64 - int(pre));
                        for (int j = jlo; j < jhi; j++) {
                            const int idx = int(pre) + j - int(c0);
                            const R t = res_t[idx];
                            if (t <= t_lo || t_max <= t) continue;
                            t_max = t; hit_u = res_u[idx]; hit_v = res_v[idx];
                            hit_tri = int32_t(first + uint32_t(j));
                            if constexpr (MULTI) mcur = (mcur & 0xC0007FFFu) | (((mcur & 0x7FFFu) + 1u) << 15);
                        }
                    }
                    __builtin_amdgcn_wave_barrier();
                }
                if (leaf) {
                    tmax32 = f32_at_least(t_max - cr.t_shift);
                    pop_next();
                }
            }
        }
    }
    if (STATS) {
        atomicAdd(&counters->mesh_rays, (unsigned long long)cnt.mesh_rays);
        atomicAdd(&counters->node_visits, (unsigned long long)cnt.node_visits);
        atomicAdd(&counters->tri_tests, (unsigned long long)cnt.tri_tests);
        atomicAdd(&counters->refill_lanes, (unsigned long long)l_refill);
        atomicAdd(&counters->pops_culled, (unsigned long long)l_culled);
        uint32_t wn = w_node, wt = w_tri, wr = w_refill;
        if ((threadIdx.x & 63u) == 0) {
            atomicAdd(&counters->node_wave_iters, (unsigned long long)wn);
            atomicAdd(&counters->tri_wave_iters, (unsigned long long)wt);
            atomicAdd(&counters->refill_wave_iters, (unsigned long long)wr);
        }
    }
}

constexpr uint32_t kShadeListBytes = 2u * WF_CHUNK * 2u + 8u * 4u;
#ifndef RT_SHADE_WAVES
#define RT_SHADE_WAVES 5
#endif
#ifndef RT_SHADE_WAVES_LG
#define RT_SHADE_WAVES_LG (sizeof(R) == 8 ? 4 : RT_SHADE_WAVES)
#endif
#define RT_SHADE_BOUNDS __launch_bounds__(256, TEX ? 1 : (STATS ? 4 : (G::kLightGroups ? RT_SHADE_WAVES_LG : RT_SHADE_WAVES)))

#ifdef RT_SHADE_STAMPS
__device__ unsigned long long g_shade_stamps[16];
#define RT_STAMP(k)                                                     \
    do {                                                                \
        const unsigned long long now_ = __builtin_amdgcn_s_memtime();   \
        stamp_acc[k] += now_ - stamp_t;                                 \
        stamp_t = now_;                                                 \
    } while (0)
#else
#define RT_STAMP(k) do { } while (0)
#endif

template <typename R, bool STATS, int LDS, bool TEX, typename G = WfGroup<R>, bool FUSED = false>
__global__ void RT_SHADE_BOUNDS k_wf_shade(SceneView<R> sc_g, CameraView<R> cam, ParamsView<R> prm, WfPool<R> pool, G grp,
                                           const uint32_t* __restrict__ queue_in, uint32_t* __restrict__ queue_out,
                                           WfCounters* __restrict__ ctr, double* __restrict__ sample_L, DeviceCounters* counters,
                                           const WfPool<R>* __restrict__ pool_dev, uint32_t staged, uint32_t* __restrict__ mesh_queue) {
    static_assert(!FUSED || (!STATS && !TEX && LDS == 1), "only the lean variant with staged tables is fused");
    extern __shared__ __align__(16) char lds_raw[];
    uint16_t* alive_list = reinterpret_cast<uint16_t*>(lds_raw);
    uint16_t* dead_list = alive_list + WF_CHUNK;
    uint32_t* lc = reinterpret_cast<uint32_t*>(dead_list + WF_CHUNK);
    char* tables = reinterpret_cast<char*>(lc + 8);
    if (threadIdx.x < 8) lc[threadIdx.x] = 0;
    SceneView<R> sc = sc_g;
    if constexpr (LDS == 1) sc = scene_tables_to_lds<R, true>(sc_g, sc_g.lay_shade, sc_g.small_blob_shade, tables, staged);
    else if constexpr (LDS == 2) sc = scene_tables_to_lds<R, false>(sc_g, sc_g.lay_shade, sc_g.small_blob_shade, tables, staged);
    else __syncthreads();
    const uint32_t n = ctr->n_in;
    const bool full = n == pool.capacity;
    const uint32_t begin = blockIdx.x * WF_CHUNK;
// ... 407 lines not shown
```

Baseline: 1491 Msamples/s.

## Add per-child oriented slab culling to f64 quantised BVH4 mesh traversal

Each BVH4 child now stores a 16-bit oriented slab interval, taken along its quantised cone axis and bounding the projected triangle vertices, in spare padding of the 128-byte node line. The slab is built on the host and in refit. For f64 scenes with large meshes (at least 131072 triangles), the mesh kernel projects the ray segment between each child's box entry and exit onto that axis and culls children whose span misses the slab. The goal is fewer node visits and triangle tests on a dense mesh. In exchange, every node visit pays extra float arithmetic and a further 16-byte load, plus extra build and refit work.

```diff
diff --git a/include/rt_mi355.h b/include/rt_mi355.h
--- a/include/rt_mi355.h
+++ b/include/rt_mi355.h
@@ -234,6 +234,9 @@
 int rt_scene_mesh_stats(const RtSceneDesc* desc, uint64_t out[8]);
 int rt_scene_mesh_cones(const RtSceneDesc* desc, uint32_t mesh, uint32_t f32, int32_t* children_out, uint32_t* cones_out,
                         uint32_t node_capacity, uint32_t* n_nodes_out, double* tris_out, uint32_t tri_capacity, uint32_t* n_tris_out);
+
+int rt_scene_mesh_slabs(const RtSceneDesc* desc, uint32_t mesh, uint32_t f32, uint32_t* slabs_out, float* bounds_out, float* frames_out,
+                        double* pad_out, uint32_t node_capacity, uint32_t* n_nodes_out);
 int rt_debug_handout_replay(const uint32_t* policy, uint32_t n, uint32_t waves, const uint32_t* order, uint32_t n_order, uint32_t* asks_out,
                             uint32_t capacity, uint32_t* n_asks_out, uint32_t* atomics_out);
 int rt_scene_program(const RtSceneDesc* desc, int32_t* ops_out, uint32_t capacity, uint32_t* n_ops_out, uint64_t info[8]);
diff --git a/rust_raytracer_amd/api.py b/rust_raytracer_amd/api.py
--- a/rust_raytracer_amd/api.py
+++ b/rust_raytracer_amd/api.py
@@ -304,6 +304,10 @@
             lib.rt_scene_mesh_cones.argtypes = [C.POINTER(RtSceneDesc), C.c_uint32, C.c_uint32, C.c_void_p, C.c_void_p, C.c_uint32,
                                                 C.POINTER(C.c_uint32), C.c_void_p, C.c_uint32, C.POINTER(C.c_uint32)]
             lib.rt_scene_mesh_cones.restype = C.c_int
+        if hasattr(lib, "rt_scene_mesh_slabs"):
+            lib.rt_scene_mesh_slabs.argtypes = [C.POINTER(RtSceneDesc), C.c_uint32, C.c_uint32, C.c_void_p, C.c_void_p, C.c_void_p,
+                                                C.POINTER(C.c_double), C.c_uint32, C.POINTER(C.c_uint32)]
+            lib.rt_scene_mesh_slabs.restype = C.c_int
         if hasattr(lib, "rt_debug_handout_replay"):
             lib.rt_debug_handout_replay.argtypes = [C.c_void_p, C.c_uint32, C.c_uint32, C.c_void_p, C.c_uint32, C.c_void_p, C.c_uint32,
                                                     C.POINTER(C.c_uint32), C.c_void_p]
@@ -474,6 +478,23 @@
     return children, cones.view(np.int8).reshape(-1, 4, 4), tris
 
 
+def scene_mesh_slabs(desc, mesh: int = 0, f32: bool = False) -> dict:
+    import numpy as np
+    lib = load_device_lib()
+    nn, pad = C.c_uint32(), C.c_double()
+    st = lib.rt_scene_mesh_slabs(desc, mesh, int(f32), None, None, None, C.byref(pad), 0, C.byref(nn))
+    if st != RT_OK:
+        raise RtError(st, lib.rt_last_error().decode())
+    words = np.zeros((nn.value, 4), dtype=np.uint32)
+    bounds = np.zeros((nn.value, 4, 2), dtype=np.float32)
+    frames = np.zeros((nn.value, 4), dtype=np.float32)
+    st = lib.rt_scene_mesh_slabs(desc, mesh, int(f32), words.ctypes.data, bounds.ctypes.data, frames.ctypes.data, C.byref(pad),
+                                 nn.value, C.byref(nn))
+    if st != RT_OK:
+        raise RtError(st, lib.rt_last_error().decode())
+    return {"words": words, "bounds": bounds, "org": frames[:, :3].copy(), "inv_s": frames[:, 3].copy(), "pad": float(pad.value)}
+
+
 def scene_update_check(a, b) -> None:
     lib = load_device_lib()
     st = lib.rt_scene_update_check(a, b)
diff --git a/rust_raytracer_amd/csrc/rt_bvh.cpp b/rust_raytracer_amd/csrc/rt_bvh.cpp
--- a/rust_raytracer_amd/csrc/rt_bvh.cpp
+++ b/rust_raytracer_amd/csrc/rt_bvh.cpp
@@ -301,4 +301,37 @@
     }
 }
 
-}
+void build_mesh_slabs(const std::vector<BuildNode4>& nodes4, const std::vector<TriRec<double>>& tris, const std::vector<uint32_t>& cones,
+                      const BvhNode4q* qnodes, const double* node_pad, std::vector<uint32_t>* out) {
+    const size_t n_tris = tris.size();
+    struct Run { uint32_t lo = UINT32_MAX, hi = 0, count = 0; };
+    auto tri_at = [&](uint32_t t, double* v) {
+        const TriRec<double>& r = tris[t];
+        for (int a = 0; a < 3; a++) { v[a] = r.v0[a]; v[3 + a] = r.e1[a]; v[6 + a] = r.e2[a]; }
+    };
+    out->assign(4 * nodes4.size(), kNeutralSlab);
+    std::vector<Run> below(nodes4.size());
+    for (size_t i = nodes4.size(); i-- > 0;) {
+        const BuildNode4& nd = nodes4[i];
+        Run all;
+        for (int k = 0; k < 4; k++) {
+            const int32_t ch = nd.child[k];
+            if (ch == kEmptyChild) continue;
+            Run b;
+            if (ch >= 0) {
+                if (size_t(ch) <= i || size_t(ch) >= nodes4.size()) continue;
+                b = below[size_t(ch)];
+            } else {
+                const uint32_t code = uint32_t(~ch), first = code >> 3, count = (code & 7u) + 1u;
+                if (size_t(first) + count > n_tris) continue;
+                b.lo = first; b.hi = first + count; b.count = count;
+            }
+            (*out)[4 * i + size_t(k)] = rf_slab_word(cones[4 * i + size_t(k)], qnodes[i].org, qnodes[i].cell, node_pad[i], b.lo, b.hi, b.count, tri_at);
+            all.lo = std::min(all.lo, b.lo); all.hi = std::max(all.hi, b.hi);
+            all.count += b.count;
+        }
+        below[i] = all;
+    }
+}
+
+}
diff --git a/rust_raytracer_amd/csrc/rt_bvh.h b/rust_raytracer_amd/csrc/rt_bvh.h
--- a/rust_raytracer_amd/csrc/rt_bvh.h
+++ b/rust_raytracer_amd/csrc/rt_bvh.h
@@ -47,5 +47,7 @@
 ConeLimits cone_limits(bool f32);
 void build_mesh_cones(const std::vector<BuildNode4>& nodes4, const std::vector<TriRec<double>>& tris, const ConeLimits& lim,
                       std::vector<uint32_t>* out);
+void build_mesh_slabs(const std::vector<BuildNode4>& nodes4, const std::vector<TriRec<double>>& tris, const std::vector<uint32_t>& cones,
+                      const BvhNode4q* qnodes, const double* node_pad, std::vector<uint32_t>* out);
 
 }
diff --git a/rust_raytracer_amd/csrc/rt_kernels.hip b/rust_raytracer_amd/csrc/rt_kernels.hip
--- a/rust_raytracer_amd/csrc/rt_kernels.hip
+++ b/rust_raytracer_amd/csrc/rt_kernels.hip
@@ -261,6 +261,7 @@
         }
         std::vector<BvhNode4q> nodes4q(mesh_tables ? cs.nodes4.size() : 0);
         std::vector<BvhNode4q> group_nodes;
+        std::vector<double> node_pad;
         {
             auto pad_of = [&]() {
                 std::vector<std::pair<uint32_t, double>> pads;
@@ -278,11 +279,13 @@
             };
             const auto pads4 = pad_of();
             size_t pi = 0;
+            node_pad.resize(nodes4q.size());
             for (size_t i = 0; i < nodes4q.size(); i++) {
                 while (pi + 1 < pads4.size() && pads4[pi + 1].first <= i) pi++;
                 const BuildNode4& sn = cs.nodes4[i];
                 BvhNode4q& qn = nodes4q[i];
-                if (!quantise(sn, pads4.empty() ? 0.0 : pads4[pi].second, qn))
+                node_pad[i] = pads4.empty() ? 0.0 : pads4[pi].second;
+                if (!quantise(sn, node_pad[i], qn))
                     return set_err(RT_E_UNSUPPORTED, "BVH node does not fit the 8-bit grid");
             }
             group_nodes.resize(cs.group_nodes4.size());
@@ -302,10 +305,13 @@
         }
         std::vector<uint32_t> cone_words;
         if (mesh_tables) build_mesh_cones(cs.nodes4, cs.tris, cone_limits(sizeof(R) == 4), &cone_words);
+        std::vector<uint32_t> slab_words;
+        if (mesh_tables) build_mesh_slabs(cs.nodes4, cs.tris, cone_words, nodes4q.data(), node_pad.data(), &slab_words);
         std::vector<MeshNode4qc> nodes4qc(mesh_tables ? cs.nodes4.size() : 0);
         for (size_t i = 0; i < nodes4qc.size(); i++) {
             nodes4qc[i].node = nodes4q[i];
             for (int k = 0; k < 4; k++) nodes4qc[i].cones.word[k] = cone_words[4 * i + size_t(k)];
+            for (int k = 0; k < 4; k++) nodes4qc[i].slabs.word[k] = slab_words[4 * i + size_t(k)];
             for (uint32_t& x : nodes4qc[i]._pad) x = 0;
         }
         std::vector<Bounds<R>> mesh_bounds(cs.mesh_bounds.size());
@@ -711,6 +717,7 @@
     return RT_OK;
 }
 
+constexpr size_t kSlabsMinTriangles = 131072;
 static uint32_t env_u32(const char* name, uint32_t dflt) {
     const char* v = std::getenv(name);
     if (!v || !*v) return dflt;
@@ -740,13 +747,16 @@
 }
 
 template <typename R, bool ST>
-MeshKernel<R> pick_mesh_st(int node_kind, bool multi) {
+MeshKernel<R> pick_mesh_st(int node_kind, bool multi, bool slabs) {
+    if constexpr (sizeof(R) == 8) {
+        if (node_kind == 1 && slabs) return multi ? &k_wf_mesh<R, ST, 1, true, true> : &k_wf_mesh<R, ST, 1, false, true>;
+    }
     if (node_kind == 1) return multi ? &k_wf_mesh<R, ST, 1, true> : &k_wf_mesh<R, ST, 1, false>;
     return multi ? &k_wf_mesh<R, ST, 0, true> : &k_wf_mesh<R, ST, 0, false>;
 }
 template <typename R>
-MeshKernel<R> pick_mesh(bool stats, int node_kind, bool multi) {
-    return stats ? pick_mesh_st<R, true>(node_kind, multi) : pick_mesh_st<R, false>(node_kind, multi);
+MeshKernel<R> pick_mesh(bool stats, int node_kind, bool multi, bool slabs) {
+    return stats ? pick_mesh_st<R, true>(node_kind, multi, slabs) : pick_mesh_st<R, false>(node_kind, multi, slabs);
 }
 
 template <typename R, typename G>
@@ -770,6 +780,7 @@
     bool multi_mesh;
     int node_kind;
     uint32_t cones_on;
+    uint32_t slabs_on;
     int mesh_levels, lds_levels;
     uint32_t refill_min, inner_min;
     HandoutPolicy handout;
@@ -813,6 +824,10 @@
     su.multi_mesh = su.plan.multi_mesh || env_u32("RT_WF_MESH_MULTI", 0) != 0;
     su.node_kind = env_u32("RT_WF_NODES", 1) != 0 ? 1 : 0;
     su.cones_on = env_u32("RT_WF_CONES", 1) != 0 ? 1u : 0u;
+    size_t largest_mesh = 0;
+    for (const MeshInst& mi : s->compiled.meshes) largest_mesh = std::max(largest_mesh, size_t(mi.n_tris));
+    const uint32_t slabs_dflt = largest_mesh >= kSlabsMinTriangles ? 1u : 0u;
+    su.slabs_on = (sizeof(R) == 8 && su.node_kind == 1) ? std::min(env_u32("RT_WF_SLABS", slabs_dflt), 2u) : 0u;
     su.mesh_levels = int(s->compiled.max_bvh4_stack) + 1;
     su.lds_levels = std::min<int>(su.mesh_levels, int(env_u32("RT_WF_LDS_LEVELS", 12)));
     su.lds_mesh = size_t(su.lds_levels) * 256 * sizeof(uint2) + 4 * kMeshWaveLds<R>;
@@ -833,7 +848,7 @@
     su.lds_prims_launch = (vol ? size_t(0) : size_t(su.staged_prims) + su.lds_groups) + (WF_CHUNK + 4) * 4;
     su.k_intersect = pick_intersect<R>(stats, vol);
     su.k_prims = pick_prims<R>(stats, vol, su.groups, su.lds_prims);
-    su.k_mesh = pick_mesh<R>(stats, su.node_kind, su.multi_mesh);
+    su.k_mesh = pick_mesh<R>(stats, su.node_kind, su.multi_mesh, su.slabs_on != 0u);
     int n_cu = 0, blocks_per_cu = 0;
     HIP_TRY(hipDeviceGetAttribute(&n_cu, hipDeviceAttributeMultiprocessorCount, s->device));
     if (su.split) HIP_TRY(hipOccupancyMaxActiveBlocksPerMultiprocessor(&blocks_per_cu, su.k_mesh, 256, su.lds_mesh));
@@ -863,7 +878,7 @@
 template <typename R>
 void launch_mesh(const SearchSetup<R>& su, const DeviceScene<R>& ds, const WfPool<R>& pool, const SearchQueues& sq) {
     hipLaunchKernelGGL(su.k_mesh, dim3(su.isect_blocks), dim3(256), su.lds_mesh, sq.stream, ds.view, pool, sq.mesh_queue, sq.ctr, sq.counters,
-                       su.refill_min, su.inner_min, static_cast<uint2*>(sq.mesh_spill), su.lds_levels, &sq.ctr->n_mesh, &sq.ctr->cursor, su.cones_on, su.handout.mode, su.handout.left256, su.handout.left128);
+                       su.refill_min, su.inner_min, static_cast<uint2*>(sq.mesh_spill), su.lds_levels, &sq.ctr->n_mesh, &sq.ctr->cursor, su.cones_on, su.slabs_on, su.handout.mode, su.handout.left256, su.handout.left128);
 }
 template <typename R>
 void launch_intersect(const SearchSetup<R>& su, const DeviceScene<R>& ds, const WfPool<R>& pool, const SearchQueues& sq) {
@@ -2223,6 +2238,52 @@
     return RT_OK;
 }
 
+int rt_scene_mesh_slabs(const RtSceneDesc* desc, uint32_t mesh, uint32_t f32, uint32_t* slabs_out, float* bounds_out, float* frames_out,
+                        double* pad_out, uint32_t node_capacity, uint32_t* n_nodes_out) {
+    using namespace rt;
+    if (!desc || !n_nodes_out) return set_err(RT_E_INVALID, "rt_scene_mesh_slabs: NULL argument");
+    CompiledScene cs;
+    std::string err;
+    int st = compile_scene(desc, &cs, &err, CompileOptions());
+    if (st != RT_OK) return set_err(st, err);
+    if (mesh >= cs.meshes.size()) return set_err(RT_E_INVALID, "rt_scene_mesh_slabs: mesh index out of range");
+    const MeshInst& mi = cs.meshes[mesh];
+    size_t node_end = cs.nodes4.size();
+    for (const MeshInst& o : cs.meshes)
+        if (o.node4_base > mi.node4_base) node_end = std::min(node_end, size_t(o.node4_base));
+    const size_t n_nodes = node_end - mi.node4_base;
+    *n_nodes_out = uint32_t(n_nodes);
+    const double pad = rf_pad_of_box(cs.mesh_bounds[mesh].lo, cs.mesh_bounds[mesh].hi);
+    if (pad_out) *pad_out = pad;
+    if (!slabs_out) return RT_OK;
+    std::vector<uint32_t> cones, slabs;
+    build_mesh_cones(cs.nodes4, cs.tris, cone_limits(f32 != 0), &cones);
+    std::vector<BvhNode4q> qn(cs.nodes4.size());
+    std::vector<double> pads(cs.nodes4.size(), pad);
+    for (size_t i = 0; i < cs.nodes4.size(); i++) {
+        const bool own = i >= mi.node4_base && i < node_end;
+        const BuildNode4& sn = cs.nodes4[i];
+        if (own && !rf_quantise4(sn.lo, sn.hi, sn.child, pad, qn[i].org, qn[i].cell, qn[i].qlo, qn[i].qhi))
+            return set_err(RT_E_UNSUPPORTED, "BVH node does not fit the 8-bit grid");
+        if (!own)
+            for (int k = 0; k < 4; k++) cones[4 * i + size_t(k)] = kNeutralCone;
+    }
+    build_mesh_slabs(cs.nodes4, cs.tris, cones, qn.data(), pads.data(), &slabs);
+    for (size_t i = 0; i < n_nodes && i < node_capacity; i++) {
+        const size_t n = mi.node4_base + i;
+        for (int k = 0; k < 4; k++) {
+            const uint32_t w = slabs[4 * n + size_t(k)];
+            slabs_out[4 * i + size_t(k)] = w;
+            if (bounds_out) { bounds_out[8 * i + 2 * size_t(k)] = float(int16_t(w & 0xFFFFu)); bounds_out[8 * i + 2 * size_t(k) + 1] = float(int16_t(w >> 16)); }
+        }
+        if (frames_out) {
+            for (int a = 0; a < 3; a++) frames_out[4 * i + size_t(a)] = qn[n].org[a];
+            frames_out[4 * i + 3] = float(rf_slab_inv_scale(qn[n].cell));
+        }
+    }
+    return RT_OK;
+}
+
 int rt_scene_program(const RtSceneDesc* desc, int32_t* ops_out, uint32_t capacity, uint32_t* n_ops_out, uint64_t info[8]) {
     using namespace rt;
     if (!desc || !n_ops_out || !info) return set_err(RT_E_INVALID, "rt_scene_program: NULL argument");
diff --git a/rust_raytracer_amd/csrc/rt_refit.h b/rust_raytracer_amd/csrc/rt_refit.h
--- a/rust_raytracer_amd/csrc/rt_refit.h
+++ b/rust_raytracer_amd/csrc/rt_refit.h
@@ -182,6 +182,41 @@
     return word;
 }
 
+RT_HD inline double rf_slab_inv_scale(const float* cell) {
+    const double cmax = rf_max(double(cell[0]), rf_max(double(cell[1]), double(cell[2])));
+    return 0.25 / cmax;
+}
+RT_HD inline double rf_slab_margin(const int* q, double pad, double inv_s) {
+    const double l1 = double((q[0] < 0 ? -q[0] : q[0]) + (q[1] < 0 ? -q[1] : q[1]) + (q[2] < 0 ? -q[2] : q[2]));
+    return l1 * (2.0 * pad * inv_s + 1.0 / 4096.0);
+}
+
+template <typename TriAt>
+RT_HD inline uint32_t rf_slab_word(uint32_t cone, const float* org, const float* cell, double pad, uint32_t lo, uint32_t hi, uint32_t count, TriAt tri_at) {
+    if (cone == kNeutralCone || count == 0 || hi - lo != count) return kNeutralSlab;
+    const int q[3] = {int(int8_t(cone & 0xFFu)), int(int8_t((cone >> 8) & 0xFFu)), int(int8_t((cone >> 16) & 0xFFu))};
+    const double inv_s = rf_slab_inv_scale(cell);
+    if (!(inv_s > 0.0) || !std::isfinite(inv_s) || !std::isfinite(pad)) return kNeutralSlab;
+    double plo = INFINITY, phi = -INFINITY;
+    for (uint32_t t = lo; t < hi; t++) {
+        double v[9];
+        tri_at(t, v);
+        for (int c = 0; c < 3; c++) {
+            double x[3];
+            for (int a = 0; a < 3; a++) x[a] = c == 0 ? v[a] : v[a] + v[3 * c + a];
+            const double p = double(q[0]) * ((x[0] - double(org[0])) * inv_s) + double(q[1]) * ((x[1] - double(org[1])) * inv_s) +
+                             double(q[2]) * ((x[2] - double(org[2])) * inv_s);
+            plo = rf_min(plo, p);
+            phi = rf_max(phi, p);
+        }
+    }
+    if (!(plo <= phi) || !std::isfinite(plo) || !std::isfinite(phi)) return kNeutralSlab;
+    const double margin = rf_slab_margin(q, pad, inv_s);
+    const double l = rf_max(std::floor(plo - margin), -32768.0), h = rf_min(std::ceil(phi + margin), 32767.0);
+    if (!(l <= 32767.0 && h >= -32768.0)) return kNeutralSlab;
+    return (uint32_t(int32_t(l)) & 0xFFFFu) | (uint32_t(int32_t(h)) << 16);
+}
+
 #if defined(__HIP__)
 struct RefitMesh {
     uint32_t n_tris = 0, n_nodes = 0, n_nodes4 = 0, n_positions = 0, n_normals = 0, n_uvs = 0;
diff --git a/rust_raytracer_amd/csrc/rt_refit.hip b/rust_raytracer_amd/csrc/rt_refit.hip
--- a/rust_raytracer_amd/csrc/rt_refit.hip
+++ b/rust_raytracer_amd/csrc/rt_refit.hip
@@ -145,6 +145,7 @@
 
 __global__ void k_refit_nodes4(uint32_t n_nodes, double pad, const int32_t* __restrict__ child, const double* __restrict__ box,
                                const double* __restrict__ sum, const uint32_t* __restrict__ run, const double* __restrict__ tri_normal,
+                               const uint32_t* __restrict__ tri_order, const uint32_t* __restrict__ tri_pos, const double* __restrict__ positions,
                                BvhNode4f* __restrict__ nodes4, MeshNode4qc* __restrict__ nodes4q) {
     const uint32_t i = blockIdx.x * blockDim.x + threadIdx.x;
     if (i >= n_nodes) return;
@@ -160,7 +161,7 @@
         rf_pad_box4f(lo[k][1], hi[k][1], pad, &f.loy[k], &f.hiy[k]);
         rf_pad_box4f(lo[k][2], hi[k][2], pad, &f.loz[k], &f.hiz[k]);
     }
-    float org[3], cell[3];
+    float org[3] = {0.f, 0.f, 0.f}, cell[3] = {0.f, 0.f, 0.f};
     uint32_t qlo[3], qhi[3];
     MeshNode4qc& q = nodes4q[i];
     if (rf_quantise4(lo, hi, ch, pad, org, cell, qlo, qhi))
@@ -172,6 +173,18 @@
             word = rf_cone_word(tri_normal, r[0], r[1], r[2], sum + 3 * (4 * size_t(i) + k));
         }
         q.cones.word[k] = word;
+        uint32_t slab = kNeutralSlab;
+        if (word != kNeutralCone) {
+            const uint32_t* r = run + 3 * (4 * size_t(i) + k);
+            slab = rf_slab_word(word, org, cell, pad, r[0], r[1], r[2], [&](uint32_t slot, double* v) {
+                const size_t t = tri_order[slot];
+                const double* p0 = positions + 3 * size_t(tri_pos[3 * t]);
+                const double* p1 = positions + 3 * size_t(tri_pos[3 * t + 1]);
+                const double* p2 = positions + 3 * size_t(tri_pos[3 * t + 2]);
+                for (int a = 0; a < 3; a++) { v[a] = p0[a]; v[3 + a] = p1[a] - p0[a]; v[6 + a] = p2[a] - p0[a]; }
+            });
+        }
+        q.slabs.word[k] = slab;
     }
 }
 
@@ -242,7 +255,7 @@
                        rm.tri_box.get(), rm.tri_normal.get(), rm.box4.get(), rm.sum4.get(), rm.run4.get());
     hipLaunchKernelGGL((k_refit_nodes2<R>), grid_for(rm.n_nodes), block, 0, stream, rm.n_nodes, rm.box2.get(), t.nodes);
     hipLaunchKernelGGL(k_refit_nodes4, grid_for(rm.n_nodes4), block, 0, stream, rm.n_nodes4, t.pad4, rm.child4.get(), rm.box4.get(), rm.sum4.get(), rm.run4.get(),
-                       rm.tri_normal.get(), t.nodes4, t.nodes4q);
+                       rm.tri_normal.get(), rm.tri_order.get(), rm.tri_pos.get(), rm.positions.get(), t.nodes4, t.nodes4q);
     REFIT_TRY(hipGetLastError());
     return true;
 }
diff --git a/rust_raytracer_amd/csrc/rt_scene.h b/rust_raytracer_amd/csrc/rt_scene.h
--- a/rust_raytracer_amd/csrc/rt_scene.h
+++ b/rust_raytracer_amd/csrc/rt_scene.h
@@ -128,13 +128,18 @@
 struct alignas(16) NodeCones4 {
     uint32_t word[4];
 };
+struct alignas(16) NodeSlabs4 {
+    uint32_t word[4];
+};
 struct alignas(128) MeshNode4qc {
     BvhNode4q node;
     NodeCones4 cones;
-    uint32_t _pad[12];
+    NodeSlabs4 slabs;
+    uint32_t _pad[8];
 };
 static_assert(sizeof(MeshNode4qc) == 128, "one cache line per mesh node");
 constexpr uint32_t kNeutralCone = 0x7F000000u;
+constexpr uint32_t kNeutralSlab = 0x7FFF8000u;
 constexpr uint32_t kNoCullDir = 0x81000000u;
 
 template <typename R>
diff --git a/rust_raytracer_amd/csrc/rt_traverse.h b/rust_raytracer_amd/csrc/rt_traverse.h
--- a/rust_raytracer_amd/csrc/rt_traverse.h
+++ b/rust_raytracer_amd/csrc/rt_traverse.h
@@ -117,7 +117,7 @@
 constexpr float kNoEntry = __builtin_huge_valf();
 
 template <typename R>
-RT_DEV uint32_t node4q_entries(uint4 h0, uint4 h1, uint4 h2, const CullRay<R>& cr, float tmax32, const int32_t (&ch)[4], float (&nr)[4]) {
+RT_DEV uint32_t node4q_spans(uint4 h0, uint4 h1, uint4 h2, const CullRay<R>& cr, float tmax32, const int32_t (&ch)[4], float (&nr)[4], float (&fr)[4]) {
     const float ax = __uint_as_float(h0.w) * cr.ivx, ay = __uint_as_float(h1.x) * cr.ivy, az = __uint_as_float(h1.y) * cr.ivz;
     const float bx = fmaf(__uint_as_float(h0.x), cr.ivx, -cr.oix), by = fmaf(__uint_as_float(h0.y), cr.ivy, -cr.oiy), bz = fmaf(__uint_as_float(h0.z), cr.ivz, -cr.oiz);
     const bool negx = cr.negx(), negy = cr.negy(), negz = cr.negz();
@@ -133,9 +133,43 @@
         const float tf = fminf(fminf(fmaf(fxk, ax, bx), fmaf(fyk, ay, by)), fminf(fmaf(fzk, az, bz), tmax32));
         const bool h = (tn <= tf) && ch[k] != kEmptyChild;
         nr[k] = h ? tn : kNoEntry;
+        fr[k] = tf;
         entered |= uint32_t(h) << k;
     }
     return entered;
+}
+template <typename R>
+RT_DEV uint32_t node4q_entries(uint4 h0, uint4 h1, uint4 h2, const CullRay<R>& cr, float tmax32, const int32_t (&ch)[4], float (&nr)[4]) {
+    float fr[4];
+    return node4q_spans(h0, h1, h2, cr, tmax32, ch, nr, fr);
+}
+
+template <typename R>
+RT_DEV void node4q_cull_slabs(uint4 h0, uint4 h1, uint4 cn, uint4 sl, V3<R> o, V3<R> d, R t_shift, bool leaves_only, const int32_t (&ch)[4],
+                              const float (&fr)[4], float (&nr)[4]) {
+    const float cmax = fmaxf(fmaxf(__uint_as_float(h0.w), __uint_as_float(h1.x)), __uint_as_float(h1.y));
+    const float inv_s = __uint_as_float(0x7E000000u - __float_as_uint(cmax));
+    const float rx = (float(fma(d.x, t_shift, o.x)) - __uint_as_float(h0.x)) * inv_s;
+    const float ry = (float(fma(d.y, t_shift, o.y)) - __uint_as_float(h0.y)) * inv_s;
+    const float rz = (float(fma(d.z, t_shift, o.z)) - __uint_as_float(h0.z)) * inv_s;
+    float ex = float(d.x) * inv_s;
+    const float ey = float(d.y) * inv_s, ez = float(d.z) * inv_s;
+    const float em = fmaxf(fmaxf(fabsf(ex), fabsf(ey)), fabsf(ez));
+    const float gm = fmaxf(fmaxf(fmaxf(fabsf(__uint_as_float(h0.x)), fabsf(__uint_as_float(h0.y))), fabsf(__uint_as_float(h0.z))) * inv_s,
+                           fmaxf(fmaxf(fabsf(rx), fabsf(ry)), fabsf(rz)));
+    if (!(em > 1e-20f && em < 1e30f && gm < 65536.0f)) ex = __builtin_nanf("");
+    const uint32_t cw[4] = {cn.x, cn.y, cn.z, cn.w}, sw[4] = {sl.x, sl.y, sl.z, sl.w};
+#pragma unroll
+    for (int k = 0; k < 4; k++) {
+        const float qx = float(int(cw[k] << 24) >> 24), qy = float(int(cw[k] << 16) >> 24), qz = float(int(cw[k] << 8) >> 24);
+        const float A = fmaf(qx, rx, fmaf(qy, ry, qz * rz));
+        const float B = fmaf(qx, ex, fmaf(qy, ey, qz * ez));
+        const float pn = fmaf(nr[k], B, A), pf = fmaf(fr[k], B, A);
+        const float lo = float(int(sw[k] << 16) >> 16), hi = float(int(sw[k]) >> 16);
+        const bool out = bool(int(fmaxf(pn, pf) < lo) | int(fminf(pn, pf) > hi));
+        const bool may = bool(int(!leaves_only) | int(ch[k] < 0));
+        nr[k] = bool(int(out) & int(may)) ? kNoEntry : nr[k];
+    }
 }
 
 #define RT_CE(nr, ch, a, b)                                           \
diff --git a/rust_raytracer_amd/csrc/rt_wavefront.h b/rust_raytracer_amd/csrc/rt_wavefront.h
--- a/rust_raytracer_amd/csrc/rt_wavefront.h
+++ b/rust_raytracer_amd/csrc/rt_wavefront.h
@@ -670,14 +670,15 @@
 template <typename R> constexpr uint32_t kMeshStage = sizeof(R) == 8 ? kHandoutMax : 0u;
 template <typename R> constexpr uint32_t kMeshWaveLds = 1024u + 3u * 64u * uint32_t(sizeof(R)) + 4u * kMeshStage<R>;
 
-template <typename R, bool STATS, int NODE, bool MULTI>
-__global__ void __launch_bounds__(256, (sizeof(R) == 4 && !STATS && NODE == 1) ? 5 : RT_MESH_WAVES) k_wf_mesh(SceneView<R> sc, WfPool<R> pool, const uint32_t* __restrict__ mesh_queue,
+template <typename R, bool STATS, int NODE, bool MULTI, bool SLABS = false>
+__global__ void __launch_bounds__(256, (sizeof(R) == 4 && !STATS && NODE == 1) ? 5 : ((SLABS && STATS) ? 3 : RT_MESH_WAVES)) k_wf_mesh(SceneView<R> sc, WfPool<R> pool, const uint32_t* __restrict__ mesh_queue,
                                                                  WfCounters* __restrict__ ctr, DeviceCounters* counters,
                                                                  uint32_t refill_min, uint32_t inner_min,
                                                                  uint2* __restrict__ spill, int lds_levels,
                                                                  const uint32_t* __restrict__ n_ptr, uint32_t* __restrict__ cursor_ptr,
-                                                                 uint32_t cones_on, uint32_t handout_mode, uint32_t handout_256, uint32_t handout_128) {
+                                                                 uint32_t cones_on, uint32_t slabs_on, uint32_t handout_mode, uint32_t handout_256, uint32_t handout_128) {
     const HandoutPolicy handout{handout_mode, handout_256, handout_128};
+    static_assert(!SLABS || (sizeof(R) == 8 && NODE == 1), "the slab step exists for f64 and quantised nodes");
     extern __shared__ uint2 lds_stack2[];
     MeshStack stk;
     stk.lds = (LdsByte*)lds_stack2;
@@ -871,8 +872,15 @@
                     const uint4* nd = reinterpret_cast<const uint4*>(nodesq + node);
                     const uint4 h0 = nd[0], h1 = nd[1], h2 = nd[2];
                     const int4 cc = *reinterpret_cast<const int4*>(nd + 3);
-                    node4q_cull_cones(dirq, nd[4], cc, ch);
-                    node4q_entries(h0, h1, h2, cr, tmax32, ch, nr);
+                    const uint4 cn = nd[4];
+                    node4q_cull_cones(dirq, cn, cc, ch);
+                    if constexpr (SLABS) {
+                        float fr[4];
+                        node4q_spans(h0, h1, h2, cr, tmax32, ch, nr, fr);
+                        node4q_cull_slabs(h0, h1, cn, nd[5], o, d, cr.t_shift, slabs_on == 2u, ch, fr, nr);
+                    } else {
+                        node4q_entries(h0, h1, h2, cr, tmax32, ch, nr);
+                    }
                 } else {
                     const float4* nd = reinterpret_cast<const float4*>(nodes + node);
                     const uint32_t nearx = cr.negx() ? 3u : 0u, neary = cr.negy() ? 4u : 1u, nearz = cr.negz() ? 5u : 2u;
```

New measurement: 1599 Msamples/s (median of 6 runs). +7.2%, better.
